# amazon-science/gnn-tail-generalization

Hardware: AMD Instinct MI355X
Metric: teachergnn_fullgraph_train_steps_per_sec (higher is better)
Workload: dtype f32

## Files before the change

### gnn-tail-generalization_amd/_lib.py

```python
import ctypes
import os

import torch

_HERE = os.path.dirname(os.path.abspath(__file__))
LIB_PATH = os.path.join(_HERE, 'lib', 'libcoldbrew_hip.so')

_c_i32p = ctypes.c_void_p
_c_f32p = ctypes.c_void_p
_I64 = ctypes.c_int64
_I32 = ctypes.c_int32
_SZ = ctypes.c_size_t
_P = ctypes.c_void_p


class CsrView(ctypes.Structure):
    _fields_ = [('rowptr', _P), ('col', _P), ('col_flags', _I32), ('n_rows', _I64), ('n_edges', _I64),
                ('hub_threshold', _I32), ('n_hubs', _I32), ('n_chunks', _I32), ('hub_rows', _P), ('hub_chunk_ptr', _P),
                ('ws', _P), ('ws_bytes', _SZ)]


class TrunkStore(ctypes.Structure):
    _fields_ = [('mix_src', _P), ('ld_mix', _I64), ('mix_index', _P), ('c_act', ctypes.c_float), ('c_mix', ctypes.c_float), ('drop_p', ctypes.c_float),
                ('seed', ctypes.c_uint64), ('seed_dev', _P), ('row0', _I64), ('relu_bits', _P), ('bits_relu_only', _I32), ('out_act', _P), ('ld_act', _I64)]


_G = ctypes.POINTER(CsrView)
_S = ctypes.POINTER(TrunkStore)

SIGNATURES = {
    'cb_version': (ctypes.c_int, []),
    'cb_last_error': (ctypes.c_char_p, []),
    'cb_device_status': (ctypes.c_int, []),
    'cb_agg_gemm_handover_selftest': (ctypes.c_int, [_P]),
    'cb_rows_zero_outside_mask_f32': (ctypes.c_int, [_P, _I64, _I64, _I64, _P, _P, _P]),
    'cb_csr_workspace_bytes': (_SZ, [_I64, _I64]),
    'cb_csr_from_coo_i64': (ctypes.c_int, [_P, _P, _I64, _I64, _P, _P, _P, _P, _P, _P, _SZ, _P]),
    'cb_deg_norm_f32': (ctypes.c_int, [_P, _I64, _P, _P]),
    'cb_csr64_from_coo_i64': (ctypes.c_int, [_P, _P, _I64, _I64, _P, _P, _P, _P, _P, _P, _SZ, _P]),
    'cb_csr_rebase_i64': (ctypes.c_int, [_P, _I64, _I64, _P, _P]),
    'cb_deg_norm_i64ptr_f32': (ctypes.c_int, [_P, _I64, _P, _P]),
    'cb_spmm_hub_count': (ctypes.c_int, [_P, _I64, _I32, _P, _P]),
    'cb_spmm_hub_fill_scratch_ints': (_I64, [_I64]),
    'cb_spmm_hub_fill': (ctypes.c_int, [_P, _I64, _I32, _I32, _P, _P, _P, _P]),
    'cb_spmm_workspace_bytes': (_SZ, [_I64, _I64]),
    'cb_spmm_csr_f32': (ctypes.c_int, [_G, _P, _I32, _I64, _I64, _P, _P, _P, ctypes.c_int, _P, _I64, _P, _I64, _P]),
    'cb_dropout_f32': (ctypes.c_int, [_P, _P, _I64, ctypes.c_float, ctypes.c_uint64, _P, _I64, _P]),
    'cb_axpby_f32': (ctypes.c_int, [ctypes.c_float, _P, ctypes.c_float, _P, _P, _I64, _P]),
    'cb_colsum_workspace_bytes': (_SZ, [_I64, _I64]),
    'cb_act_bwd_f32': (ctypes.c_int, [_P, _P, _P, _P, _I64, _I64, _P, _P, _SZ, _P]),
    'cb_reduce_workspace_bytes': (_SZ, []),
    'cb_frobenius_norm_f32': (ctypes.c_int, [_P, _I64, _P, _P, _SZ, _P]),
    'cb_nll_logsoftmax_f32': (ctypes.c_int, [_P, _I64, _P, _P, _I64, _I64, _I64, _P, _P, _P, _SZ, _P]),
    'cb_adam_step_f32': (ctypes.c_int, [_P, _P, _P, _P, _I64, ctypes.c_float, ctypes.c_float, ctypes.c_float,
                                        ctypes.c_float, ctypes.c_float, _I64, _P, _P]),
    'cb_adam_multi_f32': (ctypes.c_int, [_I32, _P, _P, _P, _P, _P, _P, ctypes.c_float, ctypes.c_float, ctypes.c_float, ctypes.c_float,
                                         ctypes.c_float, _I64, _P, _P, _P]),
    'cb_gemm_nn_workspace_bytes': (_SZ, [_I64, _I64]),
    'cb_gemm_nn_splitk_workspace_bytes': (_SZ, [_I64, _I64, _I64]),
    'cb_gemm_nn_f32': (ctypes.c_int, [_P, _I64, _P, _I64, _P, _I64, _I64, _I64, _I64, _P, _P, _I64, _P, ctypes.c_int, _P, _SZ, _P]),
    'cb_gemm_nn_drop2_f32': (ctypes.c_int, [_P, _I64, _P, _I64, _P, _I64, _P, _I64, _I64, _I64, _I64, _P, _P, _I64, _P, ctypes.c_int,
                                            ctypes.c_float, ctypes.c_uint64, _P, _I64, _P, _SZ, _P]),
    'cb_gemm_tn_workspace_bytes': (_SZ, [_I64, _I64, _I64]),
    'cb_gemm_tn_f32': (ctypes.c_int, [_P, _I64, _P, _I64, _P, _P, _I64, _I64, _I64, _P, _SZ, _P]),
    'cb_spmm_csr_fused_f32': (ctypes.c_int, [_G, _P, _P, _I32, _I64, _I64, _P, _P, _P, _I64, _S, _P, _I64, _P]),
    'cb_trunk_layer_bwd_f32': (ctypes.c_int, [_P, _P, _P, _P, ctypes.c_int, _P, ctypes.c_int, _I64, _I64, ctypes.c_float, ctypes.c_uint64,
                                              _P, _I64, ctypes.c_float, ctypes.c_float, _P, ctypes.c_uint64, ctypes.c_float, _P, _P, _P, _SZ, _P]),
    'cb_gemm_nn_bf16out_f32': (ctypes.c_int, [_P, _I64, _P, _I64, _P, _I64, _I64, _I64, _I64, _P, _P, _I64, _P, ctypes.c_int, _P, _SZ, _P]),
    'cb_node_norm_fwd_f32': (ctypes.c_int, [_P, _P, _P, _I64, _I64, ctypes.c_float, ctypes.c_float, ctypes.c_float, _P]),
    'cb_node_norm_bwd_f32': (ctypes.c_int, [_P, _P, _P, _P, _I64, _I64, ctypes.c_float, ctypes.c_float, _P]),
    'cb_colstats_workspace_bytes': (_SZ, [_I64, _I64]),
    'cb_colstats_f32': (ctypes.c_int, [_P, _P, _P, _I64, _I64, _P, _P, _P, _SZ, _P]),
    'cb_col_affine_f32': (ctypes.c_int, [_P, _P, _P, _P, ctypes.c_float, _P, _I64, _I64, _P]),
    'cb_col_bwd_combine_f32': (ctypes.c_int, [_P, _P, _P, _P, _P, _P, ctypes.c_float, ctypes.c_float, _P, _I64, _I64, _P]),
    'cb_topk_replace_workspace_bytes': (_SZ, [_I64, _I64, _I64]),
    'cb_topk_replace_f32': (ctypes.c_int, [_P, _I64, _P, _I64, _I64, _I64, _I64, _I32, _P, _P, _P, _P, _SZ, _P]),
    'cb_gather_rows_f32': (ctypes.c_int, [_P, _I64, _P, _I64, _I64, _P, _P]),
    'cb_gather_rows_bf16_f32': (ctypes.c_int, [_P, _I64, _P, _I64, _I64, _P, _P]),
    'cb_adam_norm_workspace_bytes': (ctypes.c_size_t, [_I32]),
    'cb_adam_multi_norm_f32': (ctypes.c_int, [_I32, _P, _P, _P, _P, _P, _P, _P, ctypes.c_float, ctypes.c_float, ctypes.c_float, ctypes.c_float,
                                              ctypes.c_float, _I64, _P, _P, _P, _SZ, _P]),
    'cb_expand_rows_f32': (ctypes.c_int, [_P, _P, _I64, _I64, ctypes.c_float, _P, _P]),
    'cb_gemm_nn_store_rows_supported': (ctypes.c_int, [_P, _I64, _P, _I64, _P, _I64, _I64, _I64, _I64]),
    'cb_gemm_nn_store_rows_f32': (ctypes.c_int, [_P, _I64, _P, _I64, _P, _I64, _I64, _I64, _I64, _P, _P, _I64, _P, _P, _S, _P, _SZ, _P]),
    'cb_trunk_store_rows_f32': (ctypes.c_int, [_P, _P, _I64, _I64, _S, _P, _P]),
    'cb_agg_gemm_image_bytes': (_SZ, [_I64, _I64]),
    'cb_agg_gemm_image_f32': (ctypes.c_int, [_P, _I64, _I64, _I64, ctypes.c_int, _P, _SZ, _P]),
    'cb_spmm_gemm_f32': (ctypes.c_int, [_G, _P, _I64, _I64, _P, _P, ctypes.c_int, _P, _I64, _P, _I64, _P, _P, _P, _I64, _P, _I64, _P]),
    'cb_spmm_gemm_fused_f32': (ctypes.c_int, [_G, _P, _I64, _P, _I64, _I64, _P, _P, _S, _P, _I64, _I32, _P, _P, _P, _I64, _P, _I64, _P]),
    'cb_agg_gemm_head_image_bytes': (_SZ, [_I64, _I64]),
    'cb_agg_gemm_head_image_f32': (ctypes.c_int, [_P, _I64, _I64, _I64, ctypes.c_int, _P, _SZ, _P]),
    'cb_spmm_gemm_fused_head_f32': (ctypes.c_int, [_G, _P, _I64, _P, _I64, _I64, _P, _P, _S, _P, _I64, _I32, _P, _P, _I64, _P, _I64, _P]),
    'cb_spmm_gemm_store_rows_f32': (ctypes.c_int, [_G, _P, _I64, _I64, _P, _P, _I64, _P, _P, _P, _P, _S, _P, _I64, _P]),
    'cb_spmm_csr_weighted_f32': (ctypes.c_int, [_P, _P, _P, _I64, _I64, _P, _I64, _I64, _P, _P, ctypes.c_int, _P, _I64, _P]),
    'cb_spmm_edge_dot_f32': (ctypes.c_int, [_P, _P, _I64, _I64, _P, _I64, _P, _I64, _I64, _P, _P]),
    'cb_gemm_nn_indrop_supported': (ctypes.c_int, [_P, _I64, _P, _I64, _P, _I64, _P, _I64, _I64, _I64, _I64]),
    'cb_gemm_nn_indrop_drop2_f32': (ctypes.c_int, [_P, _I64, _P, _I64, _P, _I64, _P, _I64, _I64, _I64, _I64, _P, ctypes.c_int, ctypes.c_float,
                                                   ctypes.c_uint64, ctypes.c_float, ctypes.c_uint64, _P, _I64, _P, _P]),
    'cb_gemm_nn_indrop_f32': (ctypes.c_int, [_P, _I64, _P, _I64, _P, _I64, _I64, _I64, _I64, _P, _P, _I64, _P, ctypes.c_int, ctypes.c_float,
                                             ctypes.c_uint64, _P, _I64, _P, _P]),
    'cb_gemm_tn_adrop_supported': (ctypes.c_int, [_P, _I64, _P, _I64, _I64, _I64]),
    'cb_gemm_tn_adrop_f32': (ctypes.c_int, [_P, _I64, _P, _I64, _P, _P, _I64, _I64, _I64, ctypes.c_float, ctypes.c_uint64, _P, _I64, _P, _SZ, _P]),
    'cb_front_image_bytes': (_SZ, [_I64]),
    'cb_front_image_f32': (ctypes.c_int, [_P, _I64, _I64, ctypes.c_int, _P, _SZ, _P]),
    'cb_trunk_front_f32': (ctypes.c_int, [_P, _I64, _I64, _I64, _P, _P, _P, _P, _P, _I64, _P, _I64, _P, _P, _I64, _P, _I64, ctypes.c_float,
                                          ctypes.c_uint64, ctypes.c_uint64, _P, _I64, _P]),
    'cb_gemm_tn_gdrop_supported': (ctypes.c_int, [_P, _I64, _P, _I64, _I64, _I64]),
    'cb_gemm_tn_gdrop_f32': (ctypes.c_int, [_P, _I64, _P, _I64, _P, _I64, _I64, _I64, ctypes.c_float, ctypes.c_uint64, _P, _I64, _P, _SZ, _P]),
    'cb_spmm_csr_lp_f32': (ctypes.c_int, [_G, _P, _I64, _I64, _P, _P, _I64, ctypes.c_float, _P, _P, _I64, _P]),
    'cb_spmm_csr_prop_f32': (ctypes.c_int, [_G, _P, _I64, _I64, _P, _P, _I64, ctypes.c_float, ctypes.c_float, ctypes.c_float, _P, _P, _P, _I64, _P]),
    'cb_cs_workspace_bytes': (_SZ, [_I64, _I64]),
    'cb_cs_residual_init_f32': (ctypes.c_int, [_P, _I64, _P, _P, _I64, _I64, _I64, _P, _P, _P, _P, _P, _SZ, _P]),
    'cb_cs_correct_snap_f32': (ctypes.c_int, [_I32, _P, _I64, _P, _I64, _P, _P, _I64, _I64, _I64, _P, _I64, ctypes.c_float, _P, _P, _I64, _P, _P, _P]),
    'cb_trunk_input_bwd_multi_f32': (ctypes.c_int, [_P, ctypes.c_uint64, _I32, _P, _P, ctypes.c_float, _P, _P, _I64, _I64, ctypes.c_float,
                                                    _P, _I64, _P, _P, _SZ, _P, _P, _P]),
    'cb_trunk_input_bwd_multi_cs_f32': (ctypes.c_int, [_P, ctypes.c_uint64, _I32, _P, _P, ctypes.c_float, _P, _P, _I64, _I64, ctypes.c_float,
                                                       _P, _I64, _P, _P, _SZ, _P, _P, _I32, _P, _P, _P, _P, _P, _SZ, _P]),
    'cb_spmm_csr_store_bwd_f32': (ctypes.c_int, [_G, _P, _I64, _I64, _P, _P, _P, ctypes.c_float, ctypes.c_float, ctypes.c_uint64, _P, _I64, _P, _I64, _P, _I64, _P]),
    'cb_spmm_store_bwd_mix_workspace_bytes': (_SZ, [_I64, _I64, _I64]),
    'cb_spmm_csr_store_bwd_mix_f32': (ctypes.c_int, [_G, _P, _I64, _I64, _P, _P, _P, ctypes.c_float, ctypes.c_float, ctypes.c_uint64, _P, _I64, _P, _I64, _P, _I64,
                                                     _I32, _P, _P, _P, ctypes.c_float, _P, _P, _SZ, _P]),
    'cb_gemm_tn_instage_supported': (ctypes.c_int, [_P, _P, _P, _I64, _I64, _I64]),
    'cb_gemm_tn_instage_workspace_bytes': (_SZ, [_I64, _I64]),
    'cb_gemm_tn_instage_f32': (ctypes.c_int, [_P, _P, _P, _P, _I64, _P, _P, _I64, _I64, ctypes.c_float, ctypes.c_uint64, ctypes.c_float, ctypes.c_uint64, _P, _I64,
                                              _P, _SZ, _P]),
    'cb_trunk_layer_bwd_fold_f32': (ctypes.c_int, [_P, _P, _P, _P, _I64, _I64, ctypes.c_float, ctypes.c_uint64, _P, _I64, ctypes.c_float, ctypes.c_float, _I32, _P, _P, _P,
                                                   _P, _P, _P, _SZ, _I32, _P, ctypes.c_float, _P, _P, _SZ, _P]),
    'cb_trunk_layer_bwd_rows_f32': (ctypes.c_int, [_P, _P, _I64, _P, _P, _P, _I64, ctypes.c_float, ctypes.c_uint64, _P, _I64, ctypes.c_float,
                                                   _P, ctypes.c_uint64, ctypes.c_float, _P, _P, _P, _SZ, _P]),
    'cb_id_count_i64': (ctypes.c_int, [_P, _I64, _I64, _P, _P, _P]),
    'cb_value_hist_i32': (ctypes.c_int, [_P, _I64, _I32, _P, _P, _P]),
    'cb_compact_workspace_bytes': (_SZ, [_I64]),
    'cb_select_range_i32': (ctypes.c_int, [_P, _I64, _I32, _I32, _P, _P, _P, _P, _SZ, _P]),
    'cb_craft_isolation_i64': (ctypes.c_int, [_P, _P, _I64, _P, _I64, _P, _P, _P, _P, _SZ, _P]),
    'cb_symmetrize_workspace_bytes': (_SZ, [_I64, _I64]),
    'cb_symmetrize_i64': (ctypes.c_int, [_P, _P, _I64, _I64, _P, _P, _P, _P, _P, _SZ, _P]),
    'cb_trunk_input_bwd_f32': (ctypes.c_int, [_P, _P, _P, _P, _I64, _I64, ctypes.c_float, ctypes.c_uint64, _P, _I64, _P, _P, _SZ, _P]),
    'cb_ln_gelu_drop_fwd_f32': (ctypes.c_int, [_P, _I64, _I64, _P, _P, ctypes.c_float, ctypes.c_float, ctypes.c_uint64, _P, _P, _P, _P]),
    'cb_ln_gelu_drop_bwd_workspace_bytes': (_SZ, [_I64, _I64]),
    'cb_ln_gelu_drop_bwd_f32': (ctypes.c_int, [_P, _P, _P, _I64, _I64, _P, _P, ctypes.c_float, ctypes.c_uint64, _P, _P, _P, _P, _P, _P, _SZ, _P]),
    'cb_mse_rows_f32': (ctypes.c_int, [_P, _I64, _I64, _P, _I64, _I64, _P, _P, _P, _P, _SZ, _P]),
    'cb_part2_assemble_f32': (ctypes.c_int, [_P, _I64, _P, _P, _I64, _P, _I64, _P, _P]),
    'cb_part2_assemble_bwd_f32': (ctypes.c_int, [_P, _I64, _P, _P, _I64, _I64, _P, _P, _SZ, _P]),
    'cb_ncloss_positions_i64': (ctypes.c_int, [_P, _I64, _I64, _P, _P, _P]),
    'cb_ncloss_row_norms_f32': (ctypes.c_int, [_P, _I64, _I64, _I64, _P, _P, _P]),
    'cb_cosine_scale_f32': (ctypes.c_int, [_P, _I64, _I64, _P, _P]),
    'cb_ncloss_uses_limb_core': (ctypes.c_int, [_P, _I64, _I64]),
    'cb_ncloss_workspace_bytes': (_SZ, [_I64, _I32]),
    'cb_ncloss_fwd_f32': (ctypes.c_int, [_P, _I64, _I64, _I64, ctypes.c_float, _P, _P, _P, _I64, _P, _P, _P, _I32, _P, _P, _P, _P, _P, _P, _P, _P, _SZ, _P]),
    'cb_ncloss_normalize_rows_f32': (ctypes.c_int, [_P, _I64, _I64, _I64, _P, _P, _P]),
    'cb_ncloss_bwd_slab_f32': (ctypes.c_int, [_P, _I64, _I64, _I64, ctypes.c_float, _P, _P, _I64, _I64, _I32, _P, _I64, _P]),
    'cb_ncloss_bwd_finish_f32': (ctypes.c_int, [_P, _I64, _P, _I64, _I64, ctypes.c_float, _P, _P, _P, _P, _P, _P, _P, _P, _I64, _P, _P, _P, _P, _P, _P, _P]),
    'cb_spgemm_offsets_workspace_bytes': (_SZ, [_I64]),
    'cb_spgemm_entry_offsets_i64': (ctypes.c_int, [_P, _I64, _P, _I64, _P, _P, _P, _SZ, _P]),
    'cb_spgemm_chunk_workspace_bytes': (_SZ, [_I64]),
    'cb_spgemm_chunk_count_f32': (ctypes.c_int, [_P, _P, _P, _P, _P, _P, _P, _I64, _I64, _I64, _I64, _I64, _P, _P, _SZ, _P]),
    'cb_spgemm_chunk_emit_f32': (ctypes.c_int, [_P, _SZ, _I64, _I64, _I64, _I64, _I64, _I64, _P, _P, _P, _P]),
    'cb_csr_transpose_workspace_bytes': (_SZ, [_I64]),
    'cb_csr_transpose_f32': (ctypes.c_int, [_P, _P, _P, _I64, _I64, _I64, _P, _P, _P, _P, _SZ, _P]),
    'cb_linkp_max_tries': (ctypes.c_int, []),
    'cb_linkp_valid_counts_i32': (ctypes.c_int, [_P, _P, _I32, _P, _P]),
    'cb_linkp_positives_i32': (ctypes.c_int, [_P, _P, _I32, _P, _I64, _I64, ctypes.c_uint64, _P, _P, _P]),
    'cb_linkp_negatives_i32': (ctypes.c_int, [_P, _P, _I32, _P, _I64, _I64, ctypes.c_uint64, _P, _P, _P, _P]),
    'cb_linkp_loss_fwd_f32': (ctypes.c_int, [_P, _I64, _I64, _I64, _P, _I64, _P, _I64, _P, _P, _P, _P, _P]),
    'cb_linkp_mrr_f32': (ctypes.c_int, [_P, _I64, _P, _I64, _P, _P]),
    'cb_linkp_bwd_workspace_bytes': (_SZ, [_I64, _I64]),
    'cb_linkp_loss_bwd_f32': (ctypes.c_int, [_P, _I64, _I64, _I64, _P, _I64, _P, _I64, _P, _P, _P, _I64, _P, _SZ, _P]),
    'cb_heur_aa_weights_f64': (ctypes.c_int, [_P, _P, _P]),
    'cb_heur_pair_scores_f32': (ctypes.c_int, [_P, _P, _P, _I64, _P, _P, _P]),
    'cb_heur_pair_scores_width_f32': (ctypes.c_int, [_P, _P, _P, _I64, _I32, _P, _P, _P]),
    'cb_rank_counts_workspace_bytes': (_SZ, [_I64, _I64]),
    'cb_rank_counts_f32': (ctypes.c_int, [_P, _I64, _P, _I64, _P, _P, _P, _P, _SZ, _P]),
    'cb_lpx_max_tries': (ctypes.c_int, []),
    'cb_lpx_neg_global_i32': (ctypes.c_int, [_P, _I64, ctypes.c_uint64, _P, _P, _P]),
    'cb_lpx_neg_local_i32': (ctypes.c_int, [_P, _I64, _I64, _I64, ctypes.c_uint64, _P, _P]),
    'cb_lpx_permutation_workspace_bytes': (_SZ, [_I64]),
    'cb_lpx_permutation_i32': (ctypes.c_int, [_I64, ctypes.c_uint64, _P, _P, _SZ, _P]),
    'cb_lpx_row_ranks_f32': (ctypes.c_int, [_P, _I64, _P, _I64, _I64, _P, _P, _P, _P]),
    'cb_lpx_recall_topk_workspace_bytes': (_SZ, [_I64, _I64]),
    'cb_lpx_recall_topk_f32': (ctypes.c_int, [_P, _I64, _P, _I64, _I64, _P, _P, _P, _SZ, _P]),
    'cb_pair_gemm_nn_supported': (ctypes.c_int, [_P, _I64, _P, _I64, _I64, _I64]),
    'cb_pair_gemm_nn_f32': (ctypes.c_int, [_P, _I64, _I64, _P, _I64, _P, _I64, _P, _I64, _P, _I64, _I64, _I64, _P, ctypes.c_int, ctypes.c_float,
                                           ctypes.c_uint64, _P, _I64, _P, _P]),
    'cb_pair_dot_f32': (ctypes.c_int, [_P, _I64, _I64, _I64, _P, _I64, _P, _P, _P]),
    'cb_pair_scatter_workspace_bytes': (_SZ, [_I64]),
    'cb_pair_scatter_f32': (ctypes.c_int, [_P, _I64, _I64, _I64, _P, _I64, _P, _I64, _P, _I64, _P, _SZ, _P]),
    'cb_rank_loss_workspace_bytes': (_SZ, []),
    'cb_rank_loss_fwd_f32': (ctypes.c_int, [_I32, _P, _I64, _P, _I64, _P, _P, _P, _SZ, _P]),
    'cb_rank_loss_bwd_f32': (ctypes.c_int, [_I32, _P, _I64, _P, _I64, _P, _P, _P, _P, _P]),
    'cb_rows_gemm_nn_supported': (ctypes.c_int, [_P, _I64, _I64, _I32, _P, _I64, _I64]),
    'cb_rows_gemm_nn_f32': (ctypes.c_int, [_P, _I64, _I64, _I64, _P, _I32, _I64, _P, _I64, _P, _I64, _P, _I64, _I64, _P, ctypes.c_int, ctypes.c_float,
                                           ctypes.c_uint64, _P, _I64, _P, _P]),
    'cb_rows_bilinear_supported': (ctypes.c_int, [_P, _I64, _I64, _P, _I64]),
    'cb_rows_bilinear_workspace_bytes': (_SZ, [_I64, _I64]),
    'cb_rows_bilinear_f32': (ctypes.c_int, [_P, _I64, _I64, _I64, _P, _I64, _P, _I64, _P, _P, _P, _SZ, _P]),
    'cb_rows_scatter_f32': (ctypes.c_int, [_I64, _I64, _P, _I64, _P, _I64, _P, _I64, _P, _I64, _P, _SZ, _P]),
    'cb_sage_image_bytes': (_SZ, [ctypes.c_int]),
    'cb_sage_image_f32': (ctypes.c_int, [_P, _I64, _P, _I64, ctypes.c_int, _P, _SZ, _P]),
    'cb_sage_layer_supported': (ctypes.c_int, [_I64, _I64, _I32, _P, _I64, _P, _I64, _P, _I64, _P, _I64]),
    'cb_sage_layer_f32': (ctypes.c_int, [_P, _P, _I64, _P, _I64, _P, _P, _P, _P, ctypes.c_int, ctypes.c_float, ctypes.c_uint64, _P, _I64, _P, _I64, _I32,
                                         _P, _I64, _P]),
    'cb_attn_supported': (ctypes.c_int, [_I64, _P, _I64]),
    'cb_attn_workspace_bytes': (_SZ, [_I64, _I64]),
    'cb_attn_fwd_f32': (ctypes.c_int, [_P, _I64, _P, _I64, _P, _I64, _P, _I64, _P, _I64, ctypes.c_int, _P, _I64, _P, _P]),
    'cb_attn_bwd_dst_f32': (ctypes.c_int, [_P, _I64, _P, _I64, _P, _I64, _P, _I64, _P, _I64, _P, _P, _I64, _P, _P]),
    'cb_attn_bwd_src_f32': (ctypes.c_int, [_P, _I64, _P, _I64, _P, _I64, _P, _I64, _P, _I64, _P, _P, _P, _I64, _P, _I64, _P]),
}

# ... 89 lines not shown
```

### gnn-tail-generalization_amd/csrc/cb_front.hip

```cpp
#include <type_traits>

#include "cb_common.h"
#include "cb_limb_core.h"
#include "cb_philox.h"
#include "cb_tile_gemm.h"
#include "cb_trunk_store.h"

namespace cb {

struct FrontArgs {
  const float* x;
  int64_t ld_x;
  const uint4* image_in;
  const float* bias_in;
  const uint4* image_0;
  const float* rowscale;
  const float* addend;
  int64_t ld_add;
  float* x0;
  int64_t ld_x0;
  unsigned long long* bits;
  float* x0_drop;
  int64_t ld_drop;
  float* z0;
  int64_t ld_z;
  int64_t M;
  uint32_t thresh;
  float keep_scale;
  uint64_t seed_x, seed_x0;
  const uint64_t* seed_dev;
  int64_t row0;
  int n_tiles;
};

template <int NS1, bool DROP>
__global__ void __launch_bounds__(256, 2) k_front(FrontArgs fa) {
  constexpr int K1 = 16 * NS1, LDX = K1 + 4, NV = kTM * K1 / 4 / 256;
  static_assert(NV >= 1 && kTM * LDX <= kTM * kTLD, "x tile must fit the region of the X0 tile");
  static_assert(NV == NS1 && NS1 <= 8, "mask draws: one quad per K step, P0's bits in one word");
  __shared__ __attribute__((aligned(16))) float tile[kTM * kTLD];
  constexpr int kScratch = 2 * RowOperand<kTM>::BYTES > 4 * 8 * kCLD * 4 ? 2 * RowOperand<kTM>::BYTES : 4 * 8 * kCLD * 4;
  __shared__ __attribute__((aligned(16))) char scratch[kScratch];
  float (*cstrip)[8 * kCLD] = reinterpret_cast<float (*)[8 * kCLD]>(scratch);
  __shared__ float rs_tile[2][kTM];
  const int t = threadIdx.x, lane = t & 63, w = __builtin_amdgcn_readfirstlane(t >> 6);
  const uint64_t sx = fa.seed_dev ? fa.seed_x + *fa.seed_dev : fa.seed_x, s0 = fa.seed_dev ? fa.seed_x0 + *fa.seed_dev : fa.seed_x0;
  float4 xr[NV];
  auto load_x = [&](int tile_id) {
    const int64_t m0 = (int64_t)tile_id * kTM;
#pragma unroll
    for (int j = 0; j < NV; ++j) {
      const int idx = t + 256 * j, row = idx / (K1 / 4), c4 = idx % (K1 / 4);
      const int64_t m = m0 + row;
      xr[j] = (tile_id < fa.n_tiles && m < fa.M) ? *reinterpret_cast<const float4*>(fa.x + m * fa.ld_x + 4 * c4) : make_float4(0.f, 0.f, 0.f, 0.f);
    }
  };
  float rs_next = 1.f;
  auto load_rs = [&](int tile_id) {
    const int64_t m = (int64_t)tile_id * kTM + t;
    rs_next = (t < kTM && fa.rowscale && tile_id < fa.n_tiles && m < fa.M) ? fa.rowscale[m] : 1.f;
  };
  float bvec[4] = {0.f, 0.f, 0.f, 0.f};
  if (fa.bias_in) {
#pragma unroll
    for (int i = 0; i < 4; ++i) bvec[i] = fa.bias_in[4 * lane + i];
  }
  load_rs(blockIdx.x);
  load_x(blockIdx.x);
  uint32_t kx = 0;
  uint64_t k3 = 0;
  int64_t qx = 0, q3 = 0;
  auto aim_x = [&](int tile_id) { qx = (fa.row0 + (int64_t)tile_id * kTM) * (K1 / 4) + t; };
  auto aim_3 = [&](int tile_id) { q3 = (fa.row0 + (int64_t)tile_id * kTM + 16 * w) * (kND / 4) + lane; };
  auto draw_x = [&](int) {
    uint64_t seed = sx;
    asm volatile("" : "+s"(seed));
    kx = (kx >> 4) | (keep4_bits(seed, qx, fa.thresh) << 28);
    qx += 256;
    asm volatile("" : "+v"(kx));
  };
  auto draw_3 = [&](int) {
    uint64_t seed = s0;
    asm volatile("" : "+s"(seed));
    k3 = (k3 >> 4) | ((uint64_t)keep4_bits(seed, q3, fa.thresh) << 60);
    q3 += kND / 4;
    asm volatile("" : "+v"(k3));
  };
  if constexpr (DROP) {
    aim_x(blockIdx.x);
    aim_3(blockIdx.x);
#pragma unroll 1
    for (int s = 0; s < 16; ++s) {
      if (s < NS1) draw_x(s);
      draw_3(s);
    }
  }
  int par = 0;
  for (int tile_id = blockIdx.x; tile_id < fa.n_tiles; tile_id += gridDim.x, par ^= 1) {
    const int64_t m0 = (int64_t)tile_id * kTM;
#pragma unroll
    for (int j = 0; j < NV; ++j) {
      const int idx = t + 256 * j, row = idx / (K1 / 4), c4 = idx % (K1 / 4);
      float v[4] = {xr[j].x, xr[j].y, xr[j].z, xr[j].w};
      if constexpr (DROP) {
#pragma unroll
        for (int i = 0; i < 4; ++i) v[i] = mul_rounded(v[i], (kx >> (32 - 4 * NV + 4 * j + i)) & 1u ? fa.keep_scale : 0.f);
      }
      *reinterpret_cast<float4*>(tile + row * LDX + 4 * c4) = make_float4(v[0], v[1], v[2], v[3]);
    }
    if constexpr (DROP) aim_x(tile_id + (int)gridDim.x);
    if (t < kTM) rs_tile[par][t] = rs_next;
    __syncthreads();
    f32x16 acc[2][2];
    if constexpr (DROP) tile_times_image_coop<NS1, LDX, 1>(tile, scratch, fa.image_in, w, lane, t, acc, draw_x);
    else tile_times_image_coop<NS1, LDX, 1>(tile, scratch, fa.image_in, w, lane, t, acc);
    {
      const int l31 = lane & 31, lh = lane >> 5;
#pragma unroll
      for (int i = 0; i < 2; ++i)
#pragma unroll
        for (int j = 0; j < 2; ++j)
#pragma unroll
          for (int reg = 0; reg < 16; ++reg)
            tile[(32 * i + (reg & 3) + 8 * (reg >> 2) + 4 * lh) * kTLD + 64 * w + 32 * j + l31] = acc[i][j][reg];
    }
    __syncthreads();
#pragma unroll 4
    for (int r = 0; r < 16; ++r) {
      const int row = 16 * w + r;
      const int64_t m = m0 + row;
      float* tp = tile + row * kTLD + 4 * lane;
      const float4 v = *reinterpret_cast<const float4*>(tp);
      float o[4] = {v.x, v.y, v.z, v.w};
#pragma unroll
      for (int i = 0; i < 4; ++i) o[i] = fmaxf(o[i] + bvec[i], 0.f);
      float xd[4] = {o[0], o[1], o[2], o[3]};
      if constexpr (DROP) {
#pragma unroll
        for (int i = 0; i < 4; ++i) xd[i] = o[i] * ((uint32_t)k3 >> i & 1u ? fa.keep_scale : 0.f);
        k3 >>= 4;
      }
      *reinterpret_cast<float4*>(tp) = make_float4(xd[0], xd[1], xd[2], xd[3]);
      if (m < fa.M) {
        store_stream4(fa.x0 + m * fa.ld_x0 + 4 * lane, o);
        if (fa.bits) {
          const bool pos[4] = {o[0] > 0.f, o[1] > 0.f, o[2] > 0.f, o[3] > 0.f};
          write_row_mask_words(fa.bits + m * 4, lane, pos);
        }
        if (fa.x0_drop) store_stream4(fa.x0_drop + m * fa.ld_drop + 4 * lane, xd);
      }
    }
    __syncthreads();
    if constexpr (DROP) aim_3(tile_id + (int)gridDim.x);
    if constexpr (DROP) tile_times_image_coop<kNS, kTLD, 1>(tile, scratch, fa.image_0, w, lane, t, acc, draw_3);
    else tile_times_image_coop<kNS, kTLD, 1>(tile, scratch, fa.image_0, w, lane, t, acc);
    load_rs(tile_id + gridDim.x);
    load_x(tile_id + gridDim.x);
    auto z0_epilogue = [&](auto HAS_ADD) {
      acc_rows_through_strip(acc, cstrip[w], w, lane, [&](int row, int n, const float4& v) {
        const int64_t m = m0 + row;
        if (m < fa.M) {
          const float rs = rs_tile[par][row];
          float ad[4] = {0.f, 0.f, 0.f, 0.f};
          if constexpr (decltype(HAS_ADD)::value) {
            const float4 a4 = *reinterpret_cast<const float4*>(fa.addend + m * fa.ld_add + n);
            ad[0] = a4.x; ad[1] = a4.y; ad[2] = a4.z; ad[3] = a4.w;
          }
          const float zero_bias = 0.f;
          float o[4] = {v.x, v.y, v.z, v.w};
#pragma unroll
          for (int e = 0; e < 4; ++e) o[e] = o[e] * rs + ad[e] + zero_bias;
          store_stream4(fa.z0 + m * fa.ld_z + n, o);
        }
      });
    };
    if (fa.addend) z0_epilogue(std::true_type{});
    else z0_epilogue(std::false_type{});
  }
}

}

using namespace cb;

extern "C" size_t cb_front_image_bytes(int64_t K) {
  if (K != 64 && K != 128) return 0;
  return (size_t)(K / 16) * kNT * 3 * 64 * sizeof(uint4);
}

extern "C" int cb_front_image_f32(const float* W, int64_t ld, int64_t K, int transpose, void* image, size_t image_bytes, void* stream) {
  CB_CHECK_ARG(cb_front_image_bytes(K) > 0, CB_E_INVALID, "cb_front_image_f32: K must be 64 or 128 (got %lld)", (long long)K);
  CB_CHECK_ARG(W && image && ld >= (transpose ? K : kND), CB_E_INVALID, "cb_front_image_f32: null pointer / bad leading dimension");
  CB_CHECK_ARG(image_bytes >= cb_front_image_bytes(K) && aligned16(image), CB_E_WORKSPACE, "cb_front_image_f32: image buffer too small or misaligned");
  const int64_t sk = transpose ? 1 : ld, sn = transpose ? ld : 1;
  const int ns = (int)(K / 16);
  hipLaunchKernelGGL(k_weight_image, dim3(ns * kNT * 64 / 256), dim3(256), 0, (hipStream_t)stream, W, sk, sn, (uint4*)image, ns);
  CB_LAUNCH_CHECK();
  return CB_OK;
}

extern "C" int cb_trunk_front_f32(const float* x, int64_t ld_x, int64_t M, int64_t K, const void* image_in, const float* bias_in, const void* image_0,
                                  const float* rowscale, const float* addend, int64_t ld_add, float* x0, int64_t ld_x0, uint64_t* relu_bits,
                                  float* x0_drop, int64_t ld_drop, float* z0, int64_t ld_z, float drop_p, uint64_t seed_x, uint64_t seed_x0,
                                  const uint64_t* seed_dev, int64_t row0, void* stream) {
  CB_CHECK_ARG(M >= 0 && cb_front_image_bytes(K) > 0 && drop_p >= 0.f && drop_p < 1.f && row0 >= 0, CB_E_INVALID,
               "cb_trunk_front_f32: bad size (K must be 64 or 128; hidden width 256) or p");
  CB_CHECK_ARG(M < ((int64_t)1 << 31) * kTM / 2, CB_E_RANGE, "cb_trunk_front_f32: size out of range");
  if (M == 0) return CB_OK;
  CB_CHECK_ARG(x && image_in && image_0 && x0 && z0, CB_E_INVALID, "cb_trunk_front_f32: null pointer");
  CB_CHECK_ARG(aligned16(x) && ld_x % 4 == 0 && ld_x >= K && aligned16(image_in) && aligned16(image_0) && aligned16(x0) && ld_x0 % 4 == 0 && ld_x0 >= kND &&
                   aligned16(z0) && ld_z % 4 == 0 && ld_z >= kND && (!addend || (aligned16(addend) && ld_add % 4 == 0 && ld_add >= kND)) &&
                   (!x0_drop || (aligned16(x0_drop) && ld_drop % 4 == 0 && ld_drop >= kND)) && (!relu_bits || (uintptr_t)relu_bits % 8 == 0),
               CB_E_INVALID, "cb_trunk_front_f32: 16-byte aligned rows required");
  FrontArgs fa{x, ld_x, (const uint4*)image_in, bias_in, (const uint4*)image_0, rowscale, addend, ld_add, x0, ld_x0, (unsigned long long*)relu_bits,
               x0_drop, ld_drop, z0, ld_z, M};
  fa.thresh = drop_p > 0.f ? dropout_threshold(drop_p) : 0u;
  fa.keep_scale = 1.f / (1.f - drop_p);
  fa.seed_x = seed_x; fa.seed_x0 = seed_x0; fa.seed_dev = seed_dev; fa.row0 = row0;
  fa.n_tiles = (int)((M + kTM - 1) / kTM);
  int dev = 0, n_cu = 0;
  if (hipGetDevice(&dev) != hipSuccess || hipDeviceGetAttribute(&n_cu, hipDeviceAttributeMultiprocessorCount, dev) != hipSuccess || n_cu <= 0) n_cu = 256;
  const int blocks = fa.n_tiles < 2 * n_cu ? fa.n_tiles : 2 * n_cu;
  const dim3 grid((unsigned)blocks), blk(256);
  hipStream_t st = (hipStream_t)stream;
  if (K == 64 && fa.thresh) hipLaunchKernelGGL((k_front<4, true>), grid, blk, 0, st, fa);
  else if (K == 64) hipLaunchKernelGGL((k_front<4, false>), grid, blk, 0, st, fa);
  else if (fa.thresh) hipLaunchKernelGGL((k_front<8, true>), grid, blk, 0, st, fa);
  else hipLaunchKernelGGL((k_front<8, false>), grid, blk, 0, st, fa);
  CB_LAUNCH_CHECK();
  return CB_OK;
}
```

### gnn-tail-generalization_amd/csrc/cb_gemm.hip

```cpp
#include <stdlib.h>

#include "cb_common.h"
#include "cb_gemm_core.h"
#include "cb_gemm_limb.h"

namespace cb {

template <int WM, int WN, bool ALIGNED, bool OUT_BF16, int BKT = BK, int WTN = 2>
__global__ void __launch_bounds__(256) k_gemm_nn(const float* __restrict__ A, int64_t lda, const float* __restrict__ B, int64_t ldb,
                                                 void* __restrict__ Cv, int64_t ldc, int64_t M, int N, int K, GemmEpilogue ep,
                                                 int n_row_blocks, int n_col_blocks, int c_vec_ok, int k_chunk) {
  using T = Tile<WM, WN, BKT, WTN>;
  if (k_chunk) {
    const int k0 = blockIdx.y * k_chunk;
    A += k0;
    B += (int64_t)k0 * ldb;
    Cv = reinterpret_cast<float*>(Cv) + (int64_t)blockIdx.y * M * ldc;
    K = min(k_chunk, K - k0);
  }
  constexpr int BM = T::BM, BN = T::BN, LDA = T::LDA, LDB = T::LDB;
  __shared__ __attribute__((aligned(16))) float smem[T::SMEM_FLOATS];
  auto As = [&](int b) { return smem + b * (BKT * LDA); };
  auto Bs = [&](int b) { return smem + 2 * BKT * LDA + b * (BKT * LDB); };
  const int per_group = 8 * n_col_blocks;
// ... 302 lines not shown
               "cb_gemm_nn_bf16out_f32: null pointer or leading dimension too small");
  GemmEpilogue ep{rowscale, addend, ld_add, bias, relu, nullptr, 0, 0u, 1.f, 0ull, nullptr, 0, gemm_nt_store(M, N)};
  hipStream_t st = (hipStream_t)stream;
  if (limb3_on() && limb3_nn_eligible(A, lda, B, ldb, N, K)) return launch_nn_limb3(A, lda, B, ldb, C, ldc, M, N, K, ep, true, st, ws, ws_bytes);
  if (N <= 64) return launch_nn<4, 1, true>(A, lda, B, ldb, C, ldc, M, N, K, ep, st);
  return launch_nn<2, 2, true>(A, lda, B, ldb, C, ldc, M, N, K, ep, st);
}

extern "C" size_t cb_gemm_tn_workspace_bytes(int64_t M, int64_t K1, int64_t K2) {
  if (M <= 0 || K1 <= 0 || K2 <= 0) return 0;
  int bm, bn;
  tn_tile(K1, K2, bm, bn);
  const int tiles = (int)(((K1 + bm - 1) / bm) * ((K2 + bn - 1) / bn));
  return (size_t)tn_splits(M, tiles) * (size_t)K1 * (size_t)K2 * sizeof(float);
}

extern "C" int cb_gemm_nn_store_rows_supported(const float* A, int64_t lda, const float* B, int64_t ldb, const float* C, int64_t ldc, int64_t M, int64_t N,
                                               int64_t K) {
  return limb3_on() && N == 256 && M > 0 && limb3_nn_eligible(A, lda, B, ldb, N, K) && aligned16(C) && ldc % 4 == 0 ? 1 : 0;
}

extern "C" int cb_gemm_nn_store_rows_f32(const float* A, int64_t lda, const float* B, int64_t ldb, float* C, int64_t ldc, int64_t M, int64_t N, int64_t K,
                                         const float* rowscale, const float* addend, int64_t ld_add, const float* bias, const int64_t* row_index,
                                         const cb_trunk_store* store, void* ws, size_t ws_bytes, void* stream) {
  CB_CHECK_ARG(M >= 0 && N == 256 && K > 0, CB_E_INVALID, "cb_gemm_nn_store_rows_f32: bad size (N must be 256)");
  CB_CHECK_ARG(K < (1 << 24) && (M + 63) / 64 < (1 << 24), CB_E_RANGE, "cb_gemm_nn_store_rows_f32: size out of range");
  if (M == 0) return CB_OK;
  CB_CHECK_ARG(A && B && C && row_index && lda >= K && ldb >= N && ldc >= N && (!addend || ld_add >= N), CB_E_INVALID,
               "cb_gemm_nn_store_rows_f32: null pointer or leading dimension too small");
  const int rcs = check_trunk_store("cb_gemm_nn_store_rows_f32", store, N);
  if (rcs != CB_OK) return rcs;
  CB_CHECK_ARG(cb_gemm_nn_store_rows_supported(A, lda, B, ldb, C, ldc, M, N, K) && (!addend || (aligned16(addend) && ld_add % 4 == 0)), CB_E_INVALID,
               "cb_gemm_nn_store_rows_f32: shape / alignment outside the fused form (cb_gemm_nn_store_rows_supported)");
  GemmEpilogue ep{rowscale, addend, ld_add, bias, 1, nullptr, 0, 0u, 1.f, 0ull, nullptr, 0, 0};
  ep.row_ids = row_index; ep.st = make_trunk_store(*store);
  return launch_nn_limb3(A, lda, B, ldb, C, ldc, M, N, K, ep, false, (hipStream_t)stream, ws, ws_bytes);
}

extern "C" int cb_gemm_tn_f32(const float* A, int64_t lda, const float* G, int64_t ldg, const float* rowscale, float* C, int64_t M,
                              int64_t K1, int64_t K2, void* ws, size_t ws_bytes, void* stream) {
  CB_CHECK_ARG(M >= 0 && K1 >= 0 && K2 >= 0, CB_E_INVALID, "cb_gemm_tn_f32: negative size");
  CB_CHECK_ARG(K1 < (1 << 20) && K2 < (1 << 20), CB_E_RANGE, "cb_gemm_tn_f32: size out of range");
  if (K1 == 0 || K2 == 0) return CB_OK;
  CB_CHECK_ARG(C && (M == 0 || (A && G)) && lda >= K1 && ldg >= K2, CB_E_INVALID, "cb_gemm_tn_f32: null pointer or bad ld");
  hipStream_t st = (hipStream_t)stream;
  if (M == 0) {
    CB_HIP(hipMemsetAsync(C, 0, (size_t)K1 * K2 * sizeof(float), st));
    return CB_OK;
  }
  CB_CHECK_ARG(ws && ws_bytes >= cb_gemm_tn_workspace_bytes(M, K1, K2), CB_E_WORKSPACE, "cb_gemm_tn_f32: workspace too small");
  int bm, bn;
  tn_tile(K1, K2, bm, bn);
  if (bm == 64) return launch_tn<1, 4>(A, lda, G, ldg, rowscale, C, M, K1, K2, (float*)ws, st);
  if (bm == 256) return launch_tn<4, 1>(A, lda, G, ldg, rowscale, C, M, K1, K2, (float*)ws, st);
  return launch_tn<2, 2>(A, lda, G, ldg, rowscale, C, M, K1, K2, (float*)ws, st);
}

extern "C" int cb_gemm_tn_gdrop_supported(const float* A, int64_t lda, const float* G, int64_t ldg, int64_t K1, int64_t K2) {
  return limb3_on() && K2 % 4 == 0 && limb3_tn_eligible(A, lda, G, ldg, K1, K2) ? 1 : 0;
}

extern "C" int cb_gemm_tn_gdrop_f32(const float* A, int64_t lda, const float* G, int64_t ldg, float* C, int64_t M, int64_t K1, int64_t K2,
                                    float g_drop_p, uint64_t g_seed, const uint64_t* seed_dev, int64_t row0, void* ws, size_t ws_bytes,
                                    void* stream) {
  CB_CHECK_ARG(M >= 0 && K1 >= 0 && K2 >= 0 && g_drop_p > 0.f && g_drop_p < 1.f && row0 >= 0, CB_E_INVALID, "cb_gemm_tn_gdrop_f32: bad size or p");
  CB_CHECK_ARG(K1 < (1 << 20) && K2 < (1 << 20), CB_E_RANGE, "cb_gemm_tn_gdrop_f32: size out of range");
  if (K1 == 0 || K2 == 0) return CB_OK;
  CB_CHECK_ARG(C && (M == 0 || (A && G)) && lda >= K1 && ldg >= K2, CB_E_INVALID, "cb_gemm_tn_gdrop_f32: null pointer or bad ld");
  hipStream_t st = (hipStream_t)stream;
  if (M == 0) {
    CB_HIP(hipMemsetAsync(C, 0, (size_t)K1 * K2 * sizeof(float), st));
    return CB_OK;
  }
  CB_CHECK_ARG(cb_gemm_tn_gdrop_supported(A, lda, G, ldg, K1, K2), CB_E_INVALID, "cb_gemm_tn_gdrop_f32: operands outside the three-limb path");
  CB_CHECK_ARG(ws && ws_bytes >= cb_gemm_tn_workspace_bytes(M, K1, K2), CB_E_WORKSPACE, "cb_gemm_tn_gdrop_f32: workspace too small");
  const DropSpec gd{dropout_threshold(g_drop_p), 1.f / (1.f - g_drop_p), g_seed, seed_dev, row0, K2};
  int bm, bn;
  tn_tile(K1, K2, bm, bn);
  if (bm == 64) return launch_tn<1, 4>(A, lda, G, ldg, nullptr, C, M, K1, K2, (float*)ws, st, &gd);
  if (bm == 256) return launch_tn<4, 1>(A, lda, G, ldg, nullptr, C, M, K1, K2, (float*)ws, st, &gd);
  return launch_tn<2, 2>(A, lda, G, ldg, nullptr, C, M, K1, K2, (float*)ws, st, &gd);
}

static inline int instage_splits(int64_t M) { return tn_splits(M, 2); }

extern "C" int cb_gemm_tn_instage_supported(const float* g, const float* mfold, const float* X, int64_t ldx, int64_t M, int64_t K2) {
  return limb3_on() && K2 > 64 && K2 <= 128 && K2 % 4 == 0 && ldx % 4 == 0 && ldx >= K2 && ldx < (1 << 22) && aligned16(g) && aligned16(mfold) && aligned16(X) && M > 0 &&
                 instage_splits(M) >= 256
             ? 1
             : 0;
}

extern "C" size_t cb_gemm_tn_instage_workspace_bytes(int64_t M, int64_t K2) {
  if (M <= 0 || K2 <= 0) return 0;
  return (size_t)instage_splits(M) * (size_t)256 * (size_t)(K2 + 1) * sizeof(float);
}

extern "C" int cb_gemm_tn_instage_f32(const float* g, const float* mfold, const uint64_t* x0_bits, const float* X, int64_t ldx, float* C, float* colsum, int64_t M,
                                      int64_t K2, float g_drop_p, uint64_t g_seed, float x_drop_p, uint64_t x_seed, const uint64_t* seed_dev, int64_t row0, void* ws,
                                      size_t ws_bytes, void* stream) {
  CB_CHECK_ARG(M > 0 && K2 > 0 && g_drop_p > 0.f && g_drop_p < 1.f && x_drop_p > 0.f && x_drop_p < 1.f && row0 >= 0, CB_E_INVALID,
               "cb_gemm_tn_instage_f32: bad size or p (both dropouts must be active)");
  CB_CHECK_ARG(g && mfold && x0_bits && X && C && colsum && (uintptr_t)x0_bits % 8 == 0, CB_E_INVALID, "cb_gemm_tn_instage_f32: null or misaligned pointer");
  CB_CHECK_ARG(cb_gemm_tn_instage_supported(g, mfold, X, ldx, M, K2), CB_E_INVALID, "cb_gemm_tn_instage_f32: shape / alignment outside the fused form (cb_gemm_tn_instage_supported)");
  CB_CHECK_ARG(ws && ws_bytes >= cb_gemm_tn_instage_workspace_bytes(M, K2), CB_E_WORKSPACE, "cb_gemm_tn_instage_f32: workspace too small");
  hipStream_t st = (hipStream_t)stream;
  const int nsplit = instage_splits(M);
  int64_t rows_per_split = (M + nsplit - 1) / nsplit;
  rows_per_split = (rows_per_split + 31) / 32 * 32;
  const DropSpec xd{dropout_threshold(x_drop_p), 1.f / (1.f - x_drop_p), x_seed, seed_dev, row0, K2};
  const DropSpec gd{dropout_threshold(g_drop_p), 1.f / (1.f - g_drop_p), g_seed, seed_dev, row0, 256};
  float* partial = (float*)ws;
  float* cs_partial = partial + (size_t)nsplit * 256 * K2;
  const int rc = launch_tn_instage(g, mfold, x0_bits, X, ldx, partial, cs_partial, M, K2, nsplit, rows_per_split, st, xd, gd);
  if (rc != CB_OK) return rc;
  const int64_t n = 256 * K2;
  hipLaunchKernelGGL(k_sum_partials, dim3((unsigned)((n + 255) / 256)), dim3(256), 0, st, (const float*)partial, nsplit, n, C);
  CB_LAUNCH_CHECK();
  hipLaunchKernelGGL(k_sum_partials, dim3(1), dim3(256), 0, st, (const float*)cs_partial, nsplit, (int64_t)256, colsum);
  CB_LAUNCH_CHECK();
  return CB_OK;
}

extern "C" int cb_gemm_nn_indrop_f32(const float* A, int64_t lda, const float* B, int64_t ldb, float* C, int64_t ldc, int64_t M, int64_t N, int64_t K,
                                     const float* rowscale, const float* addend, int64_t ld_add, const float* bias, int relu, float a_drop_p,
                                     uint64_t a_seed, const uint64_t* seed_dev, int64_t row0, uint64_t* relu_bits, void* stream) {
  CB_CHECK_ARG(M >= 0 && N >= 0 && K >= 0 && a_drop_p > 0.f && a_drop_p < 1.f && row0 >= 0, CB_E_INVALID, "cb_gemm_nn_indrop_f32: bad size or p");
  CB_CHECK_ARG(!relu_bits || (N == 256 && relu && (uintptr_t)relu_bits % 8 == 0), CB_E_INVALID,
               "cb_gemm_nn_indrop_f32: mask words of the ReLU exist for N == 256 with relu only");
  CB_CHECK_ARG(N < (1 << 24) && K < (1 << 24) && (M + 63) / 64 < (1 << 24), CB_E_RANGE, "cb_gemm_nn_indrop_f32: size out of range");
  if (M == 0 || N == 0) return CB_OK;
  CB_CHECK_ARG(C && A && B && lda >= K && ldb >= N && ldc >= N && (!addend || ld_add >= N), CB_E_INVALID, "cb_gemm_nn_indrop_f32: null pointer or bad ld");
  CB_CHECK_ARG(cb_gemm_nn_indrop_supported(A, lda, B, ldb, C, ldc, C, ldc, M, N, K) && (!addend || (aligned16(addend) && ld_add % 4 == 0)), CB_E_INVALID,
               "cb_gemm_nn_indrop_f32: shape / alignment outside the fused form (cb_gemm_nn_indrop_supported)");
  GemmEpilogue ep{rowscale, addend, ld_add, bias, relu, nullptr, 0, 0u, 1.f, 0ull, nullptr, 0, gemm_nt_store(M, N)};
  ep.adrop = DropSpec{dropout_threshold(a_drop_p), 1.f / (1.f - a_drop_p), a_seed, seed_dev, row0, K};
  ep.relu_bits_out = (unsigned long long*)relu_bits;
  return launch_nn_limb3(A, lda, B, ldb, C, ldc, M, N, K, ep, false, (hipStream_t)stream, nullptr, 0);
}

extern "C" int cb_gemm_tn_adrop_supported(const float* A, int64_t lda, const float* G, int64_t ldg, int64_t K1, int64_t K2) {
  int bm, bn;
  tn_tile(K1, K2, bm, bn);
  return limb3_on() && K1 % 4 == 0 && bm == 128 && limb3_tn_eligible(A, lda, G, ldg, K1, K2) ? 1 : 0;
}

extern "C" int cb_gemm_tn_adrop_f32(const float* A, int64_t lda, const float* G, int64_t ldg, const float* rowscale, float* C, int64_t M, int64_t K1,
                                    int64_t K2, float a_drop_p, uint64_t a_seed, const uint64_t* seed_dev, int64_t row0, void* ws, size_t ws_bytes,
                                    void* stream) {
  CB_CHECK_ARG(M >= 0 && K1 >= 0 && K2 >= 0 && a_drop_p > 0.f && a_drop_p < 1.f && row0 >= 0, CB_E_INVALID, "cb_gemm_tn_adrop_f32: bad size or p");
  CB_CHECK_ARG(K1 < (1 << 20) && K2 < (1 << 20), CB_E_RANGE, "cb_gemm_tn_adrop_f32: size out of range");
  if (K1 == 0 || K2 == 0) return CB_OK;
  CB_CHECK_ARG(C && (M == 0 || (A && G)) && lda >= K1 && ldg >= K2, CB_E_INVALID, "cb_gemm_tn_adrop_f32: null pointer or bad ld");
  hipStream_t st = (hipStream_t)stream;
  if (M == 0) {
    CB_HIP(hipMemsetAsync(C, 0, (size_t)K1 * K2 * sizeof(float), st));
    return CB_OK;
  }
  CB_CHECK_ARG(cb_gemm_tn_adrop_supported(A, lda, G, ldg, K1, K2), CB_E_INVALID, "cb_gemm_tn_adrop_f32: operands outside the three-limb 128-row tile path");
  CB_CHECK_ARG(ws && ws_bytes >= cb_gemm_tn_workspace_bytes(M, K1, K2), CB_E_WORKSPACE, "cb_gemm_tn_adrop_f32: workspace too small");
  const DropSpec ad{dropout_threshold(a_drop_p), 1.f / (1.f - a_drop_p), a_seed, seed_dev, row0, K1};
  return launch_tn<2, 2>(A, lda, G, ldg, rowscale, C, M, K1, K2, (float*)ws, st, nullptr, &ad);
}
```

### gnn-tail-generalization_amd/csrc/cb_gemm_limb.h

```cpp
#pragma once
#include "cb_gemm_core.h"

namespace cb {

bool limb3_on();
bool limb3_nn_eligible(const float* A, int64_t lda, const float* B, int64_t ldb, int64_t N, int64_t K);
size_t limb3_nn_workspace_bytes(int64_t N, int64_t K);
int launch_nn_limb3(const float* A, int64_t lda, const float* B, int64_t ldb, void* C, int64_t ldc, int64_t M, int64_t N, int64_t K,
                    const GemmEpilogue& ep, bool out_bf16, hipStream_t st, void* ws = nullptr, size_t ws_bytes = 0);
bool limb3_nn_dual_eligible(const float* A, int64_t lda, const float* B, int64_t ldb, const float* C, int64_t ldc, const float* C2, int64_t ldc2,
                            int64_t M, int64_t N, int64_t K, const GemmEpilogue& ep);
bool limb3_tn_eligible(const float* A, int64_t lda, const float* G, int64_t ldg, int64_t K1, int64_t K2);
int launch_tn_limb3(const float* A, int64_t lda, const float* G, int64_t ldg, const float* rowscale, float* partial, int64_t M,
                    int64_t K1, int64_t K2, int bm, int nsplit, int64_t rows_per_split, hipStream_t st, const DropSpec* gdrop = nullptr,
                    const DropSpec* adrop = nullptr);

int launch_tn_instage(const float* g, const float* mfold, const uint64_t* x0_bits, const float* X, int64_t ldx, float* partial, float* cs_partial, int64_t M, int64_t K2,
                      int nsplit, int64_t rows_per_split, hipStream_t st, const DropSpec& xd, const DropSpec& gd);

}
```

### gnn-tail-generalization_amd/csrc/cb_gemm_limb.hip

```cpp
#include <stdlib.h>

#include <utility>

#include "cb_common.h"
#include "cb_gemm_core.h"
#include "cb_gemm_limb.h"
#include "cb_limb_core.h"

namespace cb {

template <int WM, int WN, int WTN = 2, int PD = 1>
struct LTile {
  static constexpr int BM = 64 * WM, BN = 32 * WTN * WN;
  static constexpr int MINW = (WM == 2 && WTN == 2 && PD < 3 ? 3 : 2);
  static constexpr int NTHR = 64 * WM * WN;
  static_assert(WM * WN == 4 || WM * WN == 8, "four or eight wavefronts per block");
};

template <int WM, int WN, bool OUT_BF16, int WTN = 2, int PD = 1, int EPI = 0, bool ADROP = false>
__global__ void __launch_bounds__(256, (LTile<WM, WN, WTN, PD>::MINW)) k_gemm_nn_l3(const float* __restrict__ A, int64_t lda,
                                                                                 const float* __restrict__ B, int64_t ldb,
                                                                                 void* __restrict__ Cv, int64_t ldc, int64_t M, int N,
                                                                                 int K, GemmEpilogue ep, int n_row_blocks,
                                                                                 int n_col_blocks, int c_vec_ok) {
  using T = LTile<WM, WN, WTN>;
  using OA = RowOperand<T::BM, ADROP>;
  using OB = ColOperand<T::BN, false>;
  constexpr int BM = T::BM, BN = T::BN;
  constexpr int SMEM = 2 * (OA::BYTES + OB::BYTES);
  static_assert(32 * (BN + 4) * 4 <= SMEM, "epilogue staging must fit");
  __shared__ __attribute__((aligned(16))) char smem[SMEM];
  const int per_group = 8 * n_col_blocks;
  const int grp = blockIdx.x / per_group, r = blockIdx.x % per_group;
  const int row_blk = grp * 8 + (r & 7), col_blk = r >> 3;
  if (row_blk >= n_row_blocks) return;
  const int64_t m0 = (int64_t)row_blk * BM;
  const int n0 = col_blk * BN;
  const int t = threadIdx.x, lane = t & 63, w = t >> 6, wr = w / WN, wc = w % WN;

  f32x16 acc[2][WTN];
  zero_acc_n<WTN>(acc);
  OA oa;
  OB ob;
  oa.init(lda, M - m0, t);
  if constexpr (ADROP) oa.set_drop(ep.adrop, m0, K, t);
  ob.init(ldb, N - n0, t);
  const uint32_t aaddr[2] = {OA::frag_addr(wr * 64, lane), OA::frag_addr(wr * 64 + 32, lane)};
  uint32_t baddr[WTN];
#pragma unroll
  for (int j = 0; j < WTN; ++j) baddr[j] = OB::frag_addr(wc * (32 * WTN) + 32 * j, lane);
  limb_k_loop<WTN, PD, OA, OB>(oa, ob, smem, A + m0 * lda, KS, lda, B + n0, (int64_t)KS * ldb, ldb, nullptr, K, aaddr, baddr, acc, t);
  nn_epilogue<WM, WN, WTN, OUT_BF16, EPI>(acc, reinterpret_cast<float*>(smem), Cv, ldc, m0, n0, M, N, ep, c_vec_ok, t);
}

template <int WM, int WN, bool SCALED, int WTN = 2, int PD = 1, bool GDROP = false, bool ADROP = false>
__global__ void __launch_bounds__((LTile<WM, WN, WTN, PD>::NTHR), (LTile<WM, WN, WTN, PD>::MINW)) k_gemm_tn_l3(const float* __restrict__ A, int64_t lda,
                                                                                 const float* __restrict__ G, int64_t ldg,
                                                                                 const float* __restrict__ rowscale,
                                                                                 float* __restrict__ partial, int64_t M, int K1, int K2,
                                                                                 int64_t rows_per_split, int tiles_j, int n_tiles,
                                                                                 int nsplit, DropSpec gd) {
  using T = LTile<WM, WN, WTN>;
  using OA = ColOperand<T::BM, false, ADROP, T::NTHR>;
  using OB = ColOperand<T::BN, SCALED, GDROP, T::NTHR>;
  constexpr int BM = T::BM, BN = T::BN;
  __shared__ __attribute__((aligned(16))) char smem[2 * (OA::BYTES + OB::BYTES)];
  const int b = blockIdx.x;
  const int tile = (b >> 3) % n_tiles, split = (b & 7) + 8 * (b / (8 * n_tiles));
  if (split >= nsplit) return;
  const int i0 = (tile / tiles_j) * BM, j0 = (tile % tiles_j) * BN;
  const int64_t r_begin = (int64_t)split * rows_per_split;
  const int64_t r_end = min(M, r_begin + rows_per_split);
  const int t = threadIdx.x, lane = t & 63, w = t >> 6, wr = w / WN, wc = w % WN;

  f32x16 acc[2][WTN];
  zero_acc_n<WTN>(acc);
  OA oa;
  OB ob;
  oa.init(lda, K1 - i0, t);
  ob.init(ldg, K2 - j0, t);
  if constexpr (GDROP) ob.set_drop(gd, r_begin, r_end - r_begin, j0, t);
  if constexpr (ADROP) oa.set_drop(gd, r_begin, r_end - r_begin, i0, t);
  const uint32_t aaddr[2] = {OA::frag_addr(wr * 64, lane), OA::frag_addr(wr * 64 + 32, lane)};
  uint32_t baddr[WTN];
#pragma unroll
  for (int j = 0; j < WTN; ++j) baddr[j] = OB::frag_addr(wc * (32 * WTN) + 32 * j, lane);
  limb_k_loop<WTN, PD, OA, OB>(oa, ob, smem, A + r_begin * lda + i0, (int64_t)KS * lda, lda, G + r_begin * ldg + j0, (int64_t)KS * ldg, ldg,
                           SCALED ? rowscale + r_begin : nullptr, r_end - r_begin, aaddr, baddr, acc, t);
  const int l31 = lane & 31, lh = lane >> 5;
  float* P = partial + (int64_t)split * K1 * K2;
#pragma unroll
  for (int ti = 0; ti < 2; ++ti)
#pragma unroll
    for (int tj = 0; tj < WTN; ++tj) {
      const int n = j0 + wc * (32 * WTN) + tj * 32 + l31;
      if (n >= K2) continue;
#pragma unroll
      for (int reg = 0; reg < 16; ++reg) {
        const int m = i0 + wr * 64 + ti * 32 + (reg & 3) + 8 * (reg >> 2) + 4 * lh;
        if (m < K1) P[(int64_t)m * K2 + n] = acc[ti][tj][reg];
      }
    }
}

__global__ void __launch_bounds__(512, 2) k_gemm_tn_instage(const float* __restrict__ g, const float* __restrict__ mfold,
                                                            const unsigned long long* __restrict__ x0_bits, const float* __restrict__ X, int64_t ldx,
                                                            float* __restrict__ partial, float* __restrict__ cs_partial, int64_t M, int K2,
                                                            int64_t rows_per_split, int nsplit, DropSpec xd, DropSpec gd) {
  using T = LTile<4, 2, 2>;
  using OA = ColOperandInStage<T::NTHR>;
  using OB = ColOperand<T::BN, false, true, T::NTHR>;
  constexpr int K1 = 256;
  __shared__ __attribute__((aligned(16))) char smem[2 * (OA::BYTES + OB::BYTES)];
  const int split = blockIdx.x;
  if (split >= nsplit) return;
  const int64_t r_begin = (int64_t)split * rows_per_split;
  const int64_t r_end = min(M, r_begin + rows_per_split);
  const int t = threadIdx.x, lane = t & 63, w = t >> 6, wr = w / 2, wc = w % 2;

  f32x16 acc[2][2];
  zero_acc_n<2>(acc);
  OA oa;
  OB ob;
  oa.init(K1, K1, t);
  ob.init(ldx, K2, t);
  oa.set_stage(g, mfold, x0_bits + r_begin * 4, gd, r_begin, r_end - r_begin, t);
  ob.set_drop(xd, r_begin, r_end - r_begin, 0, t);
  const uint32_t aaddr[2] = {OA::frag_addr(wr * 64, lane), OA::frag_addr(wr * 64 + 32, lane)};
  uint32_t baddr[2];
#pragma unroll
  for (int j = 0; j < 2; ++j) baddr[j] = OB::frag_addr(wc * 64 + 32 * j, lane);
  limb_k_loop<2, 1, OA, OB>(oa, ob, smem, g + r_begin * K1, (int64_t)KS * K1, K1, X + r_begin * ldx, (int64_t)KS * ldx, ldx, nullptr, r_end - r_begin, aaddr, baddr,
                            acc, t);
  const int l31 = lane & 31, lh = lane >> 5;
  float* P = partial + (int64_t)split * K1 * K2;
#pragma unroll
  for (int ti = 0; ti < 2; ++ti)
#pragma unroll
    for (int tj = 0; tj < 2; ++tj) {
      const int n = wc * 64 + tj * 32 + l31;
      if (n >= K2) continue;
#pragma unroll
      for (int reg = 0; reg < 16; ++reg) {
        const int m = wr * 64 + ti * 32 + (reg & 3) + 8 * (reg >> 2) + 4 * lh;
        P[(int64_t)m * K2 + n] = acc[ti][tj][reg];
      }
    }
  float* red = reinterpret_cast<float*>(smem);
#pragma unroll
  for (int i = 0; i < 4; ++i) red[w * 256 + lane * 4 + i] = oa.cs[i];
  __syncthreads();
  if (t < 256) {
    float s = 0.f;
#pragma unroll
    for (int j = 0; j < 8; ++j) s += red[j * 256 + t];
    cs_partial[(int64_t)split * 256 + t] = s;
  }
}

int launch_tn_instage(const float* g, const float* mfold, const uint64_t* x0_bits, const float* X, int64_t ldx, float* partial, float* cs_partial, int64_t M, int64_t K2,
                      int nsplit, int64_t rows_per_split, hipStream_t st, const DropSpec& xd, const DropSpec& gd) {
  hipLaunchKernelGGL(k_gemm_tn_instage, dim3((unsigned)nsplit), dim3(512), 0, st, g, mfold, (const unsigned long long*)x0_bits, X, ldx, partial, cs_partial, M, (int)K2,
                     rows_per_split, nsplit, xd, gd);
  CB_LAUNCH_CHECK();
  return CB_OK;
}

template <int WM, int WN, bool OUT_BF16, int WTN = 2>
static int launch_nn_l3_t(const float* A, int64_t lda, const float* B, int64_t ldb, void* C, int64_t ldc, int64_t M, int64_t N,
                          int64_t K, GemmEpilogue ep, hipStream_t st, void* ws = nullptr, size_t ws_bytes = 0) {
  using T = LTile<WM, WN, WTN>;
  const int nrb = (int)((M + T::BM - 1) / T::BM), ncb = (int)((N + T::BN - 1) / T::BN);
  const int64_t groups = (nrb + 7) / 8;
  const int c_vec_ok = ((uintptr_t)C % (OUT_BF16 ? 8 : 16) == 0) && ldc % 4 == 0 && (!ep.addend || (aligned16(ep.addend) && ep.ld_add % 4 == 0));
  const dim3 grid((unsigned)(groups * 8 * ncb));
  if constexpr (!OUT_BF16 && WM == 2 && WTN == 4) {
    if (ep.out2) {
      if (ep.adrop.thresh)
        hipLaunchKernelGGL((k_gemm_nn_l3<WM, WN, false, WTN, 1, 1, true>), grid, dim3(256), 0, st, A, lda, B, ldb, C, ldc, M, (int)N, (int)K, ep,
                           nrb, ncb, c_vec_ok);
      else
        hipLaunchKernelGGL((k_gemm_nn_l3<WM, WN, false, WTN, 1, 1>), grid, dim3(256), 0, st, A, lda, B, ldb, C, ldc, M, (int)N, (int)K, ep, nrb,
                           ncb, c_vec_ok);
      CB_LAUNCH_CHECK();
      return CB_OK;
    }
    if (ep.row_ids) {
      hipLaunchKernelGGL((k_gemm_nn_l3<WM, WN, false, WTN, 1, 2>), grid, dim3(256), 0, st, A, lda, B, ldb, C, ldc, M, (int)N, (int)K, ep, nrb, ncb, c_vec_ok);
      CB_LAUNCH_CHECK();
      return CB_OK;
    }
    if (ep.adrop.thresh) {
      hipLaunchKernelGGL((k_gemm_nn_l3<WM, WN, false, WTN, 1, 0, true>), grid, dim3(256), 0, st, A, lda, B, ldb, C, ldc, M, (int)N, (int)K, ep, nrb,
                         ncb, c_vec_ok);
      CB_LAUNCH_CHECK();
      return CB_OK;
    }
  }
  CB_CHECK_ARG(!ep.adrop.thresh, CB_E_INVALID, "NN contraction with operand dropout: wide fp32 tile only (check cb_gemm_nn_indrop_supported first)");
  hipLaunchKernelGGL((k_gemm_nn_l3<WM, WN, OUT_BF16, WTN, 1>), grid, dim3(256), 0, st, A, lda, B, ldb, C, ldc, M, (int)N, (int)K, ep, nrb, ncb,
                     c_vec_ok);
  CB_LAUNCH_CHECK();
  return CB_OK;
}

bool limb3_on() {
  static const bool on = getenv("CB_GEMM_PLAIN_F32") == nullptr;
  return on;
}

bool limb3_nn_eligible(const float* A, int64_t lda, const float* B, int64_t ldb, int64_t N, int64_t K) {
  return aligned16(A) && aligned16(B) && lda % 4 == 0 && ldb % 4 == 0 && K % 4 == 0 && N % 4 == 0 && K > 0 && lda < (1 << 22) && ldb < (1 << 22);
}

bool limb3_nn_dual_eligible(const float* A, int64_t lda, const float* B, int64_t ldb, const float* C, int64_t ldc, const float* C2, int64_t ldc2,
                            int64_t M, int64_t N, int64_t K, const GemmEpilogue& ep) {
  return N > 128 && ((M + 127) / 128) * ((N + 255) / 256) >= 256 && limb3_nn_eligible(A, lda, B, ldb, N, K) && aligned16(C) && aligned16(C2) && ldc % 4 == 0 && ldc2 % 4 == 0 &&
         (!ep.addend || (aligned16(ep.addend) && ep.ld_add % 4 == 0));
}

size_t limb3_nn_workspace_bytes(int64_t, int64_t) { return 0; }

int launch_nn_limb3(const float* A, int64_t lda, const float* B, int64_t ldb, void* C, int64_t ldc, int64_t M, int64_t N, int64_t K,
                    const GemmEpilogue& ep, bool out_bf16, hipStream_t st, void* ws, size_t ws_bytes) {
  if (N <= 64) {
    return out_bf16 ? launch_nn_l3_t<4, 1, true>(A, lda, B, ldb, C, ldc, M, N, K, ep, st)
                    : launch_nn_l3_t<4, 1, false>(A, lda, B, ldb, C, ldc, M, N, K, ep, st);
  }
  const bool fills = ((M + 127) / 128) * ((N + 255) / 256) >= 256 || ep.out2 || ep.adrop.thresh || ep.row_ids;
  if (N > 128 && fills)
    return out_bf16 ? launch_nn_l3_t<2, 2, true, 4>(A, lda, B, ldb, C, ldc, M, N, K, ep, st, ws, ws_bytes)
                    : launch_nn_l3_t<2, 2, false, 4>(A, lda, B, ldb, C, ldc, M, N, K, ep, st, ws, ws_bytes);
  return out_bf16 ? launch_nn_l3_t<2, 2, true>(A, lda, B, ldb, C, ldc, M, N, K, ep, st, ws, ws_bytes)
                  : launch_nn_l3_t<2, 2, false>(A, lda, B, ldb, C, ldc, M, N, K, ep, st, ws, ws_bytes);
}

template <int WM, int WN, int WTN = 2>
static void launch_tn_l3_t(const float* A, int64_t lda, const float* G, int64_t ldg, const float* rowscale, float* partial, int64_t M,
                           int64_t K1, int64_t K2, int nsplit, int64_t rows_per_split, hipStream_t st, const DropSpec& gd, const DropSpec& ad) {
  using T = LTile<WM, WN, WTN>;
  const int ti = (int)((K1 + T::BM - 1) / T::BM), tj = (int)((K2 + T::BN - 1) / T::BN);
  const dim3 grid((unsigned)(((nsplit + 7) / 8) * 8 * ti * tj));
#define CB_TN_LAUNCH(SC_, GD_, AD_)                                                                                                  \
  hipLaunchKernelGGL((k_gemm_tn_l3<WM, WN, SC_, WTN, 1, GD_, AD_>), grid, dim3(T::NTHR), 0, st, A, lda, G, ldg, rowscale, partial, M, (int)K1, \
                     (int)K2, rows_per_split, tj, ti * tj, nsplit, gd.thresh ? gd : ad)
  if (gd.thresh) CB_TN_LAUNCH(false, true, false);
// ... 40 lines not shown
```

### gnn-tail-generalization_amd/csrc/cb_limb_core.h

```cpp
#pragma once
#include <utility>

#include "cb_common.h"
#include "cb_gemm_core.h"
#include "cb_philox.h"

namespace cb {

typedef __bf16 bf16x8 __attribute__((ext_vector_type(8)));

__device__ __forceinline__ void split3x2(float a0, float a1, uint32_t& hi, uint32_t& mid, uint32_t& lo) {
  hi = cvt_pk_bf16(a0, a1);
  const float r0 = a0 - __uint_as_float(hi << 16), r1 = a1 - __uint_as_float(hi & 0xffff0000u);
  mid = cvt_pk_bf16(r0, r1);
  const float s0 = r0 - __uint_as_float(mid << 16), s1 = r1 - __uint_as_float(mid & 0xffff0000u);
  lo = cvt_pk_bf16(s0, s1);
}

__device__ __forceinline__ void split4(const float (&v)[4], uint2 (&pl)[3]) {
  uint32_t h[2], m[2], l[2];
  split3x2(v[0], v[1], h[0], m[0], l[0]);
  split3x2(v[2], v[3], h[1], m[1], l[1]);
  pl[0] = make_uint2(h[0], h[1]);
  pl[1] = make_uint2(m[0], m[1]);
  pl[2] = make_uint2(l[0], l[1]);
}

typedef short s16x4 __attribute__((ext_vector_type(4)));
typedef __attribute__((address_space(3))) s16x4 lds_s16x4;

constexpr int KS = 16;

__device__ __forceinline__ float mul_rounded(float x, float m) {
  float r = x * m;
  asm volatile("" : "+v"(r));
  return r;
}

template <int R, bool DROP = false>
struct RowOperand {
  static constexpr int PLANE = R * 32, BYTES = 3 * PLANE, NV = R / 64;
  static_assert(NV >= 1, "tile rows");
  uint32_t voff[NV];
  uint32_t woff;
  uint32_t rmask;
  static constexpr bool HAS_SC = false;
  float sc[1];
  uint64_t dseed;
  uint32_t dthresh;
  float dscale;
  int64_t dK, dbase[NV];
  __device__ __forceinline__ void set_drop(const DropSpec& d, int64_t m0, int64_t Ktot, int t) {
    dseed = d.seed_dev ? d.seed + *d.seed_dev : d.seed;
    dthresh = d.thresh;
    dscale = d.scale;
    dK = Ktot;
#pragma unroll
    for (int j = 0; j < NV; ++j) dbase[j] = (d.row0 + m0 + (t >> 2) + 64 * j) * d.width + (t & 3) * 4;
  }
  __device__ __forceinline__ void init(int64_t ld, int64_t rows_left, int t) {
    const int row = t >> 2, kq = t & 3;
    woff = row * 32 + (((kq >> 1) ^ ((row >> 3) & 1)) << 4) + ((kq & 1) << 3);
    rmask = 0;
#pragma unroll
    for (int j = 0; j < NV; ++j) {
      const bool in = row + 64 * j < rows_left;
      rmask |= in ? (1u << j) : 0u;
      voff[j] = in ? (uint32_t)((row + 64 * j) * ld + kq * 4) : 0u;
    }
  }
  template <int J>
  __device__ __forceinline__ void load(float4 (&f)[NV], const float* __restrict__ base, int64_t , int64_t k_left, const float*,
                                       int t) const {
    f[J] = *reinterpret_cast<const float4*>(base + ((t & 3) * 4 < k_left ? voff[J] : 0u));
  }
  template <int J>
  __device__ __forceinline__ void stage(const float4 (&f)[NV], char* __restrict__ S, int64_t k_left, int t) const {
    const bool live = ((rmask >> J) & 1) && (t & 3) * 4 < k_left;
    float v[4] = {live ? f[J].x : 0.f, live ? f[J].y : 0.f, live ? f[J].z : 0.f, live ? f[J].w : 0.f};
    if constexpr (DROP) {
      float mk[4];
      keep4(dseed, (dbase[J] + (dK - k_left)) >> 2, dthresh, dscale, mk);
#pragma unroll
      for (int i = 0; i < 4; ++i) v[i] = mul_rounded(v[i], mk[i]);
    }
    uint2 pl[3];
    split4(v, pl);
#pragma unroll
    for (int p = 0; p < 3; ++p) *reinterpret_cast<uint2*>(S + p * PLANE + woff + J * (64 * 32)) = pl[p];
  }
  static __device__ __forceinline__ uint32_t frag_addr(int r0, int lane) {
    const int row = r0 + (lane & 31);
    return row * 32 + (((lane >> 5) ^ ((row >> 3) & 1)) << 4);
  }
  static __device__ __forceinline__ bf16x8 frag(const char* __restrict__ S, uint32_t addr, int plane) {
    return __builtin_bit_cast(bf16x8, *reinterpret_cast<const uint4*>(S + plane * PLANE + addr));
  }
};


template <int R, int NIDX>
struct GatheredRows {
  static constexpr int PLANE = R * 32, BYTES = 3 * PLANE, NV = R / 64;
  static_assert(NV >= 1, "tile rows");
  int32_t nd[NIDX][NV];
  uint32_t woff;
  static constexpr bool HAS_SC = false;
  float sc[1];
  static __device__ __forceinline__ bool row_of(const int32_t* __restrict__ idx, int64_t Rn, int64_t rows_left, int64_t N, int row, int (&n)[NIDX], bool& in) {
    in = row < rows_left;
    bool ok = in;
#pragma unroll
    for (int s = 0; s < NIDX; ++s) {
      n[s] = in ? idx[s * Rn + row] : 0;
      ok = ok && n[s] >= 0 && n[s] < N;
    }
    return ok;
  }
  template <class OA>
// ... 84 lines not shown
    f[J] = *reinterpret_cast<const float4*>(base + ((int64_t)node * ld + col + kq4));
  }
  template <int J>
  __device__ __forceinline__ void stage(const float4 (&f)[NV], char* __restrict__ S, int64_t k_left, int t) const {
    const bool live = nd[0][J] >= 0 && (t & 3) * 4 < k_left;
    const float v[4] = {live ? f[J].x : 0.f, live ? f[J].y : 0.f, live ? f[J].z : 0.f, live ? f[J].w : 0.f};
    this->template store<J>(v, S);
  }
};

template <int C, bool SCALED, bool DROP = false, int NT = 256>
struct ColOperand {
  static constexpr int ROWB = C * 2, PLANE = 16 * ROWB, BYTES = 3 * PLANE;
  static constexpr int TPR = C / 4, KPP = NT / TPR, NV = 16 / KPP;
  static_assert(KPP >= 4 && KPP % 4 == 0 && NV >= 1, "staging map: whole swizzle groups of k rows per pass");
  static constexpr int NC = C / 32;
  static_assert(NC == 2 || NC == 4 || NC == 8, "tile widths 64 / 128 / 256");
  static __device__ __forceinline__ int swz(int k) { return NC == 2 ? ((k >> 1) & 1) : (k & 3); }
  uint32_t voff[NV];
  uint32_t woff;
  bool cok;
  static constexpr bool HAS_SC = SCALED;
  float sc[SCALED ? NV : 1];
  uint64_t dseed;
  uint32_t dthresh;
  float dscale;
  int64_t drow, dtot, dwidth;
  int dcol;
  __device__ __forceinline__ void set_drop(const DropSpec& d, int64_t r_begin, int64_t total, int j0, int t) {
    dseed = d.seed_dev ? d.seed + *d.seed_dev : d.seed;
    dthresh = d.thresh;
    dscale = d.scale;
    drow = d.row0 + r_begin + t / TPR;
    dtot = total;
    dwidth = d.width;
    dcol = j0 + (t % TPR) * 4;
  }
  __device__ __forceinline__ void init(int64_t ld, int cols_left, int t) {
    const int k = t / TPR, nq = t % TPR;
    cok = nq * 4 < cols_left;
#pragma unroll
    for (int j = 0; j < NV; ++j) voff[j] = (uint32_t)((k + KPP * j) * ld + (cok ? nq * 4 : 0));
    woff = k * ROWB + ((((nq >> 3) ^ swz(k)) & (NC - 1)) << 6) + ((nq & 7) << 3);
  }
  template <int J>
  __device__ __forceinline__ void load(float4 (&f)[NV], const float* __restrict__ base, int64_t , int64_t k_left,
                                       const float* __restrict__ kscale, int t) {
    const int k = t / TPR + KPP * J;
    const bool kin = k < k_left;
    f[J] = *reinterpret_cast<const float4*>(base + (kin ? voff[J] : 0u));
    if constexpr (SCALED) sc[J] = kscale[kin ? k : 0];
  }
  template <int J>
  __device__ __forceinline__ void stage(const float4 (&f)[NV], char* __restrict__ S, int64_t k_left, int t) const {
    const bool live = cok && t / TPR + KPP * J < k_left;
    const float m = SCALED ? sc[SCALED ? J : 0] : 1.f;
    float v[4] = {live ? f[J].x * m : 0.f, live ? f[J].y * m : 0.f, live ? f[J].z * m : 0.f, live ? f[J].w * m : 0.f};
    if constexpr (DROP) {
      static_assert(!SCALED, "dropout of a row-scaled operand is not needed anywhere");
      float mk[4];
      keep4(dseed, ((drow + KPP * J + (dtot - k_left)) * dwidth + dcol) >> 2, dthresh, dscale, mk);
#pragma unroll
      for (int i = 0; i < 4; ++i) v[i] = mul_rounded(v[i], mk[i]);
    }
    uint2 pl[3];
    split4(v, pl);
#pragma unroll
    for (int p = 0; p < 3; ++p) *reinterpret_cast<uint2*>(S + p * PLANE + woff + J * (KPP * ROWB)) = pl[p];
  }
  static __device__ __forceinline__ uint32_t frag_addr(int c0, int lane) {
    const int L = lane & 15, k = 8 * (lane >> 5) + (L >> 2);
    return k * ROWB + ((((c0 >> 5) ^ swz(k)) & (NC - 1)) << 6) + (((lane >> 4) & 1) << 5) + ((L & 3) << 3);
  }
  static __device__ __forceinline__ bf16x8 frag(const char* __restrict__ S, uint32_t addr, int plane) {
    const char* q = S + plane * PLANE + addr;
    const s16x4 lo = __builtin_amdgcn_ds_read_tr16_b64_v4i16((lds_s16x4*)(q));
    const s16x4 hi = __builtin_amdgcn_ds_read_tr16_b64_v4i16((lds_s16x4*)(q + 4 * ROWB));
    typedef short s16x8 __attribute__((ext_vector_type(8)));
    const s16x8 v = __builtin_shufflevector(lo, hi, 0, 1, 2, 3, 4, 5, 6, 7);
    return __builtin_bit_cast(bf16x8, v);
  }
};

template <int NT = 512>
struct ColOperandInStage {
  static constexpr int C = 256;
  static constexpr int ROWB = C * 2, PLANE = 16 * ROWB, BYTES = 3 * PLANE;
  static constexpr int TPR = C / 4, KPP = NT / TPR, NV = 16 / KPP;
  static_assert(TPR == 64 && KPP >= 4 && KPP % 4 == 0 && NV >= 1, "one wavefront per k row");
  static constexpr int NC = C / 32;
  static __device__ __forceinline__ int swz(int k) { return k & 3; }
  uint32_t voff[NV];
  uint32_t woff;
  bool cok;
  static constexpr bool HAS_SC = false;
  float sc[1];
  int64_t mdelta;
  const unsigned long long* bits;
  float4 fm[NV];
  unsigned long long bw[NV][4];
  uint64_t dseed;
  uint32_t dthresh;
  float dscale;
  int64_t drow, dtot, dwidth;
  int dcol, kw;
  float cs[4];
  __device__ __forceinline__ void set_stage(const float* g, const float* mfold, const unsigned long long* bits_block, const DropSpec& d, int64_t r_begin, int64_t total,
                                            int t) {
    mdelta = mfold - g;
    bits = bits_block;
    dseed = d.seed_dev ? d.seed + *d.seed_dev : d.seed;
    dthresh = d.thresh;
    dscale = d.scale;
    kw = __builtin_amdgcn_readfirstlane(t / TPR);
    drow = d.row0 + r_begin + kw;
    dtot = total;
    dwidth = d.width;
    dcol = (t % TPR) * 4;
#pragma unroll
    for (int i = 0; i < 4; ++i) cs[i] = 0.f;
  }
  __device__ __forceinline__ void init(int64_t ld, int cols_left, int t) {
    const int k = t / TPR, nq = t % TPR;
    cok = nq * 4 < cols_left;
#pragma unroll
    for (int j = 0; j < NV; ++j) voff[j] = (uint32_t)((k + KPP * j) * ld + (cok ? nq * 4 : 0));
    woff = k * ROWB + ((((nq >> 3) ^ swz(k)) & (NC - 1)) << 6) + ((nq & 7) << 3);
  }
  template <int J>
  __device__ __forceinline__ void load(float4 (&f)[NV], const float* __restrict__ base, int64_t , int64_t k_left, const float* __restrict__, int ) {
    const int k = kw + KPP * J;
    const bool kin = k < k_left;
    const float* p = base + (kin ? voff[J] : 0u);
    f[J] = *reinterpret_cast<const float4*>(p);
    fm[J] = *reinterpret_cast<const float4*>(p + mdelta);
    const unsigned long long* b = bits + ((dtot - k_left) + (kin ? k : 0)) * 4;
#pragma unroll
    for (int i = 0; i < 4; ++i) bw[J][i] = b[i];
  }
  template <int J>
  __device__ __forceinline__ void stage(const float4 (&f)[NV], char* __restrict__ S, int64_t k_left, int t) {
    const bool live = cok && kw + KPP * J < k_left;
    const int lane = t & 63;
    float mk[4];
    keep4(dseed, ((drow + KPP * J + (dtot - k_left)) * dwidth + dcol) >> 2, dthresh, dscale, mk);
    const float gv[4] = {f[J].x, f[J].y, f[J].z, f[J].w}, mv[4] = {fm[J].x, fm[J].y, fm[J].z, fm[J].w};
    float v[4];
#pragma unroll
    for (int i = 0; i < 4; ++i) {
      const float tsum = mul_rounded(gv[i], mk[i]) + mv[i];
      v[i] = (live && ((bw[J][i] >> lane) & 1ull)) ? tsum : 0.f;
      cs[i] += v[i];
    }
    uint2 pl[3];
    split4(v, pl);
#pragma unroll
    for (int p = 0; p < 3; ++p) *reinterpret_cast<uint2*>(S + p * PLANE + woff + J * (KPP * ROWB)) = pl[p];
  }
  static __device__ __forceinline__ uint32_t frag_addr(int c0, int lane) {
    const int L = lane & 15, k = 8 * (lane >> 5) + (L >> 2);
    return k * ROWB + ((((c0 >> 5) ^ swz(k)) & (NC - 1)) << 6) + (((lane >> 4) & 1) << 5) + ((L & 3) << 3);
  }
  static __device__ __forceinline__ bf16x8 frag(const char* __restrict__ S, uint32_t addr, int plane) {
    const char* q = S + plane * PLANE + addr;
    const s16x4 lo = __builtin_amdgcn_ds_read_tr16_b64_v4i16((lds_s16x4*)(q));
    const s16x4 hi = __builtin_amdgcn_ds_read_tr16_b64_v4i16((lds_s16x4*)(q + 4 * ROWB));
    typedef short s16x8 __attribute__((ext_vector_type(8)));
    const s16x8 v = __builtin_shufflevector(lo, hi, 0, 1, 2, 3, 4, 5, 6, 7);
    return __builtin_bit_cast(bf16x8, v);
  }
};

template <class OPA, class OPB>
struct Producer {
  OPA& oa;
  OPB& ob;
  float4 (&fa)[OPA::NV];
  float4 (&fb)[OPB::NV];
  char* dstA;
  char* dstB;
  const float* abase;
  const float* bbase;
  const float* bscale;
  int64_t lda, ldb;
  int64_t left1, left2;
  int t;
  bool do_stage = true;
  static constexpr int P = OPA::NV + OPB::NV;
  template <int PIECE>
  __device__ __forceinline__ void one() {
    if constexpr (PIECE < OPA::NV) {
      if (do_stage) oa.template stage<PIECE>(fa, dstA, left1, t);
      oa.template load<PIECE>(fa, abase, lda, left2, nullptr, t);
    } else {
      constexpr int J = PIECE - OPA::NV;
      if (do_stage) ob.template stage<J>(fb, dstB, left1, t);
      ob.template load<J>(fb, bbase, ldb, left2, bscale, t);
    }
  }
  template <int G, int NG, int... Is>
  __device__ __forceinline__ void group_impl(std::integer_sequence<int, Is...>) {
    ((Is * NG / P == G ? one<Is>() : void()), ...);
  }
  template <int G, int NG>
  __device__ __forceinline__ void group() { group_impl<G, NG>(std::make_integer_sequence<int, P>{}); }
};

template <int WTN, class OPA, class OPB, class PR>
__device__ __forceinline__ void limb_tile_step(const char* __restrict__ As, const char* __restrict__ Bs, const uint32_t (&aaddr)[2],
                                               const uint32_t (&baddr)[WTN], f32x16 (&acc)[2][WTN], PR& pr) {
  constexpr int NH = WTN / 2, NG = 6 * NH;
#define CB_MFMA4(A_, B_, H_, G_)                                                                             \
  _Pragma("unroll") for (int i = 0; i < 2; ++i) _Pragma("unroll") for (int j = 0; j < 2; ++j)               \
      acc[i][2 * H_ + j] = __builtin_amdgcn_mfma_f32_32x32x16_bf16(A_[i], B_[j], acc[i][2 * H_ + j], 0, 0, 0); \
  pr.template group<G_, NG>();
#define CB_HALF(H_)                                                                                                          \
  {                                                                                                                          \
    bf16x8 b_hi[2], b_mid[2], b_lo[2];                                                                                       \
    if (H_ == 0) { _Pragma("unroll") for (int i = 0; i < 2; ++i) a_lo[i] = OPA::frag(As, aaddr[i], 2); }                     \
    _Pragma("unroll") for (int j = 0; j < 2; ++j) b_hi[j] = OPB::frag(Bs, baddr[2 * H_ + j], 0);                             \
    if (H_ == 0) { _Pragma("unroll") for (int i = 0; i < 2; ++i) a_hi[i] = OPA::frag(As, aaddr[i], 0); }                     \
    _Pragma("unroll") for (int j = 0; j < 2; ++j) b_lo[j] = OPB::frag(Bs, baddr[2 * H_ + j], 2);                             \
    if (H_ == 0) { _Pragma("unroll") for (int i = 0; i < 2; ++i) a_mid[i] = OPA::frag(As, aaddr[i], 1); }                    \
    _Pragma("unroll") for (int j = 0; j < 2; ++j) b_mid[j] = OPB::frag(Bs, baddr[2 * H_ + j], 1);                            \
    CB_MFMA4(a_lo, b_hi, H_, H_ * 6 + 0)                                                                                     \
    CB_MFMA4(a_hi, b_lo, H_, H_ * 6 + 1)                                                                                     \
    CB_MFMA4(a_mid, b_mid, H_, H_ * 6 + 2)                                                                                   \
    CB_MFMA4(a_mid, b_hi, H_, H_ * 6 + 3)                                                                                    \
    CB_MFMA4(a_hi, b_mid, H_, H_ * 6 + 4)                                                                                    \
    CB_MFMA4(a_hi, b_hi, H_, H_ * 6 + 5)                                                                                     \
  }
  bf16x8 a_hi[2], a_mid[2], a_lo[2];
  static_assert(NH >= 1 && NH <= 4, "wave tiles of 64, 128 or 256 columns");
  CB_HALF(0)
  if constexpr (NH > 1) CB_HALF(1)
  if constexpr (NH > 2) CB_HALF(2)
  if constexpr (NH > 3) CB_HALF(3)
#undef CB_HALF
#undef CB_MFMA4
}

template <int WTN>
__device__ __forceinline__ void zero_acc_n(f32x16 (&acc)[2][WTN]) {
#pragma unroll
  for (int i = 0; i < 2; ++i)
#pragma unroll
    for (int j = 0; j < WTN; ++j)
#pragma unroll
      for (int e = 0; e < 16; ++e) acc[i][j][e] = 0.f;
}

template <int WTN, int PD, class OA, class OB>
// ... 48 lines not shown
```

### gnn-tail-generalization_amd/gemm.py

```python
import torch

from . import _lib


def _rowmajor(t):
    if t.dim() != 2:
        raise ValueError('expected a matrix')
    if t.shape[1] > 1 and t.stride(1) != 1:
        t = t.contiguous()
    elif t.shape[0] > 1 and t.stride(0) < t.shape[1]:
        t = t.contiguous()
    return t


def _ld(t):
    return t.stride(0) if t.shape[0] > 1 else max(t.shape[1], 1)


def _b_workspace(lib, N, K, M, device):
    wsb = lib.cb_gemm_nn_splitk_workspace_bytes(M, N, K) if K >= 512 else 0
    return (torch.empty(wsb, dtype=torch.uint8, device=device), wsb) if wsb else (None, 0)


def mm_nn(a, b, rowscale=None, addend=None, bias=None, relu=False, out_bf16=False, out=None):
# ... 33 lines not shown
        return None
    out = torch.empty((M, N), dtype=torch.float32, device=a.device)
    if not lib.cb_gemm_nn_store_rows_supported(_lib.ptr(a), _ld(a), _lib.ptr(b), _ld(b), _lib.ptr(out), _ld(out), M, N, K):
        return None
    if addend is not None:
        addend = _rowmajor(addend)
    act = torch.empty_like(out) if want_act else None
    with torch.cuda.device(a.device):
        _lib.check(lib.cb_gemm_nn_store_rows_f32(_lib.ptr(a), _ld(a), _lib.ptr(b), _ld(b), _lib.ptr(out), _ld(out), M, N, K, _lib.ptr(rowscale), _lib.ptr(addend),
                                                 _ld(addend) if addend is not None else 0, _lib.ptr(bias), _lib.ptr(row_index),
                                                 ops.store_args(mix, mix_index, c_act, c_mix, p, seed, row0, bits, relu_only, act), None, 0,
                                                 _lib.stream_ptr()), 'cb_gemm_nn_store_rows_f32')
    return out, act


def mm_nn_drop2(a, b, p, seed, row0=0, bias=None, relu=False):
    import ctypes
    from . import ops
    lib = _lib.load()
    _lib.require_device(a, b, bias)
    a, b = _rowmajor(a), _rowmajor(b)
    M, K = a.shape
    K2, N = b.shape
    if K != K2 or a.dtype != torch.float32 or b.dtype != torch.float32:
        raise ValueError(f'mm_nn_drop2: bad operands {tuple(a.shape)} @ {tuple(b.shape)}')
    y = torch.empty((M, N), dtype=torch.float32, device=a.device)
    yd = torch.empty((M, N), dtype=torch.float32, device=a.device)
    ws, wsb = _b_workspace(lib, N, K, M, a.device)
    with torch.cuda.device(a.device):
        _lib.check(lib.cb_gemm_nn_drop2_f32(_lib.ptr(a), _ld(a), _lib.ptr(b), _ld(b), _lib.ptr(y), N, _lib.ptr(yd), N, M, N, K, None, None, 0,
                                            _lib.ptr(bias), int(bool(relu)), float(p), ctypes.c_uint64(seed), ops.seed_dev_ptr(), int(row0),
                                            _lib.ptr(ws), wsb, _lib.stream_ptr()), 'cb_gemm_nn_drop2_f32')
    return y, yd


def mm_nn_indrop_drop2(a, b, p, a_seed, seed, row0=0, bias=None, relu=False, want_bits=False):
    import ctypes
    from . import ops
    lib = _lib.load()
    _lib.require_device(a, b, bias)
    a, b = _rowmajor(a), _rowmajor(b)
    M, K = a.shape
    K2, N = b.shape
    if K != K2 or a.dtype != torch.float32 or b.dtype != torch.float32 or not (0.0 < p < 1.0):
        return None
    y = torch.empty((M, N), dtype=torch.float32, device=a.device)
    yd = torch.empty((M, N), dtype=torch.float32, device=a.device)
    if not lib.cb_gemm_nn_indrop_supported(_lib.ptr(a), _ld(a), _lib.ptr(b), _ld(b), _lib.ptr(y), N, _lib.ptr(yd), N, M, N, K):
        return None
    bits = torch.empty((M, 1, 4), dtype=torch.int64, device=a.device) if (want_bits and N == 256 and relu) else None
    with torch.cuda.device(a.device):
        _lib.check(lib.cb_gemm_nn_indrop_drop2_f32(_lib.ptr(a), _ld(a), _lib.ptr(b), _ld(b), _lib.ptr(y), N, _lib.ptr(yd), N, M, N, K, _lib.ptr(bias),
                                                   int(bool(relu)), float(p), ctypes.c_uint64(a_seed), float(p), ctypes.c_uint64(seed),
                                                   ops.seed_dev_ptr(), int(row0), _lib.ptr(bits), _lib.stream_ptr()), 'cb_gemm_nn_indrop_drop2_f32')
    return (y, yd, bits) if want_bits else (y, yd)


def mm_nn_indrop(a, b, p, a_seed, row0=0, rowscale=None, addend=None, bias=None, relu=False, want_bits=False, out=None):
    import ctypes
    from . import ops
    lib = _lib.load()
    _lib.require_device(a, b, rowscale, addend, bias, out)
    a, b = _rowmajor(a), _rowmajor(b)
    M, K = a.shape
    K2, N = b.shape
    if K != K2 or a.dtype != torch.float32 or b.dtype != torch.float32 or not (0.0 < p < 1.0):
        return None
    if addend is not None:
        addend = _rowmajor(addend)
        if addend.data_ptr() % 16 or _ld(addend) % 4:
            return None
    y = out if out is not None else torch.empty((M, N), dtype=torch.float32, device=a.device)
    if not lib.cb_gemm_nn_indrop_supported(_lib.ptr(a), _ld(a), _lib.ptr(b), _ld(b), _lib.ptr(y), _ld(y), _lib.ptr(y), _ld(y), M, N, K):
        return None
    bits = torch.empty((M, 1, 4), dtype=torch.int64, device=a.device) if (want_bits and N == 256 and relu) else None
    with torch.cuda.device(a.device):
        _lib.check(lib.cb_gemm_nn_indrop_f32(_lib.ptr(a), _ld(a), _lib.ptr(b), _ld(b), _lib.ptr(y), _ld(y), M, N, K, _lib.ptr(rowscale), _lib.ptr(addend),
                                             _ld(addend) if addend is not None else 0, _lib.ptr(bias), int(bool(relu)), float(p),
                                             ctypes.c_uint64(a_seed), ops.seed_dev_ptr(), int(row0), _lib.ptr(bits), _lib.stream_ptr()),
                   'cb_gemm_nn_indrop_f32')
    return (y, bits) if want_bits else y


def trunk_front(x, w_in, b_in, w0, rowscale, addend, p, seed_x, seed_x0, row0=0, want_bits=False, want_drop=False, z_out=None):
    import ctypes
    from . import ops
    lib = _lib.load()
    _lib.require_device(x, w_in, b_in, w0, rowscale, addend)
    if x.dim() != 2 or x.dtype != torch.float32 or tuple(w_in.shape) != (256, x.shape[1]) or tuple(w0.shape) != (256, 256):
        return None
    M, K = x.shape
    nb_in = lib.cb_front_image_bytes(K)
    if not nb_in or w_in.dtype != torch.float32 or w0.dtype != torch.float32:
        return None
    x, w_in, w0 = _rowmajor(x), _rowmajor(w_in), _rowmajor(w0)
    if addend is not None:
        addend = _rowmajor(addend)
    if x.data_ptr() % 16 or _ld(x) % 4 or (addend is not None and (addend.data_ptr() % 16 or _ld(addend) % 4)):
        return None
    dev = x.device
    img_in = torch.empty(nb_in, dtype=torch.uint8, device=dev)
    nb0 = lib.cb_agg_gemm_image_bytes(256, 256)
    img0 = torch.empty(nb0, dtype=torch.uint8, device=dev)
    x0 = torch.empty((M, 256), dtype=torch.float32, device=dev)
    z0 = z_out if z_out is not None else torch.empty((M, 256), dtype=torch.float32, device=dev)
    bits = torch.empty((M, 1, 4), dtype=torch.int64, device=dev) if want_bits else None
    xd = torch.empty((M, 256), dtype=torch.float32, device=dev) if want_drop else None
    with torch.cuda.device(dev):
        _lib.check(lib.cb_front_image_f32(_lib.ptr(w_in), _ld(w_in), K, 1, _lib.ptr(img_in), nb_in, _lib.stream_ptr()), 'cb_front_image_f32')
        _lib.check(lib.cb_agg_gemm_image_f32(_lib.ptr(w0), _ld(w0), 256, 256, 0, _lib.ptr(img0), nb0, _lib.stream_ptr()), 'cb_agg_gemm_image_f32')
        _lib.check(lib.cb_trunk_front_f32(_lib.ptr(x), _ld(x), M, K, _lib.ptr(img_in), _lib.ptr(b_in), _lib.ptr(img0), _lib.ptr(rowscale),
                                          _lib.ptr(addend), _ld(addend) if addend is not None else 0, _lib.ptr(x0), 256, _lib.ptr(bits),
                                          _lib.ptr(xd), 256, _lib.ptr(z0), 256, float(p), ctypes.c_uint64(seed_x), ctypes.c_uint64(seed_x0),
                                          ops.seed_dev_ptr(), int(row0), _lib.stream_ptr()), 'cb_trunk_front_f32')
    return x0, bits, xd, z0


def mm_tn_adrop(a, g, p, a_seed, row0=0, rowscale=None):
    import ctypes
    from . import ops
    lib = _lib.load()
    _lib.require_device(a, g, rowscale)
    a, g = _rowmajor(a), _rowmajor(g)
    M, K1 = a.shape
    M2, K2 = g.shape
    if M != M2 or not (0.0 < p < 1.0) or not lib.cb_gemm_tn_adrop_supported(_lib.ptr(a), _ld(a), _lib.ptr(g), _ld(g), K1, K2):
        return None
    out = torch.empty((K1, K2), dtype=torch.float32, device=a.device)
    wsb = lib.cb_gemm_tn_workspace_bytes(M, K1, K2)
    ws = torch.empty(max(wsb, 16), dtype=torch.uint8, device=a.device)
    with torch.cuda.device(a.device):
        _lib.check(lib.cb_gemm_tn_adrop_f32(_lib.ptr(a), _ld(a), _lib.ptr(g), _ld(g), _lib.ptr(rowscale), _lib.ptr(out), M, K1, K2, float(p),
                                            ctypes.c_uint64(a_seed), ops.seed_dev_ptr(), int(row0), _lib.ptr(ws), wsb, _lib.stream_ptr()),
                   'cb_gemm_tn_adrop_f32')
    return out


def mm_tn_gdrop(a, g, p, g_seed, row0=0):
    import ctypes
    from . import ops
    lib = _lib.load()
    _lib.require_device(a, g)
    a, g = _rowmajor(a), _rowmajor(g)
    M, K1 = a.shape
    M2, K2 = g.shape
    if M != M2 or not (0.0 < p < 1.0) or not lib.cb_gemm_tn_gdrop_supported(_lib.ptr(a), _ld(a), _lib.ptr(g), _ld(g), K1, K2):
        return None
    out = torch.empty((K1, K2), dtype=torch.float32, device=a.device)
    wsb = lib.cb_gemm_tn_workspace_bytes(M, K1, K2)
    ws = torch.empty(max(wsb, 16), dtype=torch.uint8, device=a.device)
    with torch.cuda.device(a.device):
        _lib.check(lib.cb_gemm_tn_gdrop_f32(_lib.ptr(a), _ld(a), _lib.ptr(g), _ld(g), _lib.ptr(out), M, K1, K2, float(p), ctypes.c_uint64(g_seed),
                                            ops.seed_dev_ptr(), int(row0), _lib.ptr(ws), wsb, _lib.stream_ptr()), 'cb_gemm_tn_gdrop_f32')
    return out


def mm_tn_instage_supported(g_like, x, M):
    lib = _lib.load()
    return (g_like.dim() == 2 and g_like.shape[1] == 256 and g_like.is_contiguous() and x.dim() == 2 and x.stride(1) == 1
            and bool(lib.cb_gemm_tn_instage_supported(_lib.ptr(g_like), _lib.ptr(g_like), _lib.ptr(x), _ld(x), int(M), int(x.shape[1]))))


def mm_tn_instage(g, mfold, x0_bits, x, p_g, g_seed, p_x, x_seed, row0=0):
    import ctypes
    from . import ops
    lib = _lib.load()
    _lib.require_device(g, mfold, x0_bits, x)
    M, K2 = x.shape
    if (tuple(g.shape) != (M, 256) or tuple(mfold.shape) != (M, 256) or not g.is_contiguous() or not mfold.is_contiguous() or x0_bits.numel() != 4 * M
            or not x0_bits.is_contiguous() or x0_bits.dtype != torch.int64):
        raise ValueError('mm_tn_instage: contiguous [M, 256] gradients, [M, 1, 4] int64 mask words and [M, F] features expected')
    out = torch.empty((256, K2), dtype=torch.float32, device=g.device)
    colsum = torch.empty(256, dtype=torch.float32, device=g.device)
    wsb = lib.cb_gemm_tn_instage_workspace_bytes(M, K2)
    ws = torch.empty(max(wsb, 16), dtype=torch.uint8, device=g.device)
    with torch.cuda.device(g.device):
        _lib.check(lib.cb_gemm_tn_instage_f32(_lib.ptr(g), _lib.ptr(mfold), _lib.ptr(x0_bits), _lib.ptr(x), _ld(x), _lib.ptr(out), _lib.ptr(colsum), M, K2,
                                              float(p_g), ctypes.c_uint64(g_seed), float(p_x), ctypes.c_uint64(x_seed), ops.seed_dev_ptr(), int(row0),
                                              _lib.ptr(ws), wsb, _lib.stream_ptr()), 'cb_gemm_tn_instage_f32')
    return out, colsum


def mm_tn(a, g, rowscale=None):
    lib = _lib.load()
    _lib.require_device(a, g, rowscale)
    a, g = _rowmajor(a), _rowmajor(g)
    M, K1 = a.shape
    M2, K2 = g.shape
    if M != M2:
        raise ValueError(f'shape mismatch: {tuple(a.shape)}^T @ {tuple(g.shape)}')
    out = torch.empty((K1, K2), dtype=torch.float32, device=a.device)
    wsb = lib.cb_gemm_tn_workspace_bytes(M, K1, K2)
    ws = torch.empty(max(wsb, 16), dtype=torch.uint8, device=a.device)
    with torch.cuda.device(a.device):
        _lib.check(lib.cb_gemm_tn_f32(_lib.ptr(a), _ld(a), _lib.ptr(g), _ld(g), _lib.ptr(rowscale), _lib.ptr(out), M, K1, K2,
                                      _lib.ptr(ws), wsb, _lib.stream_ptr()), 'cb_gemm_tn_f32')
    return out


class _LinearRowscaleFn(torch.autograd.Function):

    @staticmethod
    def forward(ctx, x, w, rowscale, addend):
        ctx.save_for_backward(x, w, rowscale)
        ctx.has_addend = addend is not None
        return mm_nn(x, w, rowscale=rowscale, addend=addend)

    @staticmethod
    def backward(ctx, g):
        x, w, rowscale = ctx.saved_tensors
        g = _rowmajor(g)
        dx = mm_nn(g, w.t().contiguous(), rowscale=rowscale) if ctx.needs_input_grad[0] else None
        dw = mm_tn(x, g, rowscale=rowscale) if ctx.needs_input_grad[1] else None
        de = g if (ctx.has_addend and ctx.needs_input_grad[3]) else None
        return dx, dw, None, de


def linear_rowscale(x, w, rowscale=None, addend=None):
    return _LinearRowscaleFn.apply(x, w, rowscale, addend)


class _LinearFn(torch.autograd.Function):

    @staticmethod
    def forward(ctx, x, weight, bias, relu):
        y = mm_nn(x, weight.t().contiguous(), bias=bias, relu=relu)
        ctx.relu, ctx.has_bias = relu, bias is not None
        ctx.save_for_backward(x, weight, y if relu else None)
        return y

    @staticmethod
    def backward(ctx, g):
        from .ops import act_bwd
        x, weight, y = ctx.saved_tensors
        need_b = ctx.has_bias and ctx.needs_input_grad[2]
        g = _rowmajor(g)
        if ctx.relu or need_b:
            gm, db = act_bwd(g, y if ctx.relu else None, None, want_out=ctx.relu, want_colsum=need_b)
            if gm is None:
                gm = g
        else:
            gm, db = g, None
        dx = mm_nn(gm, weight) if ctx.needs_input_grad[0] else None
        dw = mm_tn(gm, x) if ctx.needs_input_grad[1] else None
        return dx, dw, db, None


def linear(x, weight, bias=None, relu=False):
    _lib.require_device(x, weight)
    return _LinearFn.apply(x, weight, bias, bool(relu))
```

### gnn-tail-generalization_amd/trunk.py

```python
import ctypes
import os
from typing import NamedTuple

import torch

from . import _lib, gemm, ops
from .graph import head_image, prof_rec, weight_image
from .tuning import T


def _switch(name, default):
    return os.environ.get(name, default)


TrunkCfg = NamedTuple('TrunkCfg', [('L', int), ('alpha', float), ('p', float), ('seeds', tuple), ('agg_bf16', bool), ('track', bool), ('loss_rows', object),
                                   ('residual', bool), ('rows_only', bool)])
TrunkCfg.__doc__ = """What one call of the trunk was asked for (second argument of _TrunkFn.apply).  L: number of GCNConv layers; alpha: weight of the mix
source in a layer's output (res_tricks.py); p: the one dropout rate (0 in evaluation); seeds: L + 2 dropout seeds (features, X0, one per layer); agg_bf16:
the gathered rows Z_l are stored as bf16; track: autograd was recording when the trunk was called (inside a Function's forward it never is, and
needs_input_grad does not know about no_grad); loss_rows: None or (bool mask [N], count), the caller's promise that the output receives gradient in those
rows only (ops.py); residual: the 'Residual' connection (mix source of layer l > 0 = the previous layer's ReLU output) instead of 'Initial' (X0);
rows_only: the second promise — the caller READS the output in the rows of loss_rows only (the others: ops.unread_rows_fill)."""


# ... 355 lines not shown
    out = torch.empty_like(y)
    act = torch.empty_like(y) if want_act else None
    with torch.cuda.device(y.device):
        _lib.check(lib.cb_trunk_store_rows_f32(_lib.ptr(y), _lib.ptr(idx), y.shape[0], y.shape[1],
                                               ops.store_args(mix, mix_index, c_act, c_mix, p, seed, row0, bits, relu_only, act), _lib.ptr(out),
                                               _lib.stream_ptr()), 'cb_trunk_store_rows_f32')
    return out, act


def _layer_on_rows(graph, space, fwd, col_scale, cur, w, b, mix, mix_index, alpha, p, seed, row0, residual, want_act=False, le=None, fwd_le=None):
    fwd.profile = getattr(graph, 'profile', None)
    b_rows = space.norm_in_of(graph)
    bits = torch.empty((graph.N, w.shape[1] // 256, 4), dtype=torch.int64, device=cur.device)
    if (le is None and tuple(w.shape) == (256, 256) and hasattr(fwd, 'spmm_gemm_store_rows') and fwd.E >= T.agg_gemm_store_rows_min_edges
            and agg_gemm_eligible(graph, 256, False)):
        h_agg, x_next, act = fwd.spmm_gemm_store_rows(cur, col_scale, weight_image(w), b_rows, b, space.idx, mix, mix_index, 1 - alpha, alpha, p, seed,
                                                      row0, bits, residual, want_act)
        return bits, x_next, act, h_agg
    h_agg = fwd.spmm(cur, col_scale=col_scale)
    le_sum = None
    if le is not None:
        fwd_le.profile = fwd.profile
        le_sum = fwd_le.spmm(le, row_scale=b_rows)
    fused = gemm.mm_nn_store_rows(h_agg, w, b_rows, le_sum, b, space.idx, mix, mix_index, 1 - alpha, alpha, p, seed, row0, bits, residual, want_act)
    if fused is not None:
        return bits, fused[0], fused[1], h_agg
    y = gemm.mm_nn(h_agg, w, rowscale=b_rows, addend=le_sum, bias=b)
    del le_sum
    x_next, act = _store_rows(y, space.idx, mix, 1 - alpha, alpha, p, seed, row0, bits, residual, mix_index, want_act)
    return bits, x_next, act, h_agg


def _last_layer_on_loss_rows(graph, plan, cur, w, b, mix, alpha, p, seed, row0, residual, w_out, b_out, below=None, le=None):
    sp = plan.space0
    fwd0 = graph.loss_rows_fwd(plan) if below is None else below.fwd0c
    mix_index = None
    if below is not None and residual:
        mix_index = getattr(plan, '_pos0_in_1', None)
        if mix_index is None:
            mix_index = plan._pos0_in_1 = below.s1.pos[sp.idx].long().contiguous()
    bits, x_l, _act, h_agg = _layer_on_rows(graph, sp, fwd0, graph.norm_out if below is None else below.s1.a, cur, w, b, mix, mix_index, alpha, p, seed, row0,
                                           residual, le=le, fwd_le=graph.loss_rows_fwd(plan) if le is not None else None)
    n = graph.N
    logits_c = gemm.mm_nn(x_l, w_out.t().contiguous(), bias=b_out)
    out = ops.expand_unread(logits_c, sp, n)
    graph.rows_only_forwards = getattr(graph, 'rows_only_forwards', 0) + 1
    return bits, x_l, (out, logits_c), h_agg


def _last_layer_on_loss_rows_sharded(graph, s0, orient, cur, w, b, mix, alpha, p, seed, row0, residual, w_out, b_out, le=None):
    lib = _lib.load()
    xs = _exchanged(graph, cur.shape[0], cur.shape[1])
    with torch.cuda.device(cur.device):
        _lib.check(lib.cb_act_bwd_f32(_lib.ptr(cur), None, _lib.ptr(graph.norm_out), _lib.ptr(xs), cur.shape[0], cur.shape[1], None, None, 0,
                                      _lib.stream_ptr()), 'cb_act_bwd_f32')
    h_agg = graph.aggregate_finish(graph.aggregate_start(xs, False, orient=orient), False)
    del xs
    b0 = s0.norm_in_of(graph)
    le_sum = graph.aggregate_finish(graph.aggregate_start(le, False, orient=orient), False, row_scale=b0) if le is not None else None
    y = gemm.mm_nn(h_agg, w, rowscale=b0, addend=le_sum, bias=b)
    del h_agg, le_sum
    n, d = graph.N, w.shape[1]
    bits = torch.empty((n, d // 256, 4), dtype=torch.int64, device=cur.device)
    x_l, _act = _store_rows(y, s0.idx, mix, 1 - alpha, alpha, p, seed, row0, bits, residual)
    del y
    logits_c = gemm.mm_nn(x_l, w_out.t().contiguous(), bias=b_out)
    out = ops.expand_unread(logits_c, s0, n)
    graph.rows_only_forwards += 1
    return bits, x_l, out


class _Forward:

    def __init__(self, ctx, graph, cfg, x, w_in, b_in, w_out, b_out, layer_params):
        self.graph, self.cfg, self.x = graph, cfg, x.contiguous()
        self.w_in, self.b_in, self.w_out, self.b_out = w_in, b_in, w_out, b_out
        self.layer_params, self.layers = layer_params, _layers(layer_params)
        self.row0, self.a = int(getattr(graph, 'row_offset', 0)), graph.norm_out
        self.bwd = bool(cfg.track) and any(ctx.needs_input_grad)
        self.z_ready = self.out_head = self.out_rows = self.h_last = self.h_below = None

    def run(self):
        cfg, graph = self.cfg, self.graph
        (self.xd, self.x0, self.x0_bits, self.cur, self.z_front), self.indrop = self._front()
        h = self.x0.shape[1]
        self.saved_in, self.saved_bits = [self.cur], []
        self.ag = agg_gemm_eligible(graph, h, cfg.agg_bf16)
        self.ro = _rows_only_decision(graph, cfg, self.x, self.x0, h, self.ag, self.bwd, self.layer_params)
        self.mix, self.kw = self.x0, dict(want_bits=self.bwd, relu_only=cfg.residual)
        for l in range(cfg.L):
            self.st = (self.layers[l][1], self.mix, 1 - cfg.alpha, cfg.alpha, cfg.p, cfg.seeds[l + 2] if cfg.p > 0 else 0)
            self.keep_act = cfg.residual and l + 1 < cfg.L
            z0 = self._z0() if l == 0 else None
            bits, self.cur, act = self._form(l, z0 is not None)(l, z0)
            del z0
            if cfg.residual:
                self.mix = act
            if self.bwd:
                self.saved_bits.append(bits)
                self.saved_in.append(self.cur)
        self.mix = None
        return self.out_head if self.out_head is not None else gemm.mm_nn(self.cur, self.w_out.t().contiguous(), bias=self.b_out)

    def _front(self):
        c, x, w_in, b_in, row0, bwd, p, seeds = self.cfg, self.x, self.w_in, self.b_in, self.row0, self.bwd, self.cfg.p, self.cfg.seeds
        indrop = p > 0 and _switch('CB_TRUNK_INDROP', '1') != '0'
        copy = _switch('CB_TRUNK_X0_COPY', '1') == '1'
        if (indrop or p == 0) and not c.agg_bf16 and c.L >= 1 and w_in.shape[0] == 256 and _switch('CB_TRUNK_FRONT', '1') != '0':
            w0, _b0, le0 = self.layers[0]
            fr = gemm.trunk_front(x, w_in, b_in, w0, self.a, le0, p, seeds[0], seeds[1], row0, want_bits=bwd, want_drop=bwd and p > 0 and copy,
                                  z_out=_exchanged(self.graph, x.shape[0]) if hasattr(self.graph, 'part') else None)
            if fr is not None:
                x0, x0_bits, cur, z_front = fr
                return (x, x0, x0_bits, x0 if p == 0 else cur, z_front), True
        if indrop:
            wb = bwd and w_in.shape[0] == 256
            r = None if copy else gemm.mm_nn_indrop(x, w_in.t().contiguous(), p, seeds[0], row0, bias=b_in, relu=True, want_bits=wb)
            if r is not None:
                return (x, *(r if wb else (r, None)), None, None), True
            r = gemm.mm_nn_indrop_drop2(x, w_in.t().contiguous(), p, seeds[0], seeds[1], row0, bias=b_in, relu=True, want_bits=wb)
            if r is not None:
                return (x, r[0], r[2] if len(r) > 2 else None, r[1], None), True
        xd = ops._dropout_raw(x, p, seeds[0], row0 * x.shape[1]) if p > 0 else x
        if p > 0:
            x0, cur = gemm.mm_nn_drop2(xd, w_in.t().contiguous(), p, seeds[1], row0, bias=b_in, relu=True)
        else:
            x0 = cur = gemm.mm_nn(xd, w_in.t().contiguous(), bias=b_in, relu=True)
        return (xd, x0, None, cur, None), False

    def dropped_x0(self):
        return ops._dropout_raw(self.x0, self.cfg.p, self.cfg.seeds[1], self.row0 * self.x0.shape[1])

    def _z0(self):
        z0, self.z_front = self.z_front, None
        if z0 is not None or self.cur is not None:
            return z0
        c, (w, _b, le) = self.cfg, self.layers[0]
        if not (c.agg_bf16 or (not self.ag and _chunked(self.graph, c.agg_bf16))):
            z0 = gemm.mm_nn_indrop(self.x0, w, c.p, c.seeds[1], self.row0, rowscale=self.a, addend=le, out=_exchanged(self.graph, self.x0.shape[0], w.shape[1]))
        if z0 is None:
            self.cur = self.saved_in[0] = self.dropped_x0()
        return z0

    def _form(self, l, have_z0):
        L, ro = self.cfg.L, self.ro
        if self.ag and ro.sum_first_below and l == L - 2:
            return self._form_sum_first_below
        if self.ag and ro.sharded is not None and l == L - 1:
            return self._form_last_on_loss_rows_sharded
        if ro.plan is not None and l == L - 1:
            return self._form_last_on_loss_rows
        if self.ag:
            if ro.sum_first_below and l + 3 == L:
                return self._form_store
            if ro.plan is not None and l + 2 == L and ro.below is not None:
                return self._form_store_on_s1
            if (ro.plan is not None or ro.sharded is not None) and l + 2 == L:
                return self._form_store
            return self._form_store_gemm if l + 1 < L else self._form_store_head
        if not have_z0 and _chunked(self.graph, self.cfg.agg_bf16):
            return self._form_chunked
        return self._form_store

    def _z(self, l, z0):
        z, self.z_ready = self.z_ready, None
        if z is None and z0 is None:
            (w, _b, le), bf = self.layers[l], self.cfg.agg_bf16
            return gemm.mm_nn(self.cur, w, rowscale=self.a, addend=le, out_bf16=bf, out=None if bf else _exchanged(self.graph, self.cur.shape[0], w.shape[1]))
        return z if z is not None else z0

    def _form_sum_first_below(self, l, z0):
        c, below, (w, b, _le) = self.cfg, self.ro.below, self.layers[l]
        bits, cur, act, self.h_below = _layer_on_rows(self.graph, below.s1, below.fwd1, self.a, self.cur, w, b, self.mix, None, c.alpha, c.p,
                                                      self.st[5], self.row0, c.residual, want_act=self.keep_act)
        self.saved_in[l] = None
        return bits, cur, act

    def _form_last_on_loss_rows_sharded(self, l, z0):
        c, (s0, orient), (w, b, le) = self.cfg, self.ro.sharded, self.layers[l]
        bits, cur, self.out_head = _last_layer_on_loss_rows_sharded(self.graph, s0, orient, self.cur, w, b, self.mix, c.alpha, c.p, self.st[5],
                                                                    self.row0, c.residual, self.w_out, self.b_out, le=le)
        return bits, cur, None

    def _form_last_on_loss_rows(self, l, z0):
        c, (w, b, le) = self.cfg, self.layers[l]
        bits, cur, (self.out_head, self.out_rows), self.h_last = _last_layer_on_loss_rows(
            self.graph, self.ro.plan, self.cur, w, b, self.mix, c.alpha, c.p, self.st[5], self.row0, c.residual, self.w_out, self.b_out,
            below=self.ro.below, le=le)
        if le is None:
            self.saved_in[l] = None
        else:
            self.h_last = None
        return bits, cur, None

    def _form_store(self, l, z0):
        return _fused_spmm(self.graph, self._z(l, z0), *self.st, want_act=self.keep_act, **self.kw)

    def _form_store_on_s1(self, l, z0):
        below, z = self.ro.below, self._z(l, z0)
        below.fwd1.profile = getattr(self.graph, 'profile', None)
        return _fused_launch(_lib.load(), self.graph, below.fwd1, z, None, *self.st, self.keep_act, row_ids=below.ids1, row_scale=below.b1, **self.kw)

    def _form_store_gemm(self, l, z0):
        w1, _, le1 = self.layers[l + 1]
        res = _fused_gemm(self.graph, self._z(l, z0), *self.st, weight_image(w1), self.a, le1, want_act=self.keep_act, **self.kw)
        self.z_ready = res[2]
        return res[0], res[1], res[3] if self.keep_act else None

    def _form_store_head(self, l, z0):
        z = self._z(l, z0)
        himg = head_image(self.w_out) if head_tail_enabled(self.bwd) else None
        if himg is None:
            return _fused_spmm(self.graph, z, *self.st, **self.kw)
        bits, cur, self.out_head = _fused_gemm(self.graph, z, *self.st, himg, None, None, head=(self.b_out, self.w_out.shape[0]), **self.kw)[:3]
        return bits, cur, None

    def _form_chunked(self, l, z0):
        (w, _b, le), cur, a = self.layers[l], self.cur, self.a
        z = _exchanged(self.graph, cur.shape[0], w.shape[1])

        def produce(k, r0, r1):
            if r1 > r0:
                gemm.mm_nn(cur[r0:r1], w, rowscale=a[r0:r1], addend=le[r0:r1] if le is not None else None, out=z[r0:r1])
        return _fused_spmm(self.graph, z, *self.st, want_act=self.keep_act, produce=produce, **self.kw)


class _TrunkFn(torch.autograd.Function):
    @staticmethod
    def forward(ctx, graph, cfg, x, w_in, b_in, w_out, b_out, *layer_params):
        f = _Forward(ctx, graph, cfg, x, w_in, b_in, w_out, b_out, layer_params)
        out = f.run()
        ctx.graph, ctx.cfg, ctx.row0, ctx.indrop, ctx.n_layer_params = graph, cfg, f.row0, f.indrop, len(layer_params)
        if f.bwd:
            _save(ctx, xd=f.xd, x0=f.x0, w_in=w_in, w_out=w_out, saved_in=f.saved_in, saved_bits=f.saved_bits, layer_params=layer_params,
                  h_last=f.h_last, h_below=f.h_below, x0_bits=f.x0_bits)
            ro = f.ro
            ctx.saved_rows = SavedRows('S0' if (ro.plan is not None or ro.sharded is not None) else 'all',
                                       'absent' if f.h_last is not None else 'S1' if (ro.plan is not None and ro.below is not None) else 'all')
        ctx.set_materialize_grads(False)
        return out, f.out_rows

    @staticmethod
    def backward(ctx, gout, gout_rows=None):
        if gout is None and gout_rows is None:
            return (None,) * (7 + ctx.n_layer_params)
        return _Backward(ctx, gout, gout_rows).run()


class _Carry:
    __slots__ = ('g', 'gr', 'dbias', 'handle', 'space', 'g_above', 'deferred')

    def __init__(self, g, gr, dbias, handle, space):
        self.g, self.gr, self.dbias, self.handle, self.space, self.g_above, self.deferred = g, gr, dbias, handle, space, None, None


class _Backward:

    def __init__(self, ctx, gout, gout_rows=None):
        self.gout_rows = gemm._rowmajor(gout_rows) if gout_rows is not None else None
        self.ctx, graph, c = ctx, ctx.graph, ctx.cfg
        self.graph, self.row0, self.L, self.alpha, self.p, self.seeds = graph, ctx.row0, c.L, c.alpha, c.p, c.seeds
        self.agg_bf16, self.residual = c.agg_bf16, c.residual
        sv = _saved(ctx)
        self.xd, self.x0, self.w_in, self.w_out = sv['xd'], sv['x0'], sv['w_in'], sv['w_out']
        self.saved_in, self.saved_bits, self.x0_bits = sv['saved_in'], sv['saved_bits'], sv['x0_bits']
        self.h_last, self.h_below = sv['h_last'], sv['h_below']
        self.lp, self.where = _layers(sv['layer_params']), ctx.saved_rows
        self.a, self.bnorm = graph.norm_out, graph.norm_in
        self.need = ctx.needs_input_grad
        self.gout = gemm._rowmajor(gout) if gout is not None else None
        self.n_rows, self.h = self.x0.shape
        self.sharded, loss_rows = hasattr(graph, 'part'), c.loss_rows
        if loss_rows is not None and self.where.x_last != 'S0' and (not ops.loss_rows_enabled() or loss_rows[0].shape[0] != self.x0.shape[0]):
            loss_rows = None
        self.loss_rows = loss_rows
        self.gather = _gather(graph, c.L, c.residual, self.x0)
        self.gx0 = None if self.gather else torch.empty_like(self.x0)
        self.g_mix, self.seeds_mix, self.mix_pos = [], [], []
        self.cs = []
        self.grads_layers = [None] * (3 * c.L)
        self.ag = agg_gemm_eligible(graph, self.h, c.agg_bf16)
        self.chunked = (self.gather and _chunked(graph, c.agg_bf16) and graph.b.plan.n_slices > 1 and not self.ag)
        self.fold_ok = (_switch('CB_INSTAGE_FOLD', '1') != '0' and self.gather and not c.residual and not c.agg_bf16 and c.p > 0
                        and ctx.indrop and self.need[3] and not self.need[2] and self.x0_bits is not None and self.h == 256
                        and gemm.mm_tn_instage_supported(self.x0, self.xd, self.x0.shape[0]))
        self.mfold, self.plan_taken = None, False

    def seed(self, i):
        return self.seeds[i] if self.p > 0 else 0

    def need_w(self, l):
        return self.need[7 + 3 * l]

    def need_b(self, l):
        return self.need[7 + 3 * l + 1]

    def need_le(self, l):
        return self.lp[l][2] is not None and self.need[7 + 3 * l + 2]

    def _dw(self, l, x_in, gz):
        if x_in is not None:
            return gemm.mm_tn(x_in, gz, rowscale=self.a)
        return _dw_regen(self.x0, gz, self.p, self.seed(1), self.row0, self.a)

    def _second(self, below, g_above, pos_above=None):
        if not self.residual or g_above is None:
            return {}
        return dict(g2=g_above, seed2=self.seed(below + 3), c2=self.alpha, **({'g2_pos': pos_above} if pos_above is not None else {}))

    def _dx_and_store_bwd(self, src, wt, rowscale, below, g_ready=None, g_above=None, orient=None, pos_above=None):
        p, alpha, row0, bnorm = self.p, self.alpha, self.row0, self.bnorm
        sd, want_b, bits = self.seed(below + 2), self.need_b(below), self.saved_bits[below]
        if self.chunked:
            g_ = torch.empty((src.shape[0], wt.shape[1]), dtype=torch.float32, device=src.device)
            gr_ = _exchanged(self.graph, g_.shape[0], g_.shape[1])
            colsums = []
            sec = self._second(below, g_above, pos_above)

            def produce(k, r0, r1):
                if r1 <= r0:
                    return
                gemm.mm_nn(src[r0:r1], wt, rowscale=rowscale[r0:r1] if rowscale is not None else None, out=g_[r0:r1])
                sec_k = dict(sec, g2=sec['g2'][r0:r1]) if sec else {}
                _, cs = _layer_bwd(g_[r0:r1], bits[r0:r1], bnorm[r0:r1], None, False, p, sd, row0 + r0, 1 - alpha, alpha, want_b, out=gr_[r0:r1], **sec_k)
                if want_b:
                    colsums.append(cs)
            h_ = self.graph.aggregate_start(gr_, True, produce=produce, orient=orient)
            db_ = None
            if want_b:
                db_ = (torch.zeros(wt.shape[1], dtype=torch.float32, device=src.device) if not colsums
                       else colsums[0] if len(colsums) == 1 else torch.stack(colsums).sum(0))
            return g_, gr_, db_, h_
        g_ = g_ready if g_ready is not None else gemm.mm_nn(src, wt, rowscale=rowscale)
        cs_ = self.cs
        if (below == 0 and self.fold_ok and self.mfold is None and self.plan_taken and len(self.g_mix) <= 2 and len(cs_) <= 1
                and all(t.is_contiguous() for t in self.g_mix) and g_.is_contiguous()):
            res = _layer_bwd_fold(g_, bits, bnorm, p, sd, row0, 1 - alpha, alpha, want_b, self.g_mix, self.mix_pos, self.seeds_mix,
                                  out=_exchanged(self.graph, g_.shape[0], g_.shape[1]) if self.sharded else None, cs=cs_[0][:3] if cs_ else None)
            gr_, db_, self.mfold = res[:3]
            if cs_:
                self.grads_layers[3 * cs_[0][3] + 1] = res[3]
                self.cs = []
            self.g_mix, self.mix_pos, self.seeds_mix = [], [], []
            return None, gr_, db_, None
        gr_, db_ = _layer_bwd(g_, bits, bnorm, self.gx0, below != self.L - 1, p, sd, row0, 1 - alpha, alpha, want_b, out_bf16=self.agg_bf16,
                              out=_exchanged(self.graph, g_.shape[0], g_.shape[1]) if (self.sharded and not self.agg_bf16) else None,
                              **self._second(below, g_above, pos_above))
        return g_, gr_, db_, None

    def _head(self, space):
        L, need, gout, xl = self.L, self.need, self.gout, self.saved_in[self.L]
        if space is not None:
            gout = ops.gather_rows_by_index(gout, space.idx) if gout is not None else None
            if self.gout_rows is not None:
                gout = self.gout_rows if gout is None else gout + self.gout_rows
            xl = xl if self.where.x_last == 'S0' else ops.gather_rows_by_index(xl, space.idx)
        self.d_w_out = gemm.mm_tn(gout, xl) if need[5] else None
        self.d_b_out = ops.act_bwd(gout, None, None, want_out=False, want_colsum=True)[1] if need[6] else None
        if space is None:
            return _Carry(*self._dx_and_store_bwd(gout, self.w_out, None, L - 1, orient=self._orient_of(L - 1)), None)
        g = gemm.mm_nn(gout, self.w_out)
        gr, dbias = _layer_bwd_rows(g, space.idx, self.saved_bits[L - 1], self.bnorm, self.p, self.seed(L + 1), self.row0, 1 - self.alpha,
                                    self.need_b(L - 1), out=_exchanged(self.graph, g.shape[0], g.shape[1]) if self.sharded else None)
        return _Carry(g, gr, dbias, None, space)

    def _sh_level(self, layer):
        j = self.L - 1 - layer
        return self.sh_levels[j] if 0 <= j < len(self.sh_levels) else None

    def _orient_of(self, layer):
        return getattr(self._sh_level(layer), 'orient', None)

    def _dw_rows(self, l, x_in, gz, dst):
        if dst is None:
            return self._dw(l, x_in, gz)
        return gemm.mm_tn(ops.gather_rows_by_index(x_in, dst.idx), gz, rowscale=dst.a)

    def _layer_source_side(self, l, gr, level, fwd_j):
        w = self.lp[l][0]
        dst = level[1]
        level[0].profile = getattr(self.graph, 'profile', None)
        if fwd_j is not None:
            fwd_j.profile = level[0].profile
        t = gemm.mm_nn(gr, w.t().contiguous())
        fused = None
# ... 1 lines not shown
                and hasattr(level[0], 'spmm_store_bwd') and t.shape[1] % 256 == 0):
            fold = self.fold_ok and l == 1 and len(self.g_mix) <= 2 and all(q is not None for q in self.mix_pos) and not self.cs
            if fold:
                self.mfold, gr_below, db0 = level[0].spmm_store_bwd(t, self.a, self.saved_bits[0], self.bnorm, 1 - self.alpha, self.p, self.seed(2), self.row0,
                                                                    mix=(self.g_mix, self.mix_pos, self.seeds_mix, self.alpha, self.need_b(0)))
                self.grads_layers[1] = db0
                self.g_mix, self.mix_pos, self.seeds_mix = [], [], []
                g_new = None
            else:
                g_new, gr_below = level[0].spmm_store_bwd(t, self.a, self.saved_bits[l - 1], self.bnorm, 1 - self.alpha, self.p, self.seed(l + 1), self.row0)
            fused = (gr_below, l - 1)
        else:
            g_new = level[0].spmm(t, row_scale=dst.a if dst is not None else self.a)
        del t
        if self.need_w(l):
            x_agg = (self.h_last if (self.where.x_below == 'absent' and l == self.L - 1) else self.h_below if (self.h_below is not None and l == self.L - 2)
                     else fwd_j.spmm(self.saved_in[l], col_scale=self.a))
            self.grads_layers[3 * l] = gemm.mm_tn(x_agg, gr)
        return None, g_new, fused

    def _layer_compact(self, l, gr, level):
        w = self.lp[l][0]
        dst = level[1]
        level[0].profile = getattr(self.graph, 'profile', None)
        gz, g_new = level[0].spmm_gemm(gr, weight_image(w, transpose=True), transpose=False, g_rowscale=dst.a if dst is not None else self.a)
        if self.need_w(l):
            if dst is not None:
                on_s1 = self.where.x_below == 'S1' and l == self.L - 1
                x_rows = self.saved_in[l] if on_s1 else ops.gather_rows_by_index(self.saved_in[l], dst.idx)
                self.grads_layers[3 * l] = gemm.mm_tn(x_rows, gz, rowscale=dst.a)
            else:
                self.grads_layers[3 * l] = self._dw(l, self.saved_in[l], gz)
        return gz, g_new

    def _layer_fused(self, l, gr, handle, dst=None):
        graph = self.graph
        a = dst.a if dst is not None else self.a
        img = weight_image(self.lp[l][0], transpose=True)

        def tail(csr, src, acc, tr):
            csr.profile = getattr(graph, 'profile', None)
            return csr.spmm_gemm(src, img, transpose=tr, g_rowscale=a, acc_init=acc)
        return (graph.aggregate_finish(handle, True, last_pass=lambda csr, recv, acc: tail(csr, recv, acc, False)) if self.sharded
                else tail(graph, gr, None, True))

    def _layer_plain(self, gr, handle):
        return self.graph.aggregate_finish(handle, True) if self.sharded else _spmm_t(self.graph, gr)

    def _resolve_plan(self):
        graph, L, gout, xl_compact = self.graph, self.L, self.gout, self.where.x_last == 'S0'
        self.sh_levels = []
        if self.gout_rows is not None and not xl_compact:
            raise RuntimeError('gradient for the compact loss-row logits, but the forward did not run rows-only')
        if self.sharded and hasattr(graph, 'support_levels') and self.loss_rows is not None:
            ops.check_rows_zero(gout, self.loss_rows[0])
            self.sh_levels = graph.support_levels(self.loss_rows[0], L, compact=self.ag and self.gather, cumulative=self.residual)
        plan = None
        hint = None if self.sharded else _support_plan(graph, self.loss_rows, self.n_rows, L, self.residual, self.h, self.x0, committed=xl_compact)
        if hint is not None:
            if gout is not None:
                ops.check_rows_zero(gout, hint[0])
            plan = graph.grad_support_plan(hint[0], L, max_frac=T.rowsparse_max_frac, cumulative=self.residual, count=not xl_compact)
        self.plan_taken = plan is not None or bool(self.sh_levels)
        if self.where.x_below == 'absent' and plan is None:
            raise RuntimeError('the forward evaluated its last layer on the loss rows (rows_only), but its backward finds no row-support plan: '
                               'CB_LOSS_ROWS / tuning.T / the mask changed between the forward and the backward')
        space0 = plan.space0 if plan is not None else (self.sh_levels[0].src if self.sh_levels else None)
        if xl_compact and space0 is None:
            raise RuntimeError('the forward evaluated its last layer on the loss rows (rows_only), but its backward has no compact level 0')
        return plan, space0

    def _layer(self, l, c, plan):
        L, graph, sharded = self.L, self.graph, self.sharded
        j = L - 1 - l
        level = plan.levels[j] if (plan is not None and j < len(plan.levels)) else None
        lv = self._sh_level(l)
        dst = level[1] if level is not None else lv.dst if lv is not None else None
        if sharded and c.handle is None:
            c.handle = graph.aggregate_start(c.gr, True, orient=self._orient_of(l))
        if c.deferred is not None:
            self.grads_layers[3 * c.deferred[0]] = self._dw_rows(*c.deferred)
            c.deferred = None
        fwd_j = plan.fwd[j] if (level is not None and j < len(plan.fwd)) else None
        source_side = ((self.where.x_below == 'absent' and l == L - 1) or (self.h_below is not None and l == L - 2)
                       or (T.rowsparse_loss_side and fwd_j is not None and not self.need_le(l)
                           and not (self.need_w(l) and self.saved_in[l] is None)
                           and not (self.where.x_below == 'S1' and l == L - 1)))
        if source_side:
            _gz, g_new, fused = self._layer_source_side(l, c.gr, level, fwd_j)
            return None, g_new, dst, fused
        if level is not None:
            return (*self._layer_compact(l, c.gr, level), dst, None)
        gz, g_new = self._layer_fused(l, c.gr, c.handle, dst) if self.ag else (self._layer_plain(c.gr, c.handle), None)
        if self.need_w(l):
            if sharded:
                c.deferred = (l, self.saved_in[l], gz, dst if self.ag else None)
            else:
                self.grads_layers[3 * l] = self._dw(l, self.saved_in[l], gz)
        return gz, g_new, dst, None

    def _store_bwd_below(self, l, c, gz, g_new, dst, fused, pos_above):
        w = self.lp[l][0]
        if l > 0 and fused is not None:
            c.g, (c.gr, _below), c.dbias = g_new, fused, None
            if self.mfold is not None:
                c.dbias = self.grads_layers[3 * (l - 1) + 1]
            elif self.need_b(l - 1):
                self.cs = self.cs + [(len(self.g_mix), self.saved_bits[l - 1], 1 - self.alpha, l - 1)]
        elif l > 0 and dst is not None:
            c.g = g_new
            c.gr, c.dbias = _layer_bwd_rows(g_new, dst.idx, self.saved_bits[l - 1], self.bnorm, self.p, self.seed(l + 1), self.row0, 1 - self.alpha,
                                            self.need_b(l - 1), out=_exchanged(self.graph, g_new.shape[0], g_new.shape[1]) if self.sharded else None,
                                            **self._second(l - 1, c.g_above, pos_above))
        elif l > 0:
            c.g, c.gr, c.dbias, c.handle = self._dx_and_store_bwd(gz, w.t().contiguous(), self.a, l - 1, g_new, c.g_above, orient=self._orient_of(l - 1),
                                                                  pos_above=pos_above)
        else:
            c.g = g_new if g_new is not None else gemm.mm_nn(gz, w.t().contiguous(), rowscale=self.a)

    def run(self):
        plan, space0 = self._resolve_plan()
        c = self._head(space0)
        for l in range(self.L - 1, -1, -1):
            if self.gather and (not self.residual or l == 0) and self.mfold is None:
                self.g_mix.append(c.g)
                self.mix_pos.append(c.space.pos if c.space is not None else None)
                self.seeds_mix.append(self.seed(l + 2))
            gz, g_new, dst, fused = self._layer(l, c, plan)
            c.g_above = c.g if self.residual else None
            pos_above = c.space.pos if (self.residual and c.space is not None) else None
            c.g = c.gr = c.handle = None
            self.grads_layers[3 * l + 1] = c.dbias
            c.space = dst
            self._store_bwd_below(l, c, gz, g_new, dst, fused, pos_above)
            c.g_above = None
            if self.need_le(l):
                if dst is not None:
                    gz = ops.expand_rows(gz, dst.pos)
                self.grads_layers[3 * l + 2] = gz
            del gz, g_new
        if c.deferred is not None:
            self.grads_layers[3 * c.deferred[0]] = self._dw_rows(*c.deferred)
        return self._input_stage(c)

    def _input_stage(self, c):
        graph, p, need, xd, row0 = self.graph, self.p, self.need, self.xd, self.row0
        g, c.g = c.g, None
        if self.mfold is not None:
            d_w_in, d_b_in = gemm.mm_tn_instage(g, self.mfold, self.x0_bits, xd, p, self.seed(1), p, self.seeds[0], row0)
            del g
            self.gx0 = self.g_mix = self.mfold = None
            graph.instage_folds = getattr(graph, 'instage_folds', 0) + 1
            return (None, None, None, d_w_in, d_b_in if need[4] else None, self.d_w_out, self.d_b_out, *self.grads_layers)
        if self.gather:
            res = _input_bwd_multi(g, self.seed(1), self.g_mix, self.seeds_mix, self.alpha, self.x0, p, row0, act_bits=self.x0_bits,
                                   mix_pos=self.mix_pos, cs=[q[:3] for q in self.cs])
            gpre, d_b_in = res[0], res[1]
            for q, db in zip(self.cs, res[2] if self.cs else []):
                self.grads_layers[3 * q[3] + 1] = db
        else:
            gpre, d_b_in = _input_bwd(g, self.gx0, self.x0, p, self.seed(1), row0)
        del g
        self.gx0 = self.g_mix = None
        d_w_in = None
        if need[3]:
            if self.ctx.indrop and p > 0:
                d_w_in = gemm.mm_tn_gdrop(gpre, xd, p, self.seeds[0], row0)
                if d_w_in is None:
                    d_w_in = gemm.mm_tn(gpre, ops._dropout_raw(xd, p, self.seeds[0], row0 * xd.shape[1]))
            else:
                d_w_in = gemm.mm_tn(gpre, xd)
        d_x = None
        if need[2]:
            d_x = gemm.mm_nn(gpre, self.w_in)
            if p > 0:
                d_x = ops._dropout_raw(d_x, p, self.seeds[0], row0 * d_x.shape[1])
        return (None, None, d_x, d_w_in, d_b_in if need[4] else None, self.d_w_out, self.d_b_out, *self.grads_layers)


def forward(tc, x, graph, loss_rows=None, rows_only=False):
    L = tc.num_layers
    p = float(tc.dropout) if tc.training else 0.0
    seeds = tuple(ops.next_seed() for _ in range(L + 2)) if p > 0 else (0,) * (L + 2)
    params, se_reg_all = _collect_layer_params(tc, graph)
    agg_bf16 = getattr(tc.args, 'agg_dtype', 'f32') == 'bf16'
    if loss_rows is not None:
        mask, count = loss_rows if isinstance(loss_rows, (tuple, list)) else (loss_rows, None)
        if count is None:
            count = int(mask.sum().item())
        if mask.dtype != torch.bool or mask.dim() != 1 or mask.shape[0] != x.shape[0]:
            raise ValueError(f'loss_rows: a bool mask over the {x.shape[0]} rows expected, got {tuple(mask.shape)} {mask.dtype}')
        loss_rows = (mask, int(count))
    cfg = TrunkCfg(L, float(tc.alpha), p, seeds, agg_bf16, torch.is_grad_enabled(), loss_rows, connection(tc) == 'residual',
                   bool(rows_only) and loss_rows is not None)
    out, out_rows = _TrunkFn.apply(graph, cfg, x, tc.layers_MLP[0].weight, tc.layers_MLP[0].bias, tc.layers_MLP[1].weight, tc.layers_MLP[1].bias, *params)
    if out_rows is not None:
        out._cb_rows = (out_rows, loss_rows[0])
    return out, se_reg_all
```

### include/coldbrew_hip.h

```cpp
#ifndef COLDBREW_HIP_H
#define COLDBREW_HIP_H

#include <stddef.h>
#include <stdint.h>

#ifdef __cplusplus
extern "C" {
#endif

#define CB_OK 0
#define CB_E_INVALID (-1)
#define CB_E_RANGE (-2)
#define CB_E_WORKSPACE (-3)
#define CB_E_HIP (-4)
#define CB_E_DEVICE (-5)

#define CB_DEVERR_HANDOVER 1
#define CB_DEVERR_GRADROWS 2

int cb_version(void);
const char* cb_last_error(void);
int cb_device_status(void);

int cb_rows_zero_outside_mask_f32(const float* g, int64_t ld, int64_t rows, int64_t d, const uint8_t* mask, int32_t* guard, void* stream);
// ... 91 lines not shown
                                const uint64_t* cs_bits, float cs_c, float* colsum2, void* ws2, size_t ws2_bytes, void* stream);
int cb_trunk_layer_bwd_rows_f32(const float* g, const int64_t* row_index, int64_t n_rows, const uint64_t* relu_bits, const float* row_scale, float* out,
                                int64_t d, float drop_p, uint64_t seed, const uint64_t* seed_dev, int64_t row0, float c_act, const float* g2, uint64_t seed2,
                                float c2, const int32_t* g2_pos, float* colsum, void* ws, size_t ws_bytes, void* stream);

int cb_trunk_input_bwd_f32(const float* g, const float* add, const float* act, float* out, int64_t rows, int64_t d, float drop_p,
                           uint64_t seed, const uint64_t* seed_dev, int64_t row0, float* colsum, void* ws, size_t ws_bytes,
                           void* stream);

int cb_trunk_input_bwd_multi_f32(const float* g, uint64_t seed, int32_t n_mix, const float* const* g_mix, const uint64_t* seeds_mix,
                                 float c_mix, const float* act, float* out, int64_t rows, int64_t d, float drop_p,
                                 const uint64_t* seed_dev, int64_t row0, float* colsum, void* ws, size_t ws_bytes,
                                 const uint64_t* act_bits, const int32_t* const* g_mix_pos, void* stream);
int cb_trunk_input_bwd_multi_cs_f32(const float* g, uint64_t seed, int32_t n_mix, const float* const* g_mix, const uint64_t* seeds_mix,
                                    float c_mix, const float* act, float* out, int64_t rows, int64_t d, float drop_p,
                                    const uint64_t* seed_dev, int64_t row0, float* colsum, void* ws, size_t ws_bytes,
                                    const uint64_t* act_bits, const int32_t* const* g_mix_pos, int32_t n_cs, const int32_t* cs_src,
                                    const uint64_t* const* cs_bits, const float* cs_c, float* const* colsum2, void* ws2, size_t ws2_bytes, void* stream);
int cb_spmm_csr_store_bwd_f32(const cb_csr_view* g, const float* h, int64_t ld_h, int64_t d, const float* row_scale, const uint64_t* relu_bits,
                              const float* bwd_rowscale, float c_act, float drop_p, uint64_t seed, const uint64_t* seed_dev, int64_t row0,
                              float* out_g, int64_t ld_g, float* out_gr, int64_t ld_gr, void* stream);
size_t cb_spmm_store_bwd_mix_workspace_bytes(int64_t N, int64_t n_hubs, int64_t d);
int cb_spmm_csr_store_bwd_mix_f32(const cb_csr_view* g, const float* h, int64_t ld_h, int64_t d, const float* row_scale, const uint64_t* relu_bits,
                                  const float* bwd_rowscale, float c_act, float drop_p, uint64_t seed, const uint64_t* seed_dev, int64_t row0,
                                  float* out_m, int64_t ld_m, float* out_gr, int64_t ld_gr, int32_t n_mix, const float* const* mix_g,
                                  const int32_t* const* mix_pos, const uint64_t* mix_seeds, float c_mix, float* colsum, void* ws2, size_t ws2_bytes,
                                  void* stream);

int cb_gemm_nn_bf16out_f32(const float* A, int64_t lda, const float* B, int64_t ldb, uint16_t* C, int64_t ldc, int64_t M, int64_t N,
                           int64_t K, const float* rowscale, const float* addend, int64_t ld_add, const float* bias, int relu,
                           void* ws, size_t ws_bytes, void* stream);

int cb_node_norm_fwd_f32(const float* x, float* y, float* stats2, int64_t rows, int64_t d, float c, float q, float eps, void* stream);
int cb_node_norm_bwd_f32(const float* x, const float* g, const float* stats2, float* dx, int64_t rows, int64_t d, float c, float q,
                         void* stream);
size_t cb_colstats_workspace_bytes(int64_t rows, int64_t d);
int cb_colstats_f32(const float* x, const float* w, const float* shift, int64_t rows, int64_t d, float* colsum, float* colsum2,
                    void* ws, size_t ws_bytes, void* stream);
int cb_col_affine_f32(const float* x, const float* shift, const float* scale, const float* bias, float gscale, float* y, int64_t rows,
                      int64_t d, void* stream);
int cb_col_bwd_combine_f32(const float* g, const float* xh, const float* xs, const float* a, const float* b, const float* e, float ga,
                           float gb, float* dx, int64_t rows, int64_t d, void* stream);

size_t cb_topk_replace_workspace_bytes(int64_t B, int64_t N, int64_t K);
int cb_topk_replace_f32(const float* q, int64_t ldq, const float* t, int64_t ldt, int64_t B, int64_t N, int64_t D, int32_t K,
                        float* out, int32_t* out_idx, float* out_w, void* ws, size_t ws_bytes, void* stream);

int cb_id_count_i64(const int64_t* ids, int64_t E, int64_t N, int32_t* counts, int32_t* n_bad, void* stream);
int cb_value_hist_i32(const int32_t* vals, int64_t N, int32_t n_bins, int32_t* hist, int32_t* n_bad, void* stream);
size_t cb_compact_workspace_bytes(int64_t n);
int cb_select_range_i32(const int32_t* vals, int64_t N, int32_t lo, int32_t hi, int64_t* out_idx, uint8_t* out_mask, int64_t* count,
                        void* ws, size_t ws_bytes, void* stream);
int cb_craft_isolation_i64(const int64_t* src, const int64_t* dst, int64_t E, const uint8_t* node_flag, int64_t N, int64_t* out_src,
                           int64_t* out_dst, int64_t* count, void* ws, size_t ws_bytes, void* stream);
size_t cb_symmetrize_workspace_bytes(int64_t E, int64_t N);
int cb_symmetrize_i64(const int64_t* src, const int64_t* dst, int64_t E, int64_t N, int64_t* out_row, int64_t* out_col, int64_t* count,
                      int32_t* n_bad, void* ws, size_t ws_bytes, void* stream);

int cb_gather_rows_f32(const float* src, int64_t ld, const int64_t* idx, int64_t n_idx, int64_t d, float* out, void* stream);

size_t cb_agg_gemm_image_bytes(int64_t K, int64_t N);
int cb_agg_gemm_image_f32(const float* W, int64_t ld, int64_t K, int64_t N, int transpose, void* image, size_t image_bytes, void* stream);
int cb_spmm_gemm_f32(const cb_csr_view* g, const float* h, int64_t ld_h, int64_t d, const float* row_scale, const float* bias, int relu,
                     const float* acc_init, int64_t ld_init, float* out, int64_t ld_out, const void* image, const float* g_rowscale,
                     const float* g_addend, int64_t ld_add, float* g_out, int64_t ld_gout, void* stream);
int cb_spmm_gemm_fused_f32(const cb_csr_view* g, const float* acc_init, int64_t ld_init, const float* h, int64_t ld_h, int64_t d,
                           const float* row_scale, const float* bias, const cb_trunk_store* store, float* out_next, int64_t ld_next,
                           int32_t skip_next, const void* image, const float* g_rowscale, const float* g_addend, int64_t ld_add, float* g_out,
                           int64_t ld_gout, void* stream);
size_t cb_agg_gemm_head_image_bytes(int64_t K, int64_t C);
int cb_agg_gemm_head_image_f32(const float* W, int64_t ld, int64_t K, int64_t C, int transpose, void* image, size_t image_bytes, void* stream);
int cb_spmm_gemm_fused_head_f32(const cb_csr_view* g, const float* acc_init, int64_t ld_init, const float* h, int64_t ld_h, int64_t d,
                                const float* row_scale, const float* bias, const cb_trunk_store* store, float* out_next, int64_t ld_next,
                                int32_t skip_next, const void* head_image, const float* head_bias, int64_t C, float* logits, int64_t ld_logits,
                                void* stream);
int cb_agg_gemm_handover_selftest(void* stream);

size_t cb_front_image_bytes(int64_t K);
int cb_front_image_f32(const float* W, int64_t ld, int64_t K, int transpose, void* image, size_t image_bytes, void* stream);
int cb_trunk_front_f32(const float* x, int64_t ld_x, int64_t M, int64_t K, const void* image_in, const float* bias_in, const void* image_0,
                       const float* rowscale, const float* addend, int64_t ld_add, float* x0, int64_t ld_x0, uint64_t* relu_bits, float* x0_drop,
                       int64_t ld_drop, float* z0, int64_t ld_z, float drop_p, uint64_t seed_x, uint64_t seed_x0, const uint64_t* seed_dev,
                       int64_t row0, void* stream);

int cb_spmm_csr_weighted_f32(const int32_t* rowptr, const int32_t* col, const float* w, int64_t N, int64_t E, const float* h, int64_t ld_h,
                             int64_t d, const float* row_scale, const float* bias, int relu, float* out, int64_t ld_out, void* stream);
int cb_spmm_edge_dot_f32(const int32_t* rowptr, const int32_t* col, int64_t N, int64_t E, const float* h, int64_t ld_h, const float* g,
                         int64_t ld_g, int64_t d, float* dw, void* stream);

int cb_gemm_nn_indrop_supported(const float* A, int64_t lda, const float* B, int64_t ldb, const float* C, int64_t ldc, const float* C2, int64_t ldc2,
                                int64_t M, int64_t N, int64_t K);
int cb_gemm_nn_indrop_drop2_f32(const float* A, int64_t lda, const float* B, int64_t ldb, float* C, int64_t ldc, float* C2, int64_t ldc2,
                                int64_t M, int64_t N, int64_t K, const float* bias, int relu, float a_drop_p, uint64_t a_seed, float drop_p,
                                uint64_t seed, const uint64_t* seed_dev, int64_t row0, uint64_t* relu_bits, void* stream);
int cb_gemm_nn_indrop_f32(const float* A, int64_t lda, const float* B, int64_t ldb, float* C, int64_t ldc, int64_t M, int64_t N, int64_t K,
                          const float* rowscale, const float* addend, int64_t ld_add, const float* bias, int relu, float a_drop_p, uint64_t a_seed,
                          const uint64_t* seed_dev, int64_t row0, uint64_t* relu_bits, void* stream);
int cb_gemm_tn_adrop_supported(const float* A, int64_t lda, const float* G, int64_t ldg, int64_t K1, int64_t K2);
int cb_gemm_tn_adrop_f32(const float* A, int64_t lda, const float* G, int64_t ldg, const float* rowscale, float* C, int64_t M, int64_t K1, int64_t K2,
                         float a_drop_p, uint64_t a_seed, const uint64_t* seed_dev, int64_t row0, void* ws, size_t ws_bytes, void* stream);
int cb_gemm_tn_gdrop_supported(const float* A, int64_t lda, const float* G, int64_t ldg, int64_t K1, int64_t K2);
int cb_gemm_tn_gdrop_f32(const float* A, int64_t lda, const float* G, int64_t ldg, float* C, int64_t M, int64_t K1, int64_t K2, float g_drop_p,
                         uint64_t g_seed, const uint64_t* seed_dev, int64_t row0, void* ws, size_t ws_bytes, void* stream);
int cb_gemm_tn_instage_supported(const float* g, const float* mfold, const float* X, int64_t ldx, int64_t M, int64_t K2);
size_t cb_gemm_tn_instage_workspace_bytes(int64_t M, int64_t K2);
int cb_gemm_tn_instage_f32(const float* g, const float* mfold, const uint64_t* x0_bits, const float* X, int64_t ldx, float* C, float* colsum, int64_t M, int64_t K2,
                           float g_drop_p, uint64_t g_seed, float x_drop_p, uint64_t x_seed, const uint64_t* seed_dev, int64_t row0, void* ws, size_t ws_bytes,
                           void* stream);

int cb_spmm_gemm_store_rows_f32(const cb_csr_view* g, const float* h, int64_t ld_h, int64_t d, const float* col_scale, float* out, int64_t ld_out,
                                const void* image, const float* g_rowscale, const float* bias, const int64_t* row_ids, const cb_trunk_store* store,
                                float* g_out, int64_t ld_gout, void* stream);

int cb_spmm_csr_lp_f32(const cb_csr_view* g, const float* h, int64_t ld_h, int64_t d, const float* row_scale, const float* mix, int64_t ld_mix,
                       float c_mix, const float* post_scale, float* out, int64_t ld_out, void* stream);

int cb_spmm_csr_prop_f32(const cb_csr_view* g, const float* h, int64_t ld_h, int64_t d, const float* row_scale, const float* mix, int64_t ld_mix,
                         float c_mix, float lo, float hi, const uint8_t* fix_rows, const float* post_scale, float* out, int64_t ld_out,
                         void* stream);

size_t cb_cs_workspace_bytes(int64_t N, int64_t Cp);
int cb_cs_residual_init_f32(const float* P, int64_t ld_p, const int64_t* labels, const uint8_t* label_rows, int64_t N, int64_t C, int64_t Cp,
                            const float* state_scale, float* E0, float* state, float* abs_sum, void* ws, size_t ws_bytes, void* stream);
int cb_cs_correct_snap_f32(int32_t mode, const float* P, int64_t ld_p, const float* resid, int64_t ld_r, const int64_t* labels,
                           const uint8_t* label_rows, int64_t N, int64_t C, int64_t Cp, const float* abs_sum, int64_t n_label, float scale,
                           const float* state_scale, float* res_result, int64_t ld_res, float* y2, float* state, void* stream);

int cb_gather_rows_bf16_f32(const float* src, int64_t ld, const int64_t* idx, int64_t n_idx, int64_t d, uint16_t* out, void* stream);
int cb_expand_rows_f32(const float* src, const int32_t* pos, int64_t n_rows, int64_t d, float fill, float* out, void* stream);
int cb_trunk_store_rows_f32(const float* y, const int64_t* row_index, int64_t n_rows, int64_t d, const cb_trunk_store* store, float* out, void* stream);
int cb_gemm_nn_store_rows_supported(const float* A, int64_t lda, const float* B, int64_t ldb, const float* C, int64_t ldc, int64_t M, int64_t N, int64_t K);
int cb_gemm_nn_store_rows_f32(const float* A, int64_t lda, const float* B, int64_t ldb, float* C, int64_t ldc, int64_t M, int64_t N, int64_t K,
                              const float* rowscale, const float* addend, int64_t ld_add, const float* bias, const int64_t* row_index,
                              const cb_trunk_store* store, void* ws, size_t ws_bytes, void* stream);


int cb_ln_gelu_drop_fwd_f32(const float* z, int64_t rows, int64_t d, const float* gamma, const float* beta, float eps, float p,
                            uint64_t seed, const uint64_t* seed_dev, float* out, float* stats, void* stream);
size_t cb_ln_gelu_drop_bwd_workspace_bytes(int64_t rows, int64_t d);
int cb_ln_gelu_drop_bwd_f32(const float* dy, const float* z, const float* stats, int64_t rows, int64_t d, const float* gamma,
                            const float* beta, float p, uint64_t seed, const uint64_t* seed_dev, float* dz, float* dgamma,
                            float* dbeta, float* dbias, void* ws, size_t ws_bytes, void* stream);

int cb_mse_rows_f32(const float* pred, int64_t B, int64_t D, const float* target, int64_t ld_t, int64_t n_target_rows,
                    const int64_t* row_index, float* loss, float* grad, void* ws, size_t ws_bytes, void* stream);

int cb_part2_assemble_f32(const float* x, int64_t F, const float* replaced, const float* part1_out, int64_t D, const float* alphas,
                          int64_t B, float* out, void* stream);
int cb_part2_assemble_bwd_f32(const float* g, int64_t F, const float* replaced, const float* part1_out, int64_t D, int64_t B,
                              float* dalphas, void* ws, size_t ws_bytes, void* stream);


int cb_ncloss_positions_i64(const int64_t* batch_idx, int64_t B, int64_t n, int32_t* pos, int32_t* rep, void* stream);

int cb_ncloss_row_norms_f32(const float* x, int64_t ldx, int64_t rows, int64_t D, float* nrm, float* rinv, void* stream);

int cb_cosine_scale_f32(float* s, int64_t ld, int64_t N, const float* nrm, void* stream);

int cb_ncloss_uses_limb_core(const float* z, int64_t ldz, int64_t D);

size_t cb_ncloss_workspace_bytes(int64_t B, int32_t max_splits);
int cb_ncloss_fwd_f32(const float* z, int64_t ldz, int64_t B, int64_t D, float tau, const int32_t* rowptr, const int32_t* col,
                      const float* val, int64_t n, const int64_t* batch_idx, const int32_t* pos, const int32_t* rep, int32_t max_splits,
                      float* rinv, float* num, float* den, float* w, float* u, float* loss, int32_t* m_count, void* ws, size_t ws_bytes,
                      void* stream);

int cb_ncloss_normalize_rows_f32(const float* z, int64_t ldz, int64_t B, int64_t D, const float* rinv, float* zhat, void* stream);
int cb_ncloss_bwd_slab_f32(const float* z, int64_t ldz, int64_t B, int64_t D, float tau, const float* rinv, const float* w, int64_t row0,
                           int64_t rows, int32_t max_splits, float* P, int64_t ldp, void* stream);
int cb_ncloss_bwd_finish_f32(const float* z, int64_t ldz, const float* zhat, int64_t B, int64_t D, float tau, const float* rinv, const float* u,
                             const int32_t* rowptr, const int32_t* col, const float* val, const int32_t* rowptr_t, const int32_t* col_t,
                             const float* val_t, int64_t n, const int64_t* batch_idx, const int32_t* pos, const int32_t* rep, const float* g,
                             float* dzh, float* dz, void* stream);


size_t cb_spgemm_offsets_workspace_bytes(int64_t nnz_a);
int cb_spgemm_entry_offsets_i64(const int32_t* col_a, int64_t nnz_a, const int32_t* rowptr_b, int64_t k, int64_t* ent_off, int32_t* n_bad,
                                void* ws, size_t ws_bytes, void* stream);

size_t cb_spgemm_chunk_workspace_bytes(int64_t n_products);
int cb_spgemm_chunk_count_f32(const int32_t* rowptr_a, const int32_t* col_a, const float* val_a, const int32_t* rowptr_b, const int32_t* col_b,
                              const float* val_b, const int64_t* ent_off, int64_t row0, int64_t row1, int64_t k, int64_t n_cols,
                              int64_t n_products, int64_t* count, void* ws, size_t ws_bytes, void* stream);

int cb_spgemm_chunk_emit_f32(const void* ws, size_t ws_bytes, int64_t row0, int64_t row1, int64_t n_cols, int64_t n_products, int64_t count,
                             int64_t nnz_base, int32_t* rowptr, int32_t* col_out, float* val_out, void* stream);

size_t cb_csr_transpose_workspace_bytes(int64_t nnz);
int cb_csr_transpose_f32(const int32_t* rowptr, const int32_t* col, const float* val, int64_t m, int64_t n, int64_t nnz, int32_t* rowptr_t,
                         int32_t* col_t, float* val_t, void* ws, size_t ws_bytes, void* stream);

// ... 110 lines not shown
```

Before: 9.620.

## Save dropout keep-mask words in front kernel and reuse them in backward GEMMs

The fused front kernel can now write packed dropout keep-mask words for x and x0 to small buffers. The backward weight-gradient GEMMs (input-stage and layer-0 TN) read these words instead of regenerating Philox random numbers or reading a materialized dropped-x0 copy. When residual is off, the dropped-x0 copy is skipped entirely. This trades some extra memory traffic and storage for the mask words against less RNG recomputation and less bandwidth spent on the dropped copy. A new path also materializes dropped x0 lazily where a form still needs it.

```diff
diff --git a/gnn-tail-generalization_amd/_lib.py b/gnn-tail-generalization_amd/_lib.py
--- a/gnn-tail-generalization_amd/_lib.py
+++ b/gnn-tail-generalization_amd/_lib.py
@@ -105,6 +105,12 @@
     'cb_front_image_f32': (ctypes.c_int, [_P, _I64, _I64, ctypes.c_int, _P, _SZ, _P]),
     'cb_trunk_front_f32': (ctypes.c_int, [_P, _I64, _I64, _I64, _P, _P, _P, _P, _P, _I64, _P, _I64, _P, _P, _I64, _P, _I64, ctypes.c_float,
                                           ctypes.c_uint64, ctypes.c_uint64, _P, _I64, _P]),
+    'cb_front_keep_x0_bytes': (_SZ, [_I64]),
+    'cb_front_keep_x_bytes': (_SZ, [_I64]),
+    'cb_trunk_front_words_f32': (ctypes.c_int, [_P, _I64, _I64, _I64, _P, _P, _P, _P, _P, _I64, _P, _I64, _P, _P, _I64, _P, _I64, ctypes.c_float,
+                                                ctypes.c_uint64, ctypes.c_uint64, _P, _I64, _P, _P, _P]),
+    'cb_gemm_tn_awords_supported': (ctypes.c_int, [_P, _I64, _P, _I64, _I64, _I64]),
+    'cb_gemm_tn_awords_f32': (ctypes.c_int, [_P, _I64, _P, ctypes.c_float, _P, _I64, _P, _P, _I64, _I64, _I64, _P, _SZ, _P]),
     'cb_gemm_tn_gdrop_supported': (ctypes.c_int, [_P, _I64, _P, _I64, _I64, _I64]),
     'cb_gemm_tn_gdrop_f32': (ctypes.c_int, [_P, _I64, _P, _I64, _P, _I64, _I64, _I64, ctypes.c_float, ctypes.c_uint64, _P, _I64, _P, _SZ, _P]),
     'cb_spmm_csr_lp_f32': (ctypes.c_int, [_G, _P, _I64, _I64, _P, _P, _I64, ctypes.c_float, _P, _P, _I64, _P]),
@@ -124,6 +130,8 @@
     'cb_gemm_tn_instage_workspace_bytes': (_SZ, [_I64, _I64]),
     'cb_gemm_tn_instage_f32': (ctypes.c_int, [_P, _P, _P, _P, _I64, _P, _P, _I64, _I64, ctypes.c_float, ctypes.c_uint64, ctypes.c_float, ctypes.c_uint64, _P, _I64,
                                               _P, _SZ, _P]),
+    'cb_gemm_tn_instage_words_supported': (ctypes.c_int, [_P, _P, _P, _I64, _I64, _I64]),
+    'cb_gemm_tn_instage_words_f32': (ctypes.c_int, [_P, _P, _P, _P, _I64, _P, _P, _I64, _I64, ctypes.c_float, ctypes.c_float, _P, _P, _P, _SZ, _P]),
     'cb_trunk_layer_bwd_fold_f32': (ctypes.c_int, [_P, _P, _P, _P, _I64, _I64, ctypes.c_float, ctypes.c_uint64, _P, _I64, ctypes.c_float, ctypes.c_float, _I32, _P, _P, _P,
                                                    _P, _P, _P, _SZ, _I32, _P, ctypes.c_float, _P, _P, _SZ, _P]),
     'cb_trunk_layer_bwd_rows_f32': (ctypes.c_int, [_P, _P, _I64, _P, _P, _P, _I64, ctypes.c_float, ctypes.c_uint64, _P, _I64, ctypes.c_float,
diff --git a/gnn-tail-generalization_amd/csrc/cb_front.hip b/gnn-tail-generalization_amd/csrc/cb_front.hip
--- a/gnn-tail-generalization_amd/csrc/cb_front.hip
+++ b/gnn-tail-generalization_amd/csrc/cb_front.hip
@@ -31,9 +31,11 @@
   const uint64_t* seed_dev;
   int64_t row0;
   int n_tiles;
+  unsigned long long* keep_x0;
+  uint32_t* keep_x;
 };
 
-template <int NS1, bool DROP>
+template <int NS1, bool DROP, bool WORDS = false>
 __global__ void __launch_bounds__(256, 2) k_front(FrontArgs fa) {
   constexpr int K1 = 16 * NS1, LDX = K1 + 4, NV = kTM * K1 / 4 / 256;
   static_assert(NV >= 1 && kTM * LDX <= kTM * kTLD, "x tile must fit the region of the X0 tile");
@@ -108,6 +110,9 @@
       }
       *reinterpret_cast<float4*>(tile + row * LDX + 4 * c4) = make_float4(v[0], v[1], v[2], v[3]);
     }
+    if constexpr (WORDS && NV == 8) {
+      if (fa.keep_x) fa.keep_x[(int64_t)tile_id * 256 + t] = kx;
+    }
     if constexpr (DROP) aim_x(tile_id + (int)gridDim.x);
     if (t < kTM) rs_tile[par][t] = rs_next;
     __syncthreads();
@@ -125,6 +130,9 @@
             tile[(32 * i + (reg & 3) + 8 * (reg >> 2) + 4 * lh) * kTLD + 64 * w + 32 * j + l31] = acc[i][j][reg];
     }
     __syncthreads();
+    if constexpr (WORDS) {
+      if (fa.keep_x0) fa.keep_x0[((int64_t)tile_id * 4 + w) * 64 + lane] = k3;
+    }
 #pragma unroll 4
     for (int r = 0; r < 16; ++r) {
       const int row = 16 * w + r;
@@ -199,34 +207,60 @@
   return CB_OK;
 }
 
-extern "C" int cb_trunk_front_f32(const float* x, int64_t ld_x, int64_t M, int64_t K, const void* image_in, const float* bias_in, const void* image_0,
-                                  const float* rowscale, const float* addend, int64_t ld_add, float* x0, int64_t ld_x0, uint64_t* relu_bits,
-                                  float* x0_drop, int64_t ld_drop, float* z0, int64_t ld_z, float drop_p, uint64_t seed_x, uint64_t seed_x0,
-                                  const uint64_t* seed_dev, int64_t row0, void* stream) {
+static int trunk_front(const char* fn, const float* x, int64_t ld_x, int64_t M, int64_t K, const void* image_in, const float* bias_in, const void* image_0,
+                       const float* rowscale, const float* addend, int64_t ld_add, float* x0, int64_t ld_x0, uint64_t* relu_bits, float* x0_drop,
+                       int64_t ld_drop, float* z0, int64_t ld_z, float drop_p, uint64_t seed_x, uint64_t seed_x0, const uint64_t* seed_dev, int64_t row0,
+                       uint64_t* keep_x0, uint32_t* keep_x, void* stream) {
   CB_CHECK_ARG(M >= 0 && cb_front_image_bytes(K) > 0 && drop_p >= 0.f && drop_p < 1.f && row0 >= 0, CB_E_INVALID,
-               "cb_trunk_front_f32: bad size (K must be 64 or 128; hidden width 256) or p");
-  CB_CHECK_ARG(M < ((int64_t)1 << 31) * kTM / 2, CB_E_RANGE, "cb_trunk_front_f32: size out of range");
+               "%s: bad size (K must be 64 or 128; hidden width 256) or p", fn);
+  CB_CHECK_ARG(M < ((int64_t)1 << 31) * kTM / 2, CB_E_RANGE, "%s: size out of range", fn);
+  CB_CHECK_ARG((!keep_x0 && !keep_x) || drop_p > 0.f, CB_E_INVALID, "%s: keep words exist with p > 0 only", fn);
+  CB_CHECK_ARG(!keep_x || K == 128, CB_E_INVALID, "%s: the keep words of x exist for K = 128 only", fn);
   if (M == 0) return CB_OK;
-  CB_CHECK_ARG(x && image_in && image_0 && x0 && z0, CB_E_INVALID, "cb_trunk_front_f32: null pointer");
+  CB_CHECK_ARG(x && image_in && image_0 && x0 && z0, CB_E_INVALID, "%s: null pointer", fn);
   CB_CHECK_ARG(aligned16(x) && ld_x % 4 == 0 && ld_x >= K && aligned16(image_in) && aligned16(image_0) && aligned16(x0) && ld_x0 % 4 == 0 && ld_x0 >= kND &&
                    aligned16(z0) && ld_z % 4 == 0 && ld_z >= kND && (!addend || (aligned16(addend) && ld_add % 4 == 0 && ld_add >= kND)) &&
-                   (!x0_drop || (aligned16(x0_drop) && ld_drop % 4 == 0 && ld_drop >= kND)) && (!relu_bits || (uintptr_t)relu_bits % 8 == 0),
-               CB_E_INVALID, "cb_trunk_front_f32: 16-byte aligned rows required");
+                   (!x0_drop || (aligned16(x0_drop) && ld_drop % 4 == 0 && ld_drop >= kND)) && (!relu_bits || (uintptr_t)relu_bits % 8 == 0) &&
+                   (uintptr_t)keep_x0 % 8 == 0 && (uintptr_t)keep_x % 4 == 0,
+               CB_E_INVALID, "%s: 16-byte aligned rows required", fn);
   FrontArgs fa{x, ld_x, (const uint4*)image_in, bias_in, (const uint4*)image_0, rowscale, addend, ld_add, x0, ld_x0, (unsigned long long*)relu_bits,
                x0_drop, ld_drop, z0, ld_z, M};
   fa.thresh = drop_p > 0.f ? dropout_threshold(drop_p) : 0u;
   fa.keep_scale = 1.f / (1.f - drop_p);
   fa.seed_x = seed_x; fa.seed_x0 = seed_x0; fa.seed_dev = seed_dev; fa.row0 = row0;
   fa.n_tiles = (int)((M + kTM - 1) / kTM);
+  fa.keep_x0 = (unsigned long long*)keep_x0; fa.keep_x = keep_x;
   int dev = 0, n_cu = 0;
   if (hipGetDevice(&dev) != hipSuccess || hipDeviceGetAttribute(&n_cu, hipDeviceAttributeMultiprocessorCount, dev) != hipSuccess || n_cu <= 0) n_cu = 256;
   const int blocks = fa.n_tiles < 2 * n_cu ? fa.n_tiles : 2 * n_cu;
   const dim3 grid((unsigned)blocks), blk(256);
   hipStream_t st = (hipStream_t)stream;
-  if (K == 64 && fa.thresh) hipLaunchKernelGGL((k_front<4, true>), grid, blk, 0, st, fa);
+  const bool words = keep_x0 || keep_x;
+  if (K == 64 && words) hipLaunchKernelGGL((k_front<4, true, true>), grid, blk, 0, st, fa);
+  else if (words) hipLaunchKernelGGL((k_front<8, true, true>), grid, blk, 0, st, fa);
+  else if (K == 64 && fa.thresh) hipLaunchKernelGGL((k_front<4, true>), grid, blk, 0, st, fa);
   else if (K == 64) hipLaunchKernelGGL((k_front<4, false>), grid, blk, 0, st, fa);
   else if (fa.thresh) hipLaunchKernelGGL((k_front<8, true>), grid, blk, 0, st, fa);
   else hipLaunchKernelGGL((k_front<8, false>), grid, blk, 0, st, fa);
   CB_LAUNCH_CHECK();
   return CB_OK;
 }
+
+extern "C" int cb_trunk_front_f32(const float* x, int64_t ld_x, int64_t M, int64_t K, const void* image_in, const float* bias_in, const void* image_0,
+                                  const float* rowscale, const float* addend, int64_t ld_add, float* x0, int64_t ld_x0, uint64_t* relu_bits,
+                                  float* x0_drop, int64_t ld_drop, float* z0, int64_t ld_z, float drop_p, uint64_t seed_x, uint64_t seed_x0,
+                                  const uint64_t* seed_dev, int64_t row0, void* stream) {
+  return trunk_front("cb_trunk_front_f32", x, ld_x, M, K, image_in, bias_in, image_0, rowscale, addend, ld_add, x0, ld_x0, relu_bits, x0_drop, ld_drop, z0, ld_z,
+                     drop_p, seed_x, seed_x0, seed_dev, row0, nullptr, nullptr, stream);
+}
+
+extern "C" size_t cb_front_keep_x0_bytes(int64_t M) { return M > 0 ? (size_t)((M + kTM - 1) / kTM) * 4 * 64 * sizeof(uint64_t) : 0; }
+extern "C" size_t cb_front_keep_x_bytes(int64_t M) { return M > 0 ? (size_t)((M + kTM - 1) / kTM) * 256 * sizeof(uint32_t) : 0; }
+
+extern "C" int cb_trunk_front_words_f32(const float* x, int64_t ld_x, int64_t M, int64_t K, const void* image_in, const float* bias_in, const void* image_0,
+                                        const float* rowscale, const float* addend, int64_t ld_add, float* x0, int64_t ld_x0, uint64_t* relu_bits,
+                                        float* x0_drop, int64_t ld_drop, float* z0, int64_t ld_z, float drop_p, uint64_t seed_x, uint64_t seed_x0,
+                                        const uint64_t* seed_dev, int64_t row0, uint64_t* keep_x0, uint32_t* keep_x, void* stream) {
+  return trunk_front("cb_trunk_front_words_f32", x, ld_x, M, K, image_in, bias_in, image_0, rowscale, addend, ld_add, x0, ld_x0, relu_bits, x0_drop, ld_drop, z0,
+                     ld_z, drop_p, seed_x, seed_x0, seed_dev, row0, keep_x0, keep_x, stream);
+}
diff --git a/gnn-tail-generalization_amd/csrc/cb_gemm.hip b/gnn-tail-generalization_amd/csrc/cb_gemm.hip
--- a/gnn-tail-generalization_amd/csrc/cb_gemm.hip
+++ b/gnn-tail-generalization_amd/csrc/cb_gemm.hip
@@ -408,6 +408,33 @@
   return launch_tn<2, 2>(A, lda, G, ldg, nullptr, C, M, K1, K2, (float*)ws, st, &gd);
 }
 
+extern "C" int cb_gemm_tn_awords_supported(const float* A, int64_t lda, const float* G, int64_t ldg, int64_t K1, int64_t K2) {
+  return limb3_on() && K1 == 256 && K2 == 256 && limb3_tn_eligible(A, lda, G, ldg, K1, K2) ? 1 : 0;
+}
+
+extern "C" int cb_gemm_tn_awords_f32(const float* A, int64_t lda, const uint64_t* keep_x0, float drop_p, const float* G, int64_t ldg, const float* rowscale, float* C,
+                                     int64_t M, int64_t K1, int64_t K2, void* ws, size_t ws_bytes, void* stream) {
+  CB_CHECK_ARG(M >= 0 && drop_p > 0.f && drop_p < 1.f, CB_E_INVALID, "cb_gemm_tn_awords_f32: bad size or p");
+  CB_CHECK_ARG(C && (M == 0 || (A && G && keep_x0)) && lda >= K1 && ldg >= K2 && (uintptr_t)keep_x0 % 8 == 0, CB_E_INVALID,
+               "cb_gemm_tn_awords_f32: null / misaligned pointer or bad ld");
+  CB_CHECK_ARG(cb_gemm_tn_awords_supported(A, lda, G, ldg, K1, K2), CB_E_INVALID, "cb_gemm_tn_awords_f32: shape / alignment outside the words form (cb_gemm_tn_awords_supported)");
+  hipStream_t st = (hipStream_t)stream;
+  if (M == 0) {
+    CB_HIP(hipMemsetAsync(C, 0, (size_t)K1 * K2 * sizeof(float), st));
+    return CB_OK;
+  }
+  CB_CHECK_ARG(ws && ws_bytes >= cb_gemm_tn_workspace_bytes(M, K1, K2), CB_E_WORKSPACE, "cb_gemm_tn_awords_f32: workspace too small");
+  const int nsplit = tn_splits(M, 4);
+  int64_t rows_per_split = (M + nsplit - 1) / nsplit;
+  rows_per_split = (rows_per_split + 31) / 32 * 32;
+  const int rc = launch_tn_x0words(A, lda, keep_x0, 1.f / (1.f - drop_p), G, ldg, rowscale, (float*)ws, M, nsplit, rows_per_split, st);
+  if (rc != CB_OK) return rc;
+  const int64_t n = K1 * K2;
+  hipLaunchKernelGGL(k_sum_partials, dim3((unsigned)((n + 255) / 256)), dim3(256), 0, st, (const float*)ws, nsplit, n, C);
+  CB_LAUNCH_CHECK();
+  return CB_OK;
+}
+
 static inline int instage_splits(int64_t M) { return tn_splits(M, 2); }
 
 extern "C" int cb_gemm_tn_instage_supported(const float* g, const float* mfold, const float* X, int64_t ldx, int64_t M, int64_t K2) {
@@ -422,14 +449,14 @@
   return (size_t)instage_splits(M) * (size_t)256 * (size_t)(K2 + 1) * sizeof(float);
 }
 
-extern "C" int cb_gemm_tn_instage_f32(const float* g, const float* mfold, const uint64_t* x0_bits, const float* X, int64_t ldx, float* C, float* colsum, int64_t M,
-                                      int64_t K2, float g_drop_p, uint64_t g_seed, float x_drop_p, uint64_t x_seed, const uint64_t* seed_dev, int64_t row0, void* ws,
-                                      size_t ws_bytes, void* stream) {
+static int tn_instage(const char* fn, const float* g, const float* mfold, const uint64_t* x0_bits, const float* X, int64_t ldx, float* C, float* colsum, int64_t M,
+                      int64_t K2, float g_drop_p, uint64_t g_seed, float x_drop_p, uint64_t x_seed, const uint64_t* seed_dev, int64_t row0, const uint64_t* keep_x0,
+                      const uint32_t* keep_x, void* ws, size_t ws_bytes, void* stream) {
   CB_CHECK_ARG(M > 0 && K2 > 0 && g_drop_p > 0.f && g_drop_p < 1.f && x_drop_p > 0.f && x_drop_p < 1.f && row0 >= 0, CB_E_INVALID,
-               "cb_gemm_tn_instage_f32: bad size or p (both dropouts must be active)");
-  CB_CHECK_ARG(g && mfold && x0_bits && X && C && colsum && (uintptr_t)x0_bits % 8 == 0, CB_E_INVALID, "cb_gemm_tn_instage_f32: null or misaligned pointer");
-  CB_CHECK_ARG(cb_gemm_tn_instage_supported(g, mfold, X, ldx, M, K2), CB_E_INVALID, "cb_gemm_tn_instage_f32: shape / alignment outside the fused form (cb_gemm_tn_instage_supported)");
-  CB_CHECK_ARG(ws && ws_bytes >= cb_gemm_tn_instage_workspace_bytes(M, K2), CB_E_WORKSPACE, "cb_gemm_tn_instage_f32: workspace too small");
+               "%s: bad size or p (both dropouts must be active)", fn);
+  CB_CHECK_ARG(g && mfold && x0_bits && X && C && colsum && (uintptr_t)x0_bits % 8 == 0, CB_E_INVALID, "%s: null or misaligned pointer", fn);
+  CB_CHECK_ARG(cb_gemm_tn_instage_supported(g, mfold, X, ldx, M, K2), CB_E_INVALID, "%s: shape / alignment outside the fused form (cb_gemm_tn_instage_supported)", fn);
+  CB_CHECK_ARG(ws && ws_bytes >= cb_gemm_tn_instage_workspace_bytes(M, K2), CB_E_WORKSPACE, "%s: workspace too small", fn);
   hipStream_t st = (hipStream_t)stream;
   const int nsplit = instage_splits(M);
   int64_t rows_per_split = (M + nsplit - 1) / nsplit;
@@ -438,7 +465,7 @@
   const DropSpec gd{dropout_threshold(g_drop_p), 1.f / (1.f - g_drop_p), g_seed, seed_dev, row0, 256};
   float* partial = (float*)ws;
   float* cs_partial = partial + (size_t)nsplit * 256 * K2;
-  const int rc = launch_tn_instage(g, mfold, x0_bits, X, ldx, partial, cs_partial, M, K2, nsplit, rows_per_split, st, xd, gd);
+  const int rc = launch_tn_instage(g, mfold, x0_bits, X, ldx, partial, cs_partial, M, K2, nsplit, rows_per_split, st, xd, gd, keep_x0, keep_x);
   if (rc != CB_OK) return rc;
   const int64_t n = 256 * K2;
   hipLaunchKernelGGL(k_sum_partials, dim3((unsigned)((n + 255) / 256)), dim3(256), 0, st, (const float*)partial, nsplit, n, C);
@@ -446,6 +473,27 @@
   hipLaunchKernelGGL(k_sum_partials, dim3(1), dim3(256), 0, st, (const float*)cs_partial, nsplit, (int64_t)256, colsum);
   CB_LAUNCH_CHECK();
   return CB_OK;
+}
+
+extern "C" int cb_gemm_tn_instage_f32(const float* g, const float* mfold, const uint64_t* x0_bits, const float* X, int64_t ldx, float* C, float* colsum, int64_t M,
+                                      int64_t K2, float g_drop_p, uint64_t g_seed, float x_drop_p, uint64_t x_seed, const uint64_t* seed_dev, int64_t row0, void* ws,
+                                      size_t ws_bytes, void* stream) {
+  return tn_instage("cb_gemm_tn_instage_f32", g, mfold, x0_bits, X, ldx, C, colsum, M, K2, g_drop_p, g_seed, x_drop_p, x_seed, seed_dev, row0, nullptr, nullptr, ws,
+                    ws_bytes, stream);
+}
+
+extern "C" int cb_gemm_tn_instage_words_supported(const float* g, const float* mfold, const float* X, int64_t ldx, int64_t M, int64_t K2) {
+  return K2 == 128 && cb_gemm_tn_instage_supported(g, mfold, X, ldx, M, K2) ? 1 : 0;
+}
+
+extern "C" int cb_gemm_tn_instage_words_f32(const float* g, const float* mfold, const uint64_t* x0_bits, const float* X, int64_t ldx, float* C, float* colsum,
+                                            int64_t M, int64_t K2, float g_drop_p, float x_drop_p, const uint64_t* keep_x0, const uint32_t* keep_x, void* ws,
+                                            size_t ws_bytes, void* stream) {
+  CB_CHECK_ARG(keep_x0 && keep_x && (uintptr_t)keep_x0 % 8 == 0 && (uintptr_t)keep_x % 4 == 0, CB_E_INVALID, "cb_gemm_tn_instage_words_f32: null or misaligned keep words");
+  CB_CHECK_ARG(cb_gemm_tn_instage_words_supported(g, mfold, X, ldx, M, K2), CB_E_INVALID,
+               "cb_gemm_tn_instage_words_f32: shape / alignment outside the words form (cb_gemm_tn_instage_words_supported)");
+  return tn_instage("cb_gemm_tn_instage_words_f32", g, mfold, x0_bits, X, ldx, C, colsum, M, K2, g_drop_p, 0ull, x_drop_p, 0ull, nullptr, 0, keep_x0, keep_x, ws,
+                    ws_bytes, stream);
 }
 
 extern "C" int cb_gemm_nn_indrop_f32(const float* A, int64_t lda, const float* B, int64_t ldb, float* C, int64_t ldc, int64_t M, int64_t N, int64_t K,
diff --git a/gnn-tail-generalization_amd/csrc/cb_gemm_limb.h b/gnn-tail-generalization_amd/csrc/cb_gemm_limb.h
--- a/gnn-tail-generalization_amd/csrc/cb_gemm_limb.h
+++ b/gnn-tail-generalization_amd/csrc/cb_gemm_limb.h
@@ -15,7 +15,11 @@
                     int64_t K1, int64_t K2, int bm, int nsplit, int64_t rows_per_split, hipStream_t st, const DropSpec* gdrop = nullptr,
                     const DropSpec* adrop = nullptr);
 
+int launch_tn_x0words(const float* A, int64_t lda, const uint64_t* keep_x0, float keep_scale, const float* G, int64_t ldg, const float* rowscale, float* partial,
+                      int64_t M, int nsplit, int64_t rows_per_split, hipStream_t st);
+
 int launch_tn_instage(const float* g, const float* mfold, const uint64_t* x0_bits, const float* X, int64_t ldx, float* partial, float* cs_partial, int64_t M, int64_t K2,
-                      int nsplit, int64_t rows_per_split, hipStream_t st, const DropSpec& xd, const DropSpec& gd);
+                      int nsplit, int64_t rows_per_split, hipStream_t st, const DropSpec& xd, const DropSpec& gd, const uint64_t* keep_x0 = nullptr,
+                      const uint32_t* keep_x = nullptr);
 
 }
diff --git a/gnn-tail-generalization_amd/csrc/cb_gemm_limb.hip b/gnn-tail-generalization_amd/csrc/cb_gemm_limb.hip
--- a/gnn-tail-generalization_amd/csrc/cb_gemm_limb.hip
+++ b/gnn-tail-generalization_amd/csrc/cb_gemm_limb.hip
@@ -1,5 +1,6 @@
 #include <stdlib.h>
 
+#include <type_traits>
 #include <utility>
 
 #include "cb_common.h"
@@ -103,13 +104,71 @@
     }
 }
 
-__global__ void __launch_bounds__(512, 2) k_gemm_tn_instage(const float* __restrict__ g, const float* __restrict__ mfold,
-                                                            const unsigned long long* __restrict__ x0_bits, const float* __restrict__ X, int64_t ldx,
-                                                            float* __restrict__ partial, float* __restrict__ cs_partial, int64_t M, int K2,
-                                                            int64_t rows_per_split, int nsplit, DropSpec xd, DropSpec gd) {
+template <bool SCALED>
+__global__ void __launch_bounds__(512, 2) k_gemm_tn_x0words(const float* __restrict__ A, int64_t lda, const unsigned long long* __restrict__ keep_x0, float keep_scale,
+                                                            const float* __restrict__ G, int64_t ldg, const float* __restrict__ rowscale,
+                                                            float* __restrict__ partial, int64_t M, int64_t rows_per_split, int nsplit) {
+  using T = LTile<4, 2, 4>;
+  using OA = ColOperandKeepX0<T::NTHR>;
+  using OB = ColOperand<T::BN, SCALED, false, T::NTHR>;
+  constexpr int K1 = 256, K2 = 256, WTN = 4;
+  static_assert(T::BM == K1 && T::BN == K2, "one tile");
+  __shared__ __attribute__((aligned(16))) char smem[2 * (OA::BYTES + OB::BYTES)];
+  const int split = blockIdx.x;
+  if (split >= nsplit) return;
+  const int64_t r_begin = (int64_t)split * rows_per_split;
+  const int64_t r_end = min(M, r_begin + rows_per_split);
+  const int t = threadIdx.x, lane = t & 63, w = t >> 6, wr = w / 2, wc = w % 2;
+
+  f32x16 acc[2][WTN];
+  zero_acc_n<WTN>(acc);
+  OA oa;
+  OB ob;
+  oa.init(lda, K1, t);
+  ob.init(ldg, K2, t);
+  oa.set_words(keep_x0, keep_scale, r_begin, r_end - r_begin, t);
+  const uint32_t aaddr[2] = {OA::frag_addr(wr * 64, lane), OA::frag_addr(wr * 64 + 32, lane)};
+  uint32_t baddr[WTN];
+#pragma unroll
+  for (int j = 0; j < WTN; ++j) baddr[j] = OB::frag_addr(wc * (32 * WTN) + 32 * j, lane);
+  limb_k_loop<WTN, 1, OA, OB>(oa, ob, smem, A + r_begin * lda, (int64_t)KS * lda, lda, G + r_begin * ldg, (int64_t)KS * ldg, ldg, SCALED ? rowscale + r_begin : nullptr,
+                              r_end - r_begin, aaddr, baddr, acc, t);
+  const int l31 = lane & 31, lh = lane >> 5;
+  float* P = partial + (int64_t)split * K1 * K2;
+#pragma unroll
+  for (int ti = 0; ti < 2; ++ti)
+#pragma unroll
+    for (int tj = 0; tj < WTN; ++tj) {
+      const int n = wc * (32 * WTN) + tj * 32 + l31;
+#pragma unroll
+      for (int reg = 0; reg < 16; ++reg) {
+        const int m = wr * 64 + ti * 32 + (reg & 3) + 8 * (reg >> 2) + 4 * lh;
+        P[(int64_t)m * K2 + n] = acc[ti][tj][reg];
+      }
+    }
+}
+
+int launch_tn_x0words(const float* A, int64_t lda, const uint64_t* keep_x0, float keep_scale, const float* G, int64_t ldg, const float* rowscale, float* partial,
+                      int64_t M, int nsplit, int64_t rows_per_split, hipStream_t st) {
+  CB_CHECK_ARG(rows_per_split % 32 == 0, CB_E_INVALID, "launch_tn_x0words: a K step must not straddle a 16-row group");
+  if (rowscale)
+    hipLaunchKernelGGL(k_gemm_tn_x0words<true>, dim3((unsigned)nsplit), dim3(512), 0, st, A, lda, (const unsigned long long*)keep_x0, keep_scale, G, ldg, rowscale, partial,
+                       M, rows_per_split, nsplit);
+  else
+    hipLaunchKernelGGL(k_gemm_tn_x0words<false>, dim3((unsigned)nsplit), dim3(512), 0, st, A, lda, (const unsigned long long*)keep_x0, keep_scale, G, ldg, rowscale, partial,
+                       M, rows_per_split, nsplit);
+  CB_LAUNCH_CHECK();
+  return CB_OK;
+}
+
+template <bool WORDS>
+__device__ __forceinline__ void tn_instage(const float* __restrict__ g, const float* __restrict__ mfold, const unsigned long long* __restrict__ x0_bits,
+                                           const float* __restrict__ X, int64_t ldx, float* __restrict__ partial, float* __restrict__ cs_partial, int64_t M, int K2,
+                                           int64_t rows_per_split, int nsplit, DropSpec xd, DropSpec gd, const unsigned long long* __restrict__ keep_x0,
+                                           const uint32_t* __restrict__ keep_x) {
   using T = LTile<4, 2, 2>;
-  using OA = ColOperandInStage<T::NTHR>;
-  using OB = ColOperand<T::BN, false, true, T::NTHR>;
+  using OA = ColOperandInStage<T::NTHR, WORDS>;
+  using OB = std::conditional_t<WORDS, ColOperandKeepX<T::NTHR>, ColOperand<T::BN, false, true, T::NTHR>>;
   constexpr int K1 = 256;
   __shared__ __attribute__((aligned(16))) char smem[2 * (OA::BYTES + OB::BYTES)];
   const int split = blockIdx.x;
@@ -125,7 +184,12 @@
   oa.init(K1, K1, t);
   ob.init(ldx, K2, t);
   oa.set_stage(g, mfold, x0_bits + r_begin * 4, gd, r_begin, r_end - r_begin, t);
-  ob.set_drop(xd, r_begin, r_end - r_begin, 0, t);
+  if constexpr (WORDS) {
+    oa.set_words(keep_x0, r_begin, t);
+    ob.set_words(keep_x, xd.scale, r_begin, r_end - r_begin, t);
+  } else {
+    ob.set_drop(xd, r_begin, r_end - r_begin, 0, t);
+  }
   const uint32_t aaddr[2] = {OA::frag_addr(wr * 64, lane), OA::frag_addr(wr * 64 + 32, lane)};
   uint32_t baddr[2];
 #pragma unroll
@@ -158,10 +222,32 @@
   }
 }
 
+__global__ void __launch_bounds__(512, 2) k_gemm_tn_instage(const float* __restrict__ g, const float* __restrict__ mfold,
+                                                            const unsigned long long* __restrict__ x0_bits, const float* __restrict__ X, int64_t ldx,
+                                                            float* __restrict__ partial, float* __restrict__ cs_partial, int64_t M, int K2,
+                                                            int64_t rows_per_split, int nsplit, DropSpec xd, DropSpec gd) {
+  tn_instage<false>(g, mfold, x0_bits, X, ldx, partial, cs_partial, M, K2, rows_per_split, nsplit, xd, gd, nullptr, nullptr);
+}
+
+__global__ void __launch_bounds__(512, 2) k_gemm_tn_instage_words(const float* __restrict__ g, const float* __restrict__ mfold,
+                                                                  const unsigned long long* __restrict__ x0_bits, const float* __restrict__ X, int64_t ldx,
+                                                                  float* __restrict__ partial, float* __restrict__ cs_partial, int64_t M, int K2,
+                                                                  int64_t rows_per_split, int nsplit, DropSpec xd, DropSpec gd,
+                                                                  const unsigned long long* __restrict__ keep_x0, const uint32_t* __restrict__ keep_x) {
+  tn_instage<true>(g, mfold, x0_bits, X, ldx, partial, cs_partial, M, K2, rows_per_split, nsplit, xd, gd, keep_x0, keep_x);
+}
+
 int launch_tn_instage(const float* g, const float* mfold, const uint64_t* x0_bits, const float* X, int64_t ldx, float* partial, float* cs_partial, int64_t M, int64_t K2,
-                      int nsplit, int64_t rows_per_split, hipStream_t st, const DropSpec& xd, const DropSpec& gd) {
-  hipLaunchKernelGGL(k_gemm_tn_instage, dim3((unsigned)nsplit), dim3(512), 0, st, g, mfold, (const unsigned long long*)x0_bits, X, ldx, partial, cs_partial, M, (int)K2,
-                     rows_per_split, nsplit, xd, gd);
+                      int nsplit, int64_t rows_per_split, hipStream_t st, const DropSpec& xd, const DropSpec& gd, const uint64_t* keep_x0, const uint32_t* keep_x) {
+  CB_CHECK_ARG(rows_per_split % 32 == 0, CB_E_INVALID, "launch_tn_instage: a K step must not straddle a 16-row group");
+  if (keep_x0 || keep_x) {
+    CB_CHECK_ARG(keep_x0 && keep_x && K2 == 128, CB_E_INVALID, "launch_tn_instage: the words form needs both word buffers and 128 features");
+    hipLaunchKernelGGL(k_gemm_tn_instage_words, dim3((unsigned)nsplit), dim3(512), 0, st, g, mfold, (const unsigned long long*)x0_bits, X, ldx, partial, cs_partial, M,
+                       (int)K2, rows_per_split, nsplit, xd, gd, (const unsigned long long*)keep_x0, keep_x);
+  } else {
+    hipLaunchKernelGGL(k_gemm_tn_instage, dim3((unsigned)nsplit), dim3(512), 0, st, g, mfold, (const unsigned long long*)x0_bits, X, ldx, partial, cs_partial, M, (int)K2,
+                       rows_per_split, nsplit, xd, gd);
+  }
   CB_LAUNCH_CHECK();
   return CB_OK;
 }
diff --git a/gnn-tail-generalization_amd/csrc/cb_limb_core.h b/gnn-tail-generalization_amd/csrc/cb_limb_core.h
--- a/gnn-tail-generalization_amd/csrc/cb_limb_core.h
+++ b/gnn-tail-generalization_amd/csrc/cb_limb_core.h
@@ -35,6 +35,10 @@
   float r = x * m;
   asm volatile("" : "+v"(r));
   return r;
+}
+
+__device__ __forceinline__ float keep_factor(uint32_t bits, int i, float scale) {
+  return __uint_as_float((uint32_t)__builtin_amdgcn_sbfe((int)bits, (unsigned)i, 1u) & __float_as_uint(scale));
 }
 
 template <int R, bool DROP = false>
@@ -285,7 +289,7 @@
   }
 };
 
-template <int NT = 512>
+template <int NT = 512, bool WORDS = false>
 struct ColOperandInStage {
   static constexpr int C = 256;
   static constexpr int ROWB = C * 2, PLANE = 16 * ROWB, BYTES = 3 * PLANE;
@@ -308,6 +312,8 @@
   int64_t drow, dtot, dwidth;
   int dcol, kw;
   float cs[4];
+  const unsigned long long* kwp;
+  unsigned long long kword;
   __device__ __forceinline__ void set_stage(const float* g, const float* mfold, const unsigned long long* bits_block, const DropSpec& d, int64_t r_begin, int64_t total,
                                             int t) {
     mdelta = mfold - g;
@@ -323,6 +329,11 @@
 #pragma unroll
     for (int i = 0; i < 4; ++i) cs[i] = 0.f;
   }
+  __device__ __forceinline__ void set_words(const unsigned long long* keep_x0, int64_t r_begin, int t) {
+    static_assert(!WORDS || KPP == 8, "nibble kw of the word's J-th half");
+    kwp = keep_x0 + (r_begin >> 4) * 64 + (t % TPR);
+    kword = 0;
+  }
   __device__ __forceinline__ void init(int64_t ld, int cols_left, int t) {
     const int k = t / TPR, nq = t % TPR;
     cok = nq * 4 < cols_left;
@@ -340,13 +351,20 @@
     const unsigned long long* b = bits + ((dtot - k_left) + (kin ? k : 0)) * 4;
 #pragma unroll
     for (int i = 0; i < 4; ++i) bw[J][i] = b[i];
+    if constexpr (WORDS && J == NV - 1) kword = kwp[((dtot - k_left) >> 4) * 64];
   }
   template <int J>
   __device__ __forceinline__ void stage(const float4 (&f)[NV], char* __restrict__ S, int64_t k_left, int t) {
     const bool live = cok && kw + KPP * J < k_left;
     const int lane = t & 63;
     float mk[4];
-    keep4(dseed, ((drow + KPP * J + (dtot - k_left)) * dwidth + dcol) >> 2, dthresh, dscale, mk);
+    if constexpr (WORDS) {
+      const uint32_t nib = (uint32_t)(kword >> (32 * J)) >> (4 * kw);
+#pragma unroll
+      for (int i = 0; i < 4; ++i) mk[i] = keep_factor(nib, i, dscale);
+    } else {
+      keep4(dseed, ((drow + KPP * J + (dtot - k_left)) * dwidth + dcol) >> 2, dthresh, dscale, mk);
+    }
     const float gv[4] = {f[J].x, f[J].y, f[J].z, f[J].w}, mv[4] = {fm[J].x, fm[J].y, fm[J].z, fm[J].w};
     float v[4];
 #pragma unroll
@@ -371,6 +389,93 @@
     typedef short s16x8 __attribute__((ext_vector_type(8)));
     const s16x8 v = __builtin_shufflevector(lo, hi, 0, 1, 2, 3, 4, 5, 6, 7);
     return __builtin_bit_cast(bf16x8, v);
+  }
+};
+
+
+template <int NT = 512>
+struct ColOperandKeepX : ColOperand<128, false, false, NT> {
+  using Base = ColOperand<128, false, false, NT>;
+  using Base::cok;
+  using Base::voff;
+  using Base::woff;
+  static constexpr int TPR = Base::TPR, KPP = Base::KPP, NV = Base::NV, PLANE = Base::PLANE, ROWB = Base::ROWB;
+  static_assert(NV == 1 && KPP == 16, "one k row per thread and step");
+  const uint32_t* kxp;
+  uint32_t kword;
+  int64_t r0, dtot;
+  float dscale;
+  int khalf;
+  __device__ __forceinline__ void set_words(const uint32_t* keep_x, float scale, int64_t r_begin, int64_t total, int t) {
+    const int k = t / TPR;
+    kxp = keep_x + 32 * (k & 7) + t % TPR;
+    khalf = __builtin_amdgcn_readfirstlane(4 * (k >> 3));
+    r0 = r_begin;
+    dtot = total;
+    dscale = scale;
+    kword = 0;
+  }
+  template <int J>
+  __device__ __forceinline__ void load(float4 (&f)[NV], const float* __restrict__ base, int64_t ld, int64_t k_left, const float* __restrict__ kscale, int t) {
+    Base::template load<J>(f, base, ld, k_left, kscale, t);
+    kword = kxp[((r0 + (dtot - k_left)) >> 6) * 256];
+  }
+  template <int J>
+  __device__ __forceinline__ void stage(const float4 (&f)[NV], char* __restrict__ S, int64_t k_left, int t) const {
+    const bool live = cok && t / TPR < k_left;
+    float v[4] = {live ? f[J].x : 0.f, live ? f[J].y : 0.f, live ? f[J].z : 0.f, live ? f[J].w : 0.f};
+    const int wq = (int)((r0 + (dtot - k_left)) >> 4) & 3;
+    const uint32_t nib = kword >> (8 * wq + khalf);
+#pragma unroll
+    for (int i = 0; i < 4; ++i) v[i] = mul_rounded(v[i], keep_factor(nib, i, dscale));
+    uint2 pl[3];
+    split4(v, pl);
+#pragma unroll
+    for (int p = 0; p < 3; ++p) *reinterpret_cast<uint2*>(S + p * PLANE + woff) = pl[p];
+  }
+};
+
+template <int NT = 512>
+struct ColOperandKeepX0 : ColOperand<256, false, false, NT> {
+  using Base = ColOperand<256, false, false, NT>;
+  using Base::cok;
+  using Base::woff;
+  static constexpr int TPR = Base::TPR, KPP = Base::KPP, NV = Base::NV, PLANE = Base::PLANE, ROWB = Base::ROWB;
+  static_assert(TPR == 64 && KPP == 8 && NV == 2, "one wavefront per k row, two k rows per thread and step");
+  const unsigned long long* kwp;
+  unsigned long long kword;
+  int64_t dtot;
+  float dscale;
+  int kw;
+  __device__ __forceinline__ void set_words(const unsigned long long* keep_x0, float scale, int64_t r_begin, int64_t total, int t) {
+    kw = __builtin_amdgcn_readfirstlane(t / TPR);
+    kwp = keep_x0 + (r_begin >> 4) * 64 + (t % TPR);
+    dtot = total;
+    dscale = scale;
+    kword = 0;
+  }
+  template <int J>
+  __device__ __forceinline__ void load(float4 (&f)[NV], const float* __restrict__ base, int64_t ld, int64_t k_left, const float* __restrict__ kscale, int t) {
+    Base::template load<J>(f, base, ld, k_left, kscale, t);
+    if constexpr (J == NV - 1) kword = kwp[((dtot - k_left) >> 4) * 64];
+  }
+  template <int J>
+  __device__ __forceinline__ void stage(const float4 (&f)[NV], char* __restrict__ S, int64_t k_left, int t) const {
+    const bool live = cok && kw + KPP * J < k_left;
+    const uint32_t nib = live ? (uint32_t)(kword >> (32 * J)) >> (4 * kw) : 0u;
+    typedef float f32x2 __attribute__((ext_vector_type(2)));
+    f32x2 lo = {f[J].x, f[J].y}, hi = {f[J].z, f[J].w};
+    lo *= dscale;
+    hi *= dscale;
+    asm volatile("" : "+v"(lo), "+v"(hi));
+    const float r[4] = {lo.x, lo.y, hi.x, hi.y};
+    float v[4];
+#pragma unroll
+    for (int i = 0; i < 4; ++i) v[i] = __uint_as_float((uint32_t)__builtin_amdgcn_sbfe((int)nib, (unsigned)i, 1u) & __float_as_uint(r[i]));
+    uint2 pl[3];
+    split4(v, pl);
+#pragma unroll
+    for (int p = 0; p < 3; ++p) *reinterpret_cast<uint2*>(S + p * PLANE + woff + J * (KPP * ROWB)) = pl[p];
   }
 };
 
diff --git a/gnn-tail-generalization_amd/gemm.py b/gnn-tail-generalization_amd/gemm.py
--- a/gnn-tail-generalization_amd/gemm.py
+++ b/gnn-tail-generalization_amd/gemm.py
@@ -139,7 +139,7 @@
     return (y, bits) if want_bits else y
 
 
-def trunk_front(x, w_in, b_in, w0, rowscale, addend, p, seed_x, seed_x0, row0=0, want_bits=False, want_drop=False, z_out=None):
+def trunk_front(x, w_in, b_in, w0, rowscale, addend, p, seed_x, seed_x0, row0=0, want_bits=False, want_drop=False, z_out=None, want_words=False):
     import ctypes
     from . import ops
     lib = _lib.load()
@@ -163,13 +163,24 @@
     z0 = z_out if z_out is not None else torch.empty((M, 256), dtype=torch.float32, device=dev)
     bits = torch.empty((M, 1, 4), dtype=torch.int64, device=dev) if want_bits else None
     xd = torch.empty((M, 256), dtype=torch.float32, device=dev) if want_drop else None
+    kx0 = kx = None
+    if want_words:
+        if not (0.0 < p < 1.0):
+            raise ValueError('trunk_front: keep words exist with p > 0 only')
+        tiles = (M + 63) // 64
+        kx0 = torch.empty((tiles, 4, 64), dtype=torch.int64, device=dev)
+        kx = torch.empty((tiles, 256), dtype=torch.int32, device=dev) if K == 128 else None
     with torch.cuda.device(dev):
         _lib.check(lib.cb_front_image_f32(_lib.ptr(w_in), _ld(w_in), K, 1, _lib.ptr(img_in), nb_in, _lib.stream_ptr()), 'cb_front_image_f32')
         _lib.check(lib.cb_agg_gemm_image_f32(_lib.ptr(w0), _ld(w0), 256, 256, 0, _lib.ptr(img0), nb0, _lib.stream_ptr()), 'cb_agg_gemm_image_f32')
-        _lib.check(lib.cb_trunk_front_f32(_lib.ptr(x), _ld(x), M, K, _lib.ptr(img_in), _lib.ptr(b_in), _lib.ptr(img0), _lib.ptr(rowscale),
-                                          _lib.ptr(addend), _ld(addend) if addend is not None else 0, _lib.ptr(x0), 256, _lib.ptr(bits),
-                                          _lib.ptr(xd), 256, _lib.ptr(z0), 256, float(p), ctypes.c_uint64(seed_x), ctypes.c_uint64(seed_x0),
-                                          ops.seed_dev_ptr(), int(row0), _lib.stream_ptr()), 'cb_trunk_front_f32')
+        args = (_lib.ptr(x), _ld(x), M, K, _lib.ptr(img_in), _lib.ptr(b_in), _lib.ptr(img0), _lib.ptr(rowscale),
+                _lib.ptr(addend), _ld(addend) if addend is not None else 0, _lib.ptr(x0), 256, _lib.ptr(bits),
+                _lib.ptr(xd), 256, _lib.ptr(z0), 256, float(p), ctypes.c_uint64(seed_x), ctypes.c_uint64(seed_x0),
+                ops.seed_dev_ptr(), int(row0))
+        if want_words:
+            _lib.check(lib.cb_trunk_front_words_f32(*args, _lib.ptr(kx0), _lib.ptr(kx), _lib.stream_ptr()), 'cb_trunk_front_words_f32')
+            return x0, bits, xd, z0, kx0, kx
+        _lib.check(lib.cb_trunk_front_f32(*args, _lib.stream_ptr()), 'cb_trunk_front_f32')
     return x0, bits, xd, z0
 
 
@@ -218,12 +229,14 @@
             and bool(lib.cb_gemm_tn_instage_supported(_lib.ptr(g_like), _lib.ptr(g_like), _lib.ptr(x), _ld(x), int(M), int(x.shape[1]))))
 
 
-def mm_tn_instage(g, mfold, x0_bits, x, p_g, g_seed, p_x, x_seed, row0=0):
+def mm_tn_instage(g, mfold, x0_bits, x, p_g, g_seed, p_x, x_seed, row0=0, keep_x0=None, keep_x=None):
     import ctypes
     from . import ops
     lib = _lib.load()
     _lib.require_device(g, mfold, x0_bits, x)
     M, K2 = x.shape
+    if keep_x0 is not None and keep_x is not None and mm_tn_instage_words_supported(g, x, M):
+        return mm_tn_instage_words(g, mfold, x0_bits, x, p_g, p_x, keep_x0, keep_x)
     if (tuple(g.shape) != (M, 256) or tuple(mfold.shape) != (M, 256) or not g.is_contiguous() or not mfold.is_contiguous() or x0_bits.numel() != 4 * M
             or not x0_bits.is_contiguous() or x0_bits.dtype != torch.int64):
         raise ValueError('mm_tn_instage: contiguous [M, 256] gradients, [M, 1, 4] int64 mask words and [M, F] features expected')
@@ -236,6 +249,54 @@
                                               float(p_g), ctypes.c_uint64(g_seed), float(p_x), ctypes.c_uint64(x_seed), ops.seed_dev_ptr(), int(row0),
                                               _lib.ptr(ws), wsb, _lib.stream_ptr()), 'cb_gemm_tn_instage_f32')
     return out, colsum
+
+
+def mm_tn_instage_words_supported(g_like, x, M):
+    lib = _lib.load()
+    return (g_like.dim() == 2 and g_like.shape[1] == 256 and g_like.is_contiguous() and x.dim() == 2 and x.stride(1) == 1
+            and bool(lib.cb_gemm_tn_instage_words_supported(_lib.ptr(g_like), _lib.ptr(g_like), _lib.ptr(x), _ld(x), int(M), int(x.shape[1]))))
+
+
+def _keep_words_ok(M, keep_x0, keep_x=False):
+    tiles = (M + 63) // 64
+    return (keep_x0 is not None and keep_x0.dtype == torch.int64 and keep_x0.is_contiguous() and keep_x0.numel() == tiles * 256
+            and (keep_x is False or (keep_x is not None and keep_x.dtype == torch.int32 and keep_x.is_contiguous() and keep_x.numel() == tiles * 256)))
+
+
+def mm_tn_instage_words(g, mfold, x0_bits, x, p_g, p_x, keep_x0, keep_x):
+    lib = _lib.load()
+    _lib.require_device(g, mfold, x0_bits, x, keep_x0, keep_x)
+    M, K2 = x.shape
+    if (tuple(g.shape) != (M, 256) or tuple(mfold.shape) != (M, 256) or not g.is_contiguous() or not mfold.is_contiguous() or x0_bits.numel() != 4 * M
+            or not x0_bits.is_contiguous() or x0_bits.dtype != torch.int64 or not _keep_words_ok(M, keep_x0, keep_x)):
+        raise ValueError('mm_tn_instage_words: contiguous [M, 256] gradients, [M, 1, 4] int64 mask words, [M, 128] features and whole tiles of keep words expected')
+    out = torch.empty((256, K2), dtype=torch.float32, device=g.device)
+    colsum = torch.empty(256, dtype=torch.float32, device=g.device)
+    wsb = lib.cb_gemm_tn_instage_workspace_bytes(M, K2)
+    ws = torch.empty(max(wsb, 16), dtype=torch.uint8, device=g.device)
+    with torch.cuda.device(g.device):
+        _lib.check(lib.cb_gemm_tn_instage_words_f32(_lib.ptr(g), _lib.ptr(mfold), _lib.ptr(x0_bits), _lib.ptr(x), _ld(x), _lib.ptr(out), _lib.ptr(colsum), M, K2,
+                                                    float(p_g), float(p_x), _lib.ptr(keep_x0), _lib.ptr(keep_x), _lib.ptr(ws), wsb, _lib.stream_ptr()),
+                   'cb_gemm_tn_instage_words_f32')
+    return out, colsum
+
+
+def mm_tn_awords(a, keep_x0, p, g, rowscale=None):
+    lib = _lib.load()
+    _lib.require_device(a, keep_x0, g, rowscale)
+    a, g = _rowmajor(a), _rowmajor(g)
+    M, K1 = a.shape
+    M2, K2 = g.shape
+    if (M != M2 or not (0.0 < p < 1.0) or not _keep_words_ok(M, keep_x0)
+            or not lib.cb_gemm_tn_awords_supported(_lib.ptr(a), _ld(a), _lib.ptr(g), _ld(g), K1, K2)):
+        return None
+    out = torch.empty((K1, K2), dtype=torch.float32, device=a.device)
+    wsb = lib.cb_gemm_tn_workspace_bytes(M, K1, K2)
+    ws = torch.empty(max(wsb, 16), dtype=torch.uint8, device=a.device)
+    with torch.cuda.device(a.device):
+        _lib.check(lib.cb_gemm_tn_awords_f32(_lib.ptr(a), _ld(a), _lib.ptr(keep_x0), float(p), _lib.ptr(g), _ld(g), _lib.ptr(rowscale), _lib.ptr(out), M, K1, K2,
+                                             _lib.ptr(ws), wsb, _lib.stream_ptr()), 'cb_gemm_tn_awords_f32')
+    return out
 
 
 def mm_tn(a, g, rowscale=None):
diff --git a/gnn-tail-generalization_amd/trunk.py b/gnn-tail-generalization_amd/trunk.py
--- a/gnn-tail-generalization_amd/trunk.py
+++ b/gnn-tail-generalization_amd/trunk.py
@@ -461,6 +461,7 @@
 
     def run(self):
         cfg, graph = self.cfg, self.graph
+        self.keep_x0 = self.keep_x = None
         (self.xd, self.x0, self.x0_bits, self.cur, self.z_front), self.indrop = self._front()
         h = self.x0.shape[1]
         self.saved_in, self.saved_bits = [self.cur], []
@@ -471,7 +472,11 @@
             self.st = (self.layers[l][1], self.mix, 1 - cfg.alpha, cfg.alpha, cfg.p, cfg.seeds[l + 2] if cfg.p > 0 else 0)
             self.keep_act = cfg.residual and l + 1 < cfg.L
             z0 = self._z0() if l == 0 else None
-            bits, self.cur, act = self._form(l, z0 is not None)(l, z0)
+            form = self._form(l, z0 is not None)
+            if (l == 0 and self.cur is None and cfg.p > 0
+                    and form in (self._form_sum_first_below, self._form_last_on_loss_rows, self._form_last_on_loss_rows_sharded)):
+                self.cur = self.saved_in[0] = self.dropped_x0()
+            bits, self.cur, act = form(l, z0)
             del z0
             if cfg.residual:
                 self.mix = act
@@ -487,10 +492,13 @@
         copy = _switch('CB_TRUNK_X0_COPY', '1') == '1'
         if (indrop or p == 0) and not c.agg_bf16 and c.L >= 1 and w_in.shape[0] == 256 and _switch('CB_TRUNK_FRONT', '1') != '0':
             w0, _b0, le0 = self.layers[0]
-            fr = gemm.trunk_front(x, w_in, b_in, w0, self.a, le0, p, seeds[0], seeds[1], row0, want_bits=bwd, want_drop=bwd and p > 0 and copy,
-                                  z_out=_exchanged(self.graph, x.shape[0]) if hasattr(self.graph, 'part') else None)
+            words = bwd and p > 0 and not hasattr(self.graph, 'part') and _switch('CB_TRUNK_KEEP_WORDS', '1') != '0'
+            fr = gemm.trunk_front(x, w_in, b_in, w0, self.a, le0, p, seeds[0], seeds[1], row0, want_bits=bwd, want_drop=bwd and p > 0 and copy and not (words and not c.residual),
+                                  z_out=_exchanged(self.graph, x.shape[0]) if hasattr(self.graph, 'part') else None, want_words=words)
             if fr is not None:
-                x0, x0_bits, cur, z_front = fr
+                if words:
+                    self.keep_x0, self.keep_x = fr[4:]
+                x0, x0_bits, cur, z_front = fr[:4]
                 return (x, x0, x0_bits, x0 if p == 0 else cur, z_front), True
         if indrop:
             wb = bwd and w_in.shape[0] == 256
@@ -612,7 +620,7 @@
         ctx.graph, ctx.cfg, ctx.row0, ctx.indrop, ctx.n_layer_params = graph, cfg, f.row0, f.indrop, len(layer_params)
         if f.bwd:
             _save(ctx, xd=f.xd, x0=f.x0, w_in=w_in, w_out=w_out, saved_in=f.saved_in, saved_bits=f.saved_bits, layer_params=layer_params,
-                  h_last=f.h_last, h_below=f.h_below, x0_bits=f.x0_bits)
+                  h_last=f.h_last, h_below=f.h_below, x0_bits=f.x0_bits, keep_x0=f.keep_x0, keep_x=f.keep_x)
             ro = f.ro
             ctx.saved_rows = SavedRows('S0' if (ro.plan is not None or ro.sharded is not None) else 'all',
                                        'absent' if f.h_last is not None else 'S1' if (ro.plan is not None and ro.below is not None) else 'all')
@@ -644,6 +652,7 @@
         self.xd, self.x0, self.w_in, self.w_out = sv['xd'], sv['x0'], sv['w_in'], sv['w_out']
         self.saved_in, self.saved_bits, self.x0_bits = sv['saved_in'], sv['saved_bits'], sv['x0_bits']
         self.h_last, self.h_below = sv['h_last'], sv['h_below']
+        self.keep_x0, self.keep_x = sv['keep_x0'], sv['keep_x']
         self.lp, self.where = _layers(sv['layer_params']), ctx.saved_rows
         self.a, self.bnorm = graph.norm_out, graph.norm_in
         self.need = ctx.needs_input_grad
@@ -680,6 +689,10 @@
     def _dw(self, l, x_in, gz):
         if x_in is not None:
             return gemm.mm_tn(x_in, gz, rowscale=self.a)
+        if self.keep_x0 is not None:
+            dw = gemm.mm_tn_awords(self.x0, self.keep_x0, self.p, gz, rowscale=self.a)
+            if dw is not None:
+                return dw
         return _dw_regen(self.x0, gz, self.p, self.seed(1), self.row0, self.a)
 
     def _second(self, below, g_above, pos_above=None):
@@ -847,6 +860,8 @@
             self.grads_layers[3 * c.deferred[0]] = self._dw_rows(*c.deferred)
             c.deferred = None
         fwd_j = plan.fwd[j] if (level is not None and j < len(plan.fwd)) else None
+        if l == 0 and self.saved_in[0] is None and self.keep_x0 is not None and self.need_w(0) and level is not None and (fwd_j is not None or dst is not None):
+            self.saved_in[0] = ops._dropout_raw(self.x0, self.p, self.seed(1), self.row0 * self.x0.shape[1])
         source_side = ((self.where.x_below == 'absent' and l == L - 1) or (self.h_below is not None and l == L - 2)
                        or (T.rowsparse_loss_side and fwd_j is not None and not self.need_le(l)
                            and not (self.need_w(l) and self.saved_in[l] is None)
@@ -912,7 +927,7 @@
         graph, p, need, xd, row0 = self.graph, self.p, self.need, self.xd, self.row0
         g, c.g = c.g, None
         if self.mfold is not None:
-            d_w_in, d_b_in = gemm.mm_tn_instage(g, self.mfold, self.x0_bits, xd, p, self.seed(1), p, self.seeds[0], row0)
+            d_w_in, d_b_in = gemm.mm_tn_instage(g, self.mfold, self.x0_bits, xd, p, self.seed(1), p, self.seeds[0], row0, keep_x0=self.keep_x0, keep_x=self.keep_x)
             del g
             self.gx0 = self.g_mix = self.mfold = None
             graph.instage_folds = getattr(graph, 'instage_folds', 0) + 1
diff --git a/include/coldbrew_hip.h b/include/coldbrew_hip.h
--- a/include/coldbrew_hip.h
+++ b/include/coldbrew_hip.h
@@ -197,6 +197,12 @@
                        const float* rowscale, const float* addend, int64_t ld_add, float* x0, int64_t ld_x0, uint64_t* relu_bits, float* x0_drop,
                        int64_t ld_drop, float* z0, int64_t ld_z, float drop_p, uint64_t seed_x, uint64_t seed_x0, const uint64_t* seed_dev,
                        int64_t row0, void* stream);
+size_t cb_front_keep_x0_bytes(int64_t M);
+size_t cb_front_keep_x_bytes(int64_t M);
+int cb_trunk_front_words_f32(const float* x, int64_t ld_x, int64_t M, int64_t K, const void* image_in, const float* bias_in, const void* image_0,
+                             const float* rowscale, const float* addend, int64_t ld_add, float* x0, int64_t ld_x0, uint64_t* relu_bits, float* x0_drop,
+                             int64_t ld_drop, float* z0, int64_t ld_z, float drop_p, uint64_t seed_x, uint64_t seed_x0, const uint64_t* seed_dev,
+                             int64_t row0, uint64_t* keep_x0, uint32_t* keep_x, void* stream);
 
 int cb_spmm_csr_weighted_f32(const int32_t* rowptr, const int32_t* col, const float* w, int64_t N, int64_t E, const float* h, int64_t ld_h,
                              int64_t d, const float* row_scale, const float* bias, int relu, float* out, int64_t ld_out, void* stream);
@@ -222,6 +228,13 @@
 int cb_gemm_tn_instage_f32(const float* g, const float* mfold, const uint64_t* x0_bits, const float* X, int64_t ldx, float* C, float* colsum, int64_t M, int64_t K2,
                            float g_drop_p, uint64_t g_seed, float x_drop_p, uint64_t x_seed, const uint64_t* seed_dev, int64_t row0, void* ws, size_t ws_bytes,
                            void* stream);
+int cb_gemm_tn_instage_words_supported(const float* g, const float* mfold, const float* X, int64_t ldx, int64_t M, int64_t K2);
+int cb_gemm_tn_instage_words_f32(const float* g, const float* mfold, const uint64_t* x0_bits, const float* X, int64_t ldx, float* C, float* colsum, int64_t M,
+                                 int64_t K2, float g_drop_p, float x_drop_p, const uint64_t* keep_x0, const uint32_t* keep_x, void* ws, size_t ws_bytes,
+                                 void* stream);
+int cb_gemm_tn_awords_supported(const float* A, int64_t lda, const float* G, int64_t ldg, int64_t K1, int64_t K2);
+int cb_gemm_tn_awords_f32(const float* A, int64_t lda, const uint64_t* keep_x0, float drop_p, const float* G, int64_t ldg, const float* rowscale, float* C,
+                          int64_t M, int64_t K1, int64_t K2, void* ws, size_t ws_bytes, void* stream);
 
 int cb_spmm_gemm_store_rows_f32(const cb_csr_view* g, const float* h, int64_t ld_h, int64_t d, const float* col_scale, float* out, int64_t ld_out,
                                 const void* image, const float* g_rowscale, const float* bias, const int64_t* row_ids, const cb_trunk_store* store,
```

After: 9.672, median of 6. Within noise of the previous version (+0.5%).
